# edavalosanaya/FastPoseCNN

Hardware: AMD Instinct MI355X
Metric: img/s end-to-end 640x480 inference; hough-vote kernel HBM GB/s vs roofline (higher is better)
Workload: dtype f32

## Files before the change

### fastposecnn_amd/_native.py

```python
import ctypes
import os

import torch

_HERE = os.path.dirname(os.path.abspath(__file__))
LIB_PATH = os.path.join(_HERE, "libfpc_hip.so")

_lib = None

_vp = ctypes.c_void_p
_i = ctypes.c_int
_i64 = ctypes.c_int64
_u64 = ctypes.c_uint64
_f = ctypes.c_float
_d = ctypes.c_double
_sz = ctypes.c_size_t

_SIGNATURES = {
    "fpc_abi_version": (ctypes.c_int, []),
    "fpc_error_string": (ctypes.c_char_p, [_i]),
    "fpc_last_hip_error": (ctypes.c_char_p, []),
    "fpc_generate_hypothesis": (_i, [_vp, _vp, _vp, _vp, _i, _i, _i, _vp]),
    "fpc_voting_for_hypothesis": (_i, [_vp, _vp, _vp, _vp, _i, _i, _i, _f, _vp]),
    "fpc_ransac_workspace_bytes": (_sz, [_i, _i, _i, _i]),
    "fpc_ransac_voting_v3": (_i, [_vp, _vp, _i64, _i64, _i64, _i64, _i, _vp, _i, _i, _i, _vp, _vp, _u64, _f, _i, _i,
                                  _vp, _vp, _vp, _vp, _vp, _vp, _vp, _vp, _vp, _sz, _vp]),
    "fpc_ransac_voting_v3_bits": (_i, [_vp, _vp, _vp, _i64, _i64, _i64, _i64, _i, _vp, _i, _i, _i, _vp, _vp, _u64, _f, _i, _i, _vp, _vp, _vp, _vp, _vp, _vp, _vp, _vp, _vp, _sz, _vp]),
    "fpc_ransac_voting_v3_pose": (_i, [_vp, _vp, _vp, _i64, _i64, _i64, _i64, _i, _vp, _i, _i, _i, _vp, _vp, _u64, _f, _i, _i, _vp, _vp, _vp, _vp, _vp, _vp, _vp, _vp,
                                       _vp, _vp, _vp, _vp, _vp, _vp, _vp, _sz, _vp]),
    "fpc_vote_set_prune": (_i, [_i, _i, ctypes.POINTER(ctypes.c_int32)]),
    "fpc_vote_prune_info": (_i, [_vp, _sz, _i, _i, _i, _i, _vp, _vp]),
    "fpc_class_compress": (_i, [_vp, _vp, _vp, _vp, _vp, _vp, _i, _i, _i, _vp, _vp, _vp, _vp, _vp, _vp]),
    "fpc_class_compress_bits": (_i, [_vp, _vp, _vp, _vp, _vp, _vp, _i, _i, _i, _vp, _vp, _vp, _vp, _vp, _vp, _vp]),
    "fpc_cc_workspace_bytes": (_sz, [_i, _i, _i]),
    "fpc_cc_bits_supported": (_i, [_i, _i, _i]),
    "fpc_fg_bits": (_i, [_vp, _i, _i, _i, _vp, _vp]),
    "fpc_cc_label_bits": (_i, [_vp, _i, _i, _i, _vp, _vp, _vp, _i, _vp, _sz, _vp]),
    "fpc_cc_label": (_i, [_vp, _i, _i, _i, _vp, _vp, _vp, _i, _vp, _sz, _vp]),
    "fpc_aggregate_workspace_bytes": (_sz, [_i]),
    "fpc_aggregate": (_i, [_vp, _vp, _vp, _vp, _vp, _vp, _i, _i, _i, _i, _vp, _vp, _vp, _vp, _vp, _vp, _vp, _vp, _vp, _vp, _sz,
                           _vp]),
    "fpc_aggregate_bits": (_i, [_vp, _vp, _vp, _vp, _vp, _vp, _i, _i, _i, _i, _vp, _vp, _vp, _vp, _vp, _vp, _vp, _vp, _vp, _vp, _vp, _vp, _sz, _vp]),
    "fpc_mask_bits_words": (_sz, [_i, _i]),
    "fpc_pose_errors": (_i, [_vp, _vp, _vp, _vp, _i, _vp, _vp, _vp, _vp, _vp, _vp, _i, _vp, _vp, _vp, _vp]),
    "fpc_pose_metrics_state_words": (_sz, [_i, _i, _i, _i, _i]),
    "fpc_pose_metrics_update": (_i, [_vp, _vp, _vp, _i, _i] + [_vp] * 11 + [_i, _vp, _i, _vp, _i, _vp, _i, _vp, _i, _vp, _i] + [_vp] * 5 + [_i, _vp]),
    "fpc_confusion_update": (_i, [_vp, _vp, _i64, _i, _vp, _vp]),
    "fpc_post_network_backward": (_i, [_vp, _vp, _i, _i, _i, _i, _vp, _vp, _f, _i, _u64, _vp, _vp, _vp, _vp, _vp, _vp]),
    "fpc_vote_refine_backward": (_i, [_vp, _vp, _i64, _i64, _i64, _i64, _i, _i, _i, _vp, _f, _i, _u64, _vp, _vp, _vp]),
    "fpc_class_compress_backward": (_i, [_vp, _vp, _vp, _vp, _vp, _vp, _vp, _i, _i, _i, _vp, _vp, _vp, _vp, _vp]),
    "fpc_mask_losses": (_i, [_vp, _vp, _i, _i, _i, _i64, _i64, _f, _f, _vp, _vp, _vp, _vp]),
    "fpc_match_assign": (_i, [_vp, _vp, _vp, _i, _i, _vp, _vp, _vp, _vp]),
    "fpc_matched_losses": (_i, [_vp, _vp, _vp, _i, _i] + [_vp] * 10 + [_i, _d, _i, _i, _i, ctypes.POINTER(_d)] + [_vp] * 5),
    "fpc_matched_losses_backward": (_i, [_vp, _vp, _vp, _i, _i] + [_vp] * 10 + [_i, _d, _i, _i, _i, ctypes.POINTER(_d)] + [_vp] * 8),
    "fpc_grad_sumsq": (_i, [_vp, _sz, _vp, _vp]),
    "fpc_lookahead_radam_step": (_i, [_vp, _vp, _vp, _vp, _vp, _sz, _f, _f, _f, _f, _f, _i64, _i, _f, _vp, _vp]),
    "fpc_pose_rt": (_i, [_vp, _vp, _vp, _vp, _i, _vp, _vp, _vp, _vp]),
    "fpc_pack_pose_records": (_i, [_vp] * 9 + [_i, _i, _i, _vp, _vp]),
    "fpc_mask_iou_workspace_bytes": (_sz, [_i, _i, _i64]),
    "fpc_mask_iou": (_i, [_vp, _i, _vp, _i, _i64, _i, _vp, _vp, _vp, _vp, _sz, _vp]),
    "fpc_preprocess_workspace_bytes": (_sz, [_i]),
    "fpc_preprocess_u8": (_i, [_vp, _i, _i, _i, ctypes.POINTER(ctypes.c_double), ctypes.POINTER(ctypes.c_double), _i, _vp, _vp,
                               _sz, _vp]),
    "fpc_png_info": (_i, [_vp, _sz, ctypes.POINTER(ctypes.c_int32)]),
    "fpc_png_decode": (_i, [_vp, _sz, _vp, _sz, _i]),
    "fpc_png_decode_batch": (_i, [ctypes.POINTER(_vp), ctypes.POINTER(_sz), _i, _vp, _i, _i, _i]),
    "fpc_inflate_host": (_i, [_vp, _sz, _vp, _sz, ctypes.POINTER(_sz)]),
    "fpc_png_pack_bytes": (_sz, [_i, _i, _i]),
    "fpc_png_pack_batch": (_i, [ctypes.POINTER(_vp), ctypes.POINTER(_sz), _i, _i, _i, _i, _vp, _sz, _vp, ctypes.POINTER(_sz)]),
    "fpc_png_decode_device_workspace_bytes": (_sz, [_i, _i, _i, _i]),
    "fpc_png_decode_device": (_i, [_vp, _sz, _vp, _i, _i, _i, _i, _i, _vp, _sz, _vp, _vp, _sz, _vp]),
    "fpc_gt_build": (_i, [_vp, _i64, _i64, _i, _i, _i, _vp, _vp, _vp, _i, _vp, _vp, _i, _vp, _vp]),
    "fpc_depth_decode": (_i, [_vp, _i, _i, _i, _i, _i, _vp, _vp]),
    "fpc_net_create": (_i, [ctypes.c_char_p, _i, _i, _i, _i, ctypes.POINTER(_vp)]),
    "fpc_net_create_encoder": (_i, [_i, ctypes.POINTER(_i), _i, _i, _i, _i, ctypes.POINTER(_vp)]),
    "fpc_net_create_encoder_ex": (_i, [_i, ctypes.POINTER(_i), _i, _i, _i, _i, _i, _i, ctypes.POINTER(_vp)]),
    "fpc_net_create_encoder_se": (_i, [ctypes.POINTER(_i), _i, _i, _i, _i, _i, ctypes.POINTER(_vp)]),
    "fpc_net_destroy": (None, [_vp]),
    "fpc_net_set_graph": (_i, [_vp, _i]),
    "fpc_net_set_split_precision": (_i, [_vp, _i]),
    "fpc_net_param_count": (_i, [_vp]),
    "fpc_net_param_name": (ctypes.c_char_p, [_vp, _i]),
    "fpc_net_param_numel": (_i64, [_vp, _i]),
    "fpc_net_workspace_bytes": (_sz, [_vp]),
    "fpc_net_load_params": (_i, [_vp, _vp, _i, _vp, _sz, _vp]),
    "fpc_net_forward": (_i, [_vp, _vp, _vp, _vp, _vp, _vp, _vp, _vp, _vp, _vp, _vp, _vp, _vp]),
    "fpc_net_forward_bits": (_i, [_vp, _vp, _vp, _vp, _vp, _vp, _vp, _vp, _vp, _vp, _vp, _vp, _vp, _vp]),
    "fpc_net_autotune_next": (_i, [_vp, _i]),
    "fpc_net_conv_count": (_i, [_vp]),
    "fpc_net_conv_plan": (_i, [_vp, _i, ctypes.POINTER(_i)]),
    "fpc_net_copy_plans": (_i, [_vp, _vp]),
    "fpc_net_force_winograd": (_i, [_vp, _i]),
    "fpc_net_force_pointwise": (_i, [_vp, _i]),
    "fpc_net_force_fold": (_i, [_vp, _i]),
    "fpc_net_force_direct_h3": (_i, [_vp, _i]),
    "fpc_net_force_stem_pool": (_i, [_vp, _i]),
    "fpc_act_range": (_i, [_vp, ctypes.c_longlong, _vp, _vp]),
    "fpc_net_survey_next": (_i, [_vp, _vp, _i]),
    "fpc_net_guard_ranges": (_i, [_vp, ctypes.POINTER(ctypes.c_uint32), _i, _f, _f]),
    "fpc_net_guarded": (_i, [_vp, _i]),
    "fpc_stem_pool_tasks": (_i, [_i, _i, ctypes.POINTER(_i64)]),
    "fpc_wino_pack_geometry": (_i, [_i, _i, _i, _i, _i, ctypes.POINTER(_i64)]),
    "fpc_net_set_wino_pack": (_i, [_vp, _i]),
    "fpc_net_set_wino_orient": (_i, [_vp, _i]),
    "fpc_wino_orient_geometry": (_i, [_i, _i, _i, _i, _i, _i, ctypes.POINTER(_i64)]),
    "fpc_wino_recip": (_i, [ctypes.c_uint32, ctypes.POINTER(_i64)]),
    "fpc_wino_decode": (_i, [_i, _i, _i, _i, _i, _i, _i, ctypes.POINTER(_i64)]),
    "fpc_net_wino_blocks": (_i64, [_vp]),
    "fpc_net_graph_recorded": (_i, [_vp]),
    "fpc_net_flops": (_i, [_vp, ctypes.POINTER(ctypes.c_double)]),
    "fpc_net_tensor": (_i, [_vp, ctypes.c_char_p, ctypes.POINTER(_vp), ctypes.POINTER(_i), ctypes.POINTER(_i),
                            ctypes.POINTER(_i)]),
    "fpc_conv2d_workspace_bytes": (_sz, [_i, _i, _i, _i, _i, _i, _i]),
    "fpc_conv2d_workspace_bytes_for": (_sz, [_i, _i, _i, _i, _i, _i, _i, _i, _i, _i]),
    "fpc_conv2d_plan": (_i, [_i, _i, _i, _i, _i, _i, _i, _i, _i, _i, ctypes.POINTER(_i)]),
    "fpc_conv2d": (_i, [_vp, _i64, _i64, _i64, _i64, _vp, _vp, _vp, _vp, _vp, _vp, _vp, _i, _i, _i, _i, _i, _i, _i, _i,
                        _i, _i, _i, _i, _i, _vp, _sz, _vp]),
    "fpc_conv2d_grouped_workspace_bytes": (_sz, [_i, _i]),
    "fpc_conv2d_grouped": (_i, [_vp, _i64, _i64, _i64, _i64, _vp, _vp, _vp, _vp, _i, _i, _i, _i, _i, _i, _i, _i, _vp, _sz, _vp]),
    "fpc_conv2d_grouped_dgrad_workspace_bytes": (_sz, [_i, _i]),
    "fpc_conv2d_grouped_dgrad": (_i, [_vp, _vp, _vp, _i, _i, _i, _i, _i, _i, _vp, _sz, _vp]),
    "fpc_conv2d_grouped_wgrad_workspace_bytes": (_sz, [_i, _i, _i, _i, _i]),
    "fpc_conv2d_grouped_wgrad": (_i, [_vp, _i64, _i64, _i64, _vp, _vp, _i, _i, _i, _i, _i, _i, _vp, _sz, _vp]),
    "fpc_image_nhwc4": (_i, [_vp, _vp, _i, _i, _i, _vp]),
    "fpc_stem_wgrad_workspace_bytes": (_sz, [_i, _i, _i]),
    "fpc_stem_wgrad_slices": (_i, [_i, _i, _i]),
    "fpc_stem_wgrad": (_i, [_vp, _vp, _vp, _i, _i, _i, _vp, _sz, _vp]),
    "fpc_maxpool3x3s2_fwd": (_i, [_vp, _vp, _i, _i, _i, _i, _vp]),
    "fpc_maxpool3x3s2_bwd": (_i, [_vp, _vp, _vp, _i, _i, _i, _i, _vp]),
    "fpc_se_pool_slabs": (_i, [_i, _i, _i]),
    "fpc_se_scratch_floats": (_sz, [_i, _i, _i, _i]),
    "fpc_se_gate": (_i, [_vp, _vp, _vp, _vp, _vp, _vp, _vp, _i, _i, _i, _i, _i, _vp]),
    "fpc_se_scale_add_relu": (_i, [_vp, _vp, _vp, _vp, _i, _i, _i, _i, _vp]),
    "fpc_maxpool3x3s2_ceil_fwd": (_i, [_vp, _vp, _i, _i, _i, _i, _vp]),
    "fpc_dwconv3x3": (_i, [_vp, _vp, _vp, _vp, _vp, _i, _i, _i, _i, _i, _i, _vp]),
    "fpc_conv1x1_f32": (_i, [_vp, _vp, _vp, _vp, _vp, _vp, _i64, _i, _i, _i, _vp]),
    "fpc_conv1x1_f32_form": (_i, [_i64, _i, _i]),
    "fpc_stem3x3s2": (_i, [_vp, _vp, _vp, _vp, _vp, _i, _i, _i, _i, _vp]),
    "fpc_dwconv3x3_dgrad": (_i, [_vp, _vp, _vp, _i, _i, _i, _i, _i, _vp]),
    "fpc_dwconv3x3_wgrad_workspace_bytes": (_sz, [_i, _i, _i, _i]),
    "fpc_dwconv3x3_wgrad": (_i, [_vp, _vp, _vp, _i, _i, _i, _i, _i, _vp, _sz, _vp]),
    "fpc_se_gate_train": (_i, [_vp] * 9 + [_i, _i, _i, _i, _i, _vp]),
    "fpc_se_bwd_scratch_floats": (_sz, [_i, _i, _i, _i, _i]),
    "fpc_se_bwd": (_i, [_vp] * 15 + [_i, _i, _i, _i, _i, _vp]),
    "fpc_conv2d_wgrad_workspace_bytes": (_sz, [_i, _i, _i, _i, _i, _i, _i]),
    "fpc_upsample_bilinear_fwd": (_i, [_vp, _i64, _i64, _i64, _i64, _vp, _i, _i, _i, _i, _i, _i, _vp]),
    "fpc_upsample_bilinear_bwd_scratch_floats": (_sz, [_i, _i, _i, _i, _i]),
    "fpc_upsample_bilinear_bwd": (_i, [_vp, _i64, _i64, _i64, _i64, _vp, _vp, _i, _i, _i, _i, _i, _i, _vp]),
    "fpc_groupnorm4_relu_scratch_floats": (_sz, [_i, _i, _i]),
    "fpc_groupnorm4_relu_fwd": (_i, [_vp, _vp, _vp, _vp, _vp, _vp, _i, _i, _i, _i, ctypes.c_float, _vp]),
    "fpc_groupnorm4_relu_bwd": (_i, [_vp, _vp, _vp, _vp, _vp, _vp, _vp, _i, _i, _i, _i, _vp]),
    "fpc_batchnorm_scratch_floats": (_sz, [_i, _i]),
    "fpc_batchnorm_fwd": (_i, [_vp, _vp, _vp, _vp, _vp, _vp, _vp, _vp, _vp, _i, _i, _f, _f, _i, _vp]),
    "fpc_batchnorm_bwd": (_i, [_vp, _vp, _vp, _vp, _vp, _vp, _vp, _vp, _vp, _vp, _i, _i, _i, _vp]),
    "fpc_batchnorm_act_fwd": (_i, [_vp, _vp, _vp, _vp, _vp, _vp, _vp, _vp, _vp, _i, _i, _f, _f, _i, _vp]),
    "fpc_batchnorm_act_bwd": (_i, [_vp, _vp, _vp, _vp, _vp, _vp, _vp, _vp, _vp, _vp, _i, _i, _i, _vp]),
    "fpc_conv2d_wgrad": (_i, [_vp, _i64, _i64, _i64, _vp, _vp, _i, _i, _i, _i, _i, _i, _i, _i, _i, _vp, _sz, _vp]),
    "fpc_conv2d_wgrad_split": (_i, [_vp, _i64, _i64, _i64, _vp, _vp, _i, _i, _i, _i, _i, _i, _i, _i, _i, _vp, _sz, _vp]),
}

EXPORTED = tuple(_SIGNATURES)


def lib():
    global _lib
    if _lib is None:
        if not os.path.exists(LIB_PATH):
            raise RuntimeError(
                f"fastposecnn_amd: {LIB_PATH} is missing — build it with `python -m fastposecnn_amd.build` "
                "(hipcc --offload-arch=gfx950). There is no CPU fallback for the HIP hot path.")
        L = ctypes.CDLL(LIB_PATH)
        for name, (res, args) in _SIGNATURES.items():
            fn = getattr(L, name)
            fn.restype = res
            fn.argtypes = args
        if L.fpc_abi_version() != 11:
            raise RuntimeError("fastposecnn_amd: libfpc_hip.so ABI version mismatch")
        _lib = L
    return _lib


def check(rc, what):
    if rc != 0:
        L = lib()
        msg = L.fpc_error_string(rc).decode()
        hip = L.fpc_last_hip_error().decode() if rc == -3 else ""
        raise RuntimeError(f"fastposecnn_amd: {what} failed: {msg} (code {rc}){' — HIP: ' + hip if hip else ''}")


def ptr(t):
    return None if t is None else t.data_ptr()


_raw_stream = getattr(torch._C, "_cuda_getCurrentRawStream", None)
_cur_device = getattr(torch._C, "_cuda_getDevice", None)


def stream():
    if _raw_stream is not None and _cur_device is not None:
        return _raw_stream(_cur_device())
    return torch.cuda.current_stream().cuda_stream


def require_gpu(*tensors, what="this op"):
    for t in tensors:
        if t is not None and not t.is_cuda:
            raise RuntimeError(f"fastposecnn_amd: {what} runs only on GPU tensors (HIP kernels, no CPU fallback)")


_workspaces = {}


def workspace(tag, device, nbytes):
    key = (tag, device.index, stream())
    ws = _workspaces.get(key)
    if ws is None or ws.numel() < nbytes:
        ws = torch.empty(max(int(nbytes), 256), dtype=torch.uint8, device=device)
        assert ws.data_ptr() % 256 == 0
        _workspaces[key] = ws
    return ws
```

### fastposecnn_amd/csrc/conv2d.hip

```cpp
#include <algorithm>

#include "conv_plan.hpp"

using namespace fpc;

extern "C" int fpc_stem_pool_tasks(int Ho, int Wo, int64_t* out4) {
    if (!out4 || Ho < 2 || (Ho & 1) || Wo < 64 || (Wo & 63)) return FPC_EINVAL;
    long long o[4];
    stem_pool_tasks(Ho, Wo, kStemPoolBand, o);
    for (int i = 0; i < 4; ++i) out4[i] = o[i];
    return FPC_OK;
}

extern "C" int fpc_wino_pack_geometry(int H, int W, int B, int Cin, int fold, int64_t* out8) {
    if (!out8 || H < 1 || W < 1 || B < 1 || Cin < 1) return FPC_EINVAL;
    const WinoPackGeom q = wino_pack_geometry(H, W, B, Cin, !fold);
    out8[0] = q.G; out8[1] = q.tbx; out8[2] = q.tby; out8[3] = q.patches; out8[4] = q.slots; out8[5] = q.tiles; out8[6] = q.gn_rows;
    out8[7] = q.rx;
    return FPC_OK;
}

extern "C" int fpc_wino_orient_geometry(int H, int W, int B, int Cin, int fold, int pack, int64_t* out9) {
    if (!out9 || H < 1 || W < 1 || B < 1 || Cin < 1) return FPC_EINVAL;
    bool tr;
    const WinoPackGeom q = wino_launch_geometry(H, W, B, Cin, true, pack && !fold, &tr);
    out9[0] = tr ? 1 : 0;
    out9[1] = q.G; out9[2] = q.tbx; out9[3] = q.tby; out9[4] = q.patches; out9[5] = q.slots; out9[6] = q.tiles; out9[7] = q.gn_rows;
    out9[8] = q.rx;
    return FPC_OK;
}

extern "C" int fpc_wino_recip(uint32_t d, int64_t* out2) {
    if (!out2 || d < 1 || d > (1u << 31)) return FPC_EINVAL;
    const WinoRecip r = wino_recip(d);
    out2[0] = r.m; out2[1] = r.sh;
    return FPC_OK;
}
extern "C" int fpc_wino_decode(int Cout, int groups, int tbx, int tby, int W, int B, int pack, int64_t* out14) {
    if (!out14 || Cout < 64 || groups < 1 || tbx < 1 || tby < 1 || W < 1 || B < 1 || pack < 0) return FPC_EINVAL;
    const WinoDecode d = wino_decode(Cout, groups, tbx, tby, W, B, pack);
    const WinoRecip r[7] = {d.nnb, d.groups, d.tbx, d.tby, d.per, d.tbxl, d.tcw};
    for (int i = 0; i < 7; ++i) { out14[2 * i] = r[i].m; out14[2 * i + 1] = r[i].sh; }
    return FPC_OK;
}

extern "C" size_t fpc_conv2d_workspace_bytes(int B, int Ho, int Wo, int Cin, int Cout, int Kh, int Kw) {
    int K = Cin * Kh * Kw, Kpad = cdiv(K, kConvBK) * kConvBK, Npad = cdiv(Cout, kConvNAlign) * kConvNAlign;
    size_t packed = conv_packed_floats(Npad, Kpad);
    size_t splitk = (size_t)32 * B * (cdiv(Ho * Wo, 128) * 128) * Npad;
    size_t wino = wino_region_floats(kImgH3, Cout, Cin, true);
    return (packed + splitk + wino + kConvTickets) * sizeof(float);
}

namespace {
struct Conv2dLayout { size_t packed, splitk, wino, tickets, total; };
Conv2dLayout conv2d_layout(int B, int Cin, int Cout, int Kh, int Kw, const ConvPlan& p, const Conv2dRequest& r) {
    const int K = Cin * Kh * Kw, Kpad = cdiv(K, kConvBK) * kConvBK, Npad = cdiv(Cout, kConvNAlign) * kConvNAlign;
    Conv2dLayout L;
    L.packed = r.wino ? 0 : conv_packed_floats(Npad, Kpad);
    L.splitk = r.wino ? 0 : (splitk_floats_for(p, 1, B, Npad) + 63) / 64 * 64;
    L.wino = r.wino ? wino_region_floats(kWinoForms[r.wino].image, Cout, Cin, Cout % 128 == 0) : 0;
    L.tickets = (!r.wino && p.fused && p.nsplit > 1) ? kConvTickets : 0;
    L.total = L.packed + L.splitk + L.wino + L.tickets;
    return L;
}
ConvPlan conv2d_plan_for(int B, int Ho, int Wo, int Cin, int Cout, int Kh, int Kw, int bm, int bn, const Conv2dRequest& r) {
    const int Kpad = cdiv(Cin * Kh * Kw, kConvBK) * kConvBK;
    ConvPlan p = plan_conv(Ho * Wo, B, Cout, Kpad / kConvBK, 1, r.wino ? 0 : bm, bn, r.wino ? 1 : r.nsplit);
    p.bf3 = r.bf3 ? 1 : 0;
    p.h3 = r.h3 ? 1 : 0;
    if (r.two_launch) p.fused = 0;
    p.lat = r.lat;
    p.stem = r.stem ? 256 : 0;
    p.pool = r.pool ? 1 : 0;
    p.pw = r.pw;
    p.wino = r.wino;
    return p;
}
}

extern "C" int fpc_conv2d_plan(int B, int Ho, int Wo, int Cin, int Cout, int Kh, int Kw, int bm, int bn, int nsplit,
                               int* out4) {
    if (!out4) return FPC_EINVAL;
    const int Kpad = cdiv(Cin * Kh * Kw, kConvBK) * kConvBK;
    const Conv2dRequest r = decode_plan(nsplit);
    ConvPlan p = plan_conv(Ho * Wo, B, Cout, Kpad / kConvBK, 1, bm, bn, r.nsplit);
    p.wino = r.wino;
    out4[0] = p.bm; out4[1] = p.bn; out4[2] = r.wino ? nsplit : p.nsplit; out4[3] = plan_gn_rows(p, Ho, Wo, B, Cin, r.pack, r.orient);
    return FPC_OK;
}

extern "C" size_t fpc_conv2d_workspace_bytes_for(int B, int Ho, int Wo, int Cin, int Cout, int Kh, int Kw, int bm, int bn,
                                                 int nsplit) {
    if (B < 1 || Ho < 1 || Wo < 1 || Cin < 1 || Cout < 1 || Kh < 1 || Kw < 1) return 0;
    const Conv2dRequest r = decode_plan(nsplit);
    const ConvPlan p = conv2d_plan_for(B, Ho, Wo, Cin, Cout, Kh, Kw, bm, bn, r);
    return std::max<size_t>(conv2d_layout(B, Cin, Cout, Kh, Kw, p, r).total * sizeof(float), 256);
}

extern "C" int fpc_conv2d(const float* in, int64_t sb, int64_t sh, int64_t sw, int64_t sc, const float* w_oihw,
                          const float* scale, const float* shift, const float* res, const float* up, float* out,
                          float* gn_part, int B, int Hi, int Wi, int Cin, int Cout, int Kh, int Kw, int stride, int pad,
                          int relu, int bm, int bn, int nsplit, void* ws, size_t ws_bytes, fpc_stream_t stream) {
    if (!in || !w_oihw || !out || !ws || B < 1 || Kh != Kw) return FPC_EINVAL;
    int Ho = conv_out(Hi, Kh, stride, pad), Wo = conv_out(Wi, Kw, stride, pad);
    if (Ho < 1 || Wo < 1) return FPC_EINVAL;
    const Conv2dRequest rq = decode_plan(nsplit);
    if (rq.grp) return FPC_EINVAL;
    const int wino = rq.wino;
    ConvPlan p = conv2d_plan_for(B, Ho, Wo, Cin, Cout, Kh, Kw, bm, bn, rq);
    const Conv2dLayout lay = conv2d_layout(B, Cin, Cout, Kh, Kw, p, rq);
    if (ws_bytes < lay.total * sizeof(float) || ((uintptr_t)ws & 255)) return FPC_EWORKSPACE;
    PackedConv c;
    c.Cin = c.Cinp = Cin; c.Cout = Cout; c.Kh = Kh; c.Kw = Kw; c.stride = stride; c.pad = pad;
    c.K = Cin * Kh * Kw; c.Kpad = cdiv(c.K, kConvBK) * kConvBK; c.Npad = cdiv(Cout, kConvNAlign) * kConvNAlign;
    hipStream_t s = (hipStream_t)stream;
    float* packed = (float*)ws;
    if (rq.stem) {
        if (Cin != 4 || Kh != 7 || stride != 2 || pad != 3 || Cout != 64 || sc != 1 || sw != 4 || sh != (int64_t)4 * Wi ||
            sb != (int64_t)4 * Hi * Wi || res || up || gn_part)
            return FPC_EINVAL;
        c.Kwp = 8; c.K = 4 * 7 * 8; c.Kpad = 224;
        FPC_TRY((rq.pool ? launch_pack_weight_h3 : launch_pack_weight_bf3)(w_oihw, packed, Cout, Cin, Cin, Kh, Kw, c.Kwp, c.Npad, c.Kpad, s));
        ConvArgs a0;
        fill_conv_shape(a0, B, c, p, Hi, Wi, Ho, Wo, sb, sh, sw, sc, relu != 0, 0);
        a0.Cin = 8 * c.Cinp; a0.Kw = 1; a0.K = c.K; a0.lanepx = 1;
        a0.p[0] = ConvPtrs{in, packed, out, scale, shift, nullptr, nullptr, nullptr};
        return rq.pool ? launch_stem_pool(a0, packed, out, Ho / 2, Wo / 2, s) : launch_conv_plan(a0, p, 1, s);
    }
    static_assert(FPC_IGEMM_DMA_B, "the split-precision direct form stages its B rows from the bf16 planes by LDS-DMA; a build that loads "
                                   "them from the f32 image must pack that image here as well");
    if (!wino) FPC_TRY((p.h3 ? launch_pack_weight_h3 : p.bf3 ? launch_pack_weight_bf3 : launch_pack_weight)(w_oihw, packed, Cout, Cin, Cin, Kh, Kw, Kw, c.Npad, c.Kpad, s));
    int mode = (sc == 1 && Cin % kConvBK == 0 && Kh * Kw <= 32 && ((int64_t)Hi + 2 * pad) * sh * 4 < ((int64_t)1 << 31)) ? 0
               : (sc == 1 && Cin % 4 == 0 && sw % 4 == 0 && sh % 4 == 0 && sb % 4 == 0 && ((uintptr_t)in & 15) == 0) ? 2 : 1;
    ConvArgs a;
    fill_conv_shape(a, B, c, p, Hi, Wi, Ho, Wo, sb, sh, sw, sc, relu != 0, mode);
    a.wino_pack = rq.pack ? 1 : 0;
    a.wino_orient = rq.orient ? 1 : 0;
    a.splitk_ws = packed + lay.packed;
    a.p[0] = ConvPtrs{in, packed, out, scale, shift, res, up, gn_part};
    if (lay.tickets) {
        float* tk = packed + lay.packed + lay.splitk + lay.wino;
        a.tickets = (int*)tk;
        if (hipMemsetAsync(tk, 0, kConvTickets * sizeof(int), s) != hipSuccess) return FPC_ELAUNCH;
    }
#ifdef FPC_STAMP_WINO
    if (wino && relu == 77) { a.dbg = gn_part; a.p[0].gn_part = nullptr; a.relu = 0; }
#endif
#ifdef FPC_STAMP_IGEMM
    if (!wino && relu == 77) { a.dbg = gn_part; a.p[0].gn_part = nullptr; a.relu = 0; }
#endif
    if (wino) {
        if (Kh != 3 || stride != 1 || pad != 1 || Cin % 8 || Cout % 64 || sc != 1 || up || sw != Cin ||
            sh != (int64_t)Wi * Cin || sb != (int64_t)Hi * Wi * Cin)
            return FPC_EINVAL;
        float* wp = packed + lay.packed + lay.splitk;
        if (!wino_form_ok(wino, Cin, Cout)) return FPC_EINVAL;
        const WinoImage img = kWinoForms[wino].image;
        if (rq.orient && wino_orient_rule(Ho, Wo)) FPC_TRY(launch_wino_pack_h3(w_oihw, wp + wino_image_offset(img, Cout, Cin), Cout, Cin, true, s));
        else FPC_TRY(kWinoImages[img].pack(w_oihw, wp + wino_image_offset(img, Cout, Cin), Cout, Cin, s));
        a.wino_w[0] = wp;
        a.zeros = zero_page();
        if (!a.zeros) {
            float* zp = wp + lay.wino - 64;
            if (hipMemsetAsync(zp, 0, 64 * sizeof(float), s) != hipSuccess) return FPC_ELAUNCH;
            a.zeros = zp;
        }
        return launch_conv_plan(a, p, 1, s);
    }
    if (p.h3) {
        if (mode != 0) return FPC_EINVAL;
        a.h3_w[0] = packed;
        return launch_conv_plan(a, p, 1, s);
    }
    a.bf3 = (p.bf3 && mode == 0) ? 1 : 0;
    if (p.bf3 && mode != 0) return FPC_EINVAL;
    if (p.lat || p.pw) return launch_conv_plan(a, p, 1, s);
    return launch_conv_plan(a, ConvPlan{a.bm, a.bn, a.nsplit, a.mtiles, a.ntiles, 0, a.bf3, a.fused}, 1, s);
}

extern "C" size_t fpc_conv2d_grouped_workspace_bytes(int C, int groups) {
    if (C < 32 || C % 32 || groups < 1 || C % groups || !grouped_cg_ok(C / groups)) return 0;
    return std::max<size_t>(align_up((size_t)C * (C / groups) * 9 * sizeof(float), 256), 256);
}

extern "C" int fpc_conv2d_grouped(const float* in, int64_t sb, int64_t sh, int64_t sw, int64_t sc, const float* w_oihw,
                                  const float* scale, const float* shift, float* out, int B, int Hi, int Wi, int C, int groups,
                                  int stride, int relu, int form, void* ws, size_t ws_bytes, fpc_stream_t stream) {
    if (!in || !w_oihw || !out || !ws || B < 1 || Hi < 1 || Wi < 1 || C < 32 || C % 32 || groups < 1 || C % groups ||
        !grouped_cg_ok(C / groups) || (stride != 1 && stride != 2) || sc != 1 || form < 0 || form >= 1000)
        return FPC_EINVAL;
    const Conv2dRequest rq = decode_plan(FPC_PLAN_GROUPED + form);
    if (!rq.grp || rq.grp > kGroupedForms) return FPC_EINVAL;
    if (ws_bytes < fpc_conv2d_grouped_workspace_bytes(C, groups) || ((uintptr_t)ws & 255)) return FPC_EWORKSPACE;
    hipStream_t s = (hipStream_t)stream;
    GroupedArgs g;
    memset(&g, 0, sizeof(g));
    g.in = in; g.w = (const float*)ws; g.out = out; g.scale = scale; g.shift = shift;
    g.in_sb = sb; g.in_sh = sh; g.in_sw = sw;
    g.B = B; g.Hi = Hi; g.Wi = Wi; g.Ho = conv_out(Hi, 3, stride, 1); g.Wo = conv_out(Wi, 3, stride, 1);
    g.C = C; g.CG = C / groups; g.stride = stride; g.relu = relu ? 1 : 0; g.form = rq.grp - 1;
    if (((uintptr_t)in | (uintptr_t)out | (uintptr_t)scale | (uintptr_t)shift | (uintptr_t)w_oihw) & 15) return FPC_EINVAL;
    if ((sb | sh | sw) % 4 || sw < C) return FPC_EINVAL;
    FPC_TRY(launch_pack_grouped(w_oihw, (float*)ws, C, g.CG, s));
    return launch_conv3x3_grouped(g, s);
}
```

### fastposecnn_amd/csrc/conv_launch.hip

```cpp
#include "conv_plan.hpp"

namespace fpc {

int launch_conv_plan(ConvArgs& a, const ConvPlan& p, int groups, hipStream_t s) {
    if (p.grp || a.cg) {
        if (!p.grp || p.grp > kGroupedForms || !a.cg || !a.grp_w || groups != 1 || a.in_sc != 1 || a.Kh != 3 || a.pad != 1 ||
            a.Cin != a.Cout || a.p[0].res || a.p[0].up || a.p[0].gn_part)
            return FPC_EINVAL;
        GroupedArgs g;
        memset(&g, 0, sizeof(g));
        g.in = a.p[0].in; g.w = a.grp_w; g.out = a.p[0].out; g.scale = a.p[0].scale; g.shift = a.p[0].shift;
        g.in_sb = a.in_sb; g.in_sh = a.in_sh; g.in_sw = a.in_sw;
        g.B = a.B; g.Hi = a.Hi; g.Wi = a.Wi; g.Ho = a.Ho; g.Wo = a.Wo; g.C = a.Cout; g.CG = a.cg; g.stride = a.stride; g.relu = a.relu;
        g.form = p.grp - 1;
        return launch_conv3x3_grouped(g, s);
    }
    if (p.stem) {
        if (groups != 1 || !stem_ok(a)) return FPC_EINVAL;
        StemArgs t;
        memset(&t, 0, sizeof(t));
        t.in = a.p[0].in;
        t.wpl = reinterpret_cast<const unsigned short*>(a.p[0].w + (size_t)a.Npad * a.Kpad);
        t.out = a.p[0].out; t.scale = a.p[0].scale; t.shift = a.p[0].shift;
        t.B = a.B; t.Hi = a.Hi; t.Wi = a.Wi; t.Ho = a.Ho; t.Wo = a.Wo; t.Cout = a.Cout; t.Npad = a.Npad; t.Kpad = a.Kpad; t.relu = a.relu;
        t.grid = p.stem;
        return launch_stem7x7(t, s);
    }
    if (p.pw) {
        if (!pw_ok(a, groups)) return FPC_EINVAL;
        PwArgs w;
        memset(&w, 0, sizeof(w));
        w.in = a.p[0].in;
        for (int g = 0; g < groups; ++g) {
            w.wpl[g] = reinterpret_cast<const unsigned short*>(a.p[g].w + (size_t)a.Npad * a.Kpad);
            w.out[g] = a.p[g].out; w.scale[g] = a.p[g].scale; w.shift[g] = a.p[g].shift; w.res[g] = a.p[g].res; w.up[g] = a.p[g].up;
        }
        w.in_sb = a.in_sb; w.in_sh = a.in_sh; w.in_sw = a.in_sw;
        w.B = a.B; w.Ho = a.Ho; w.Wo = a.Wo; w.Cin = a.Cin; w.Cout = a.Cout; w.Npad = a.Npad; w.Kpad = a.Kpad; w.stride = a.stride;
        w.groups = groups; w.relu = a.relu;
        w.has_scale = a.p[0].scale != nullptr; w.has_shift = a.p[0].shift != nullptr;
        w.has_res = a.p[0].res != nullptr; w.has_up = a.p[0].up != nullptr;
        w.variant = p.pw - 1;
        return launch_conv1x1(w, s);
    }
    if (p.lat) {
        if (!lateral_ok(a, groups)) return FPC_EINVAL;
        LatArgs l;
        memset(&l, 0, sizeof(l));
        l.in = a.p[0].in;
        for (int g = 0; g < groups; ++g) {
            if (p.h3 && !a.h3_w[g]) return FPC_EINVAL;
            l.wpl[g] = reinterpret_cast<const unsigned short*>(p.h3 ? a.h3_w[g] : a.p[g].w + (size_t)a.Npad * a.Kpad);
            l.out[g] = a.p[g].out; l.shift[g] = a.p[g].shift; l.up[g] = a.p[g].up;
        }
        l.B = a.B; l.Ho = a.Ho; l.Wo = a.Wo; l.Cout = a.Cout; l.Npad = a.Npad; l.Kpad = a.Kpad; l.groups = groups; l.relu = a.relu;
        l.parts = p.lat;
        l.h3 = p.h3;
        return launch_lateral1x1(l, s);
    }
    if (p.wino) {
        if (!wino_form_ok(p.wino, a.Cin, a.Cout)) return FPC_EINVAL;
        const WinoForm& f = kWinoForms[p.wino];
        WinoArgs w;
        memset(&w, 0, sizeof(w));
        for (int g = 0; g < groups; ++g) {
            if (!a.wino_w[g] || a.p[g].up) return FPC_EINVAL;
            w.p[g] = a.p[g];
            w.p[g].w = a.wino_w[g] + wino_image_offset(f.image, a.Cout, a.Cin);
        }
        w.variant = f.variant;
        w.zeros = a.zeros;
        w.dbg = (long long*)a.dbg;
        w.groups = groups;
        w.B = a.B; w.H = a.Ho; w.W = a.Wo; w.Cin = a.Cin; w.Cout = a.Cout; w.relu = a.relu;
        w.waves = f.waves;
        const WinoGrid wg = wino_grid(p.wino, a.Ho, a.Wo);
        w.tbx = wg.tbx; w.tby = wg.tby;
        if (p.wino == kWinoH3) {
            bool tr;
            const WinoPackGeom q = wino_launch_geometry(a.Ho, a.Wo, a.B, a.Cin, a.wino_orient, a.wino_pack && !p.fold, &tr);
            if (q.G > 1 || tr) { w.pack = q.G; w.tbx = q.tbx; w.tby = q.tby; w.pack_rx = q.rx; }
            w.orient = tr ? 1 : 0;
            a.wino_blocks = q.patches * (a.Cout / 64) * groups;
        }
        if (p.fold) {
            if (p.wino != kWinoH3 || !a.fold_in) return FPC_EINVAL;
            for (int g = 0; g < groups; ++g) {
                w.in2[g] = a.fold_up[g]; w.w2[g] = a.fold_w2[g];
                w.btab[g] = a.fold_tab[g];
                w.p[g].in = a.fold_in; w.p[g].w = a.fold_w[g];
            }
            w.fold = 1; w.Cin2 = a.Cin; w.Cin = a.fold_cin;
        }
        return f.launch(w, groups, s);
    }
    a.bm = p.bm; a.bn = p.bn; a.nsplit = p.nsplit; a.mtiles = p.mtiles; a.ntiles = p.ntiles; a.groups = groups;
    a.bf3 = (p.bf3 && a.generic == 0) ? 1 : 0;
    a.fused = (p.fused && p.nsplit > 1) ? 1 : 0;
    a.h3 = 0;
    ConvArgs h;
    if (p.h3) {
        if (a.generic != 0) return FPC_EINVAL;
        h = a;
        h.bf3 = 0; h.h3 = 1;
        for (int g = 0; g < groups; ++g) {
            if (!a.h3_w[g]) return FPC_EINVAL;
            h.p[g].w = a.h3_w[g];
        }
    }
    const ConvArgs& l = p.h3 ? h : a;
    int rc = launch_conv(l, groups, s);
    if (!rc && l.nsplit > 1 && !l.fused) rc = launch_conv_splitk_epilogue(l, groups, s);
    return rc;
}

int plan_gn_rows(const ConvPlan& p, int Ho, int Wo, int B, int Cin, int pack, int orient) {
    bool tr;
    if (p.wino == kWinoH3) return wino_launch_geometry(Ho, Wo, B, Cin, orient, pack && !p.fold, &tr).gn_rows;
    return p.wino ? wino_grid(p.wino, Ho, Wo).patches() : p.mtiles * p.bm / 32;
}

int launch_stem_pool(const ConvArgs& a, const float* h3_image, float* pool, int Hp, int Wp, hipStream_t s) {
    if (!h3_image || !stem_ok(a)) return FPC_EINVAL;
    StemPoolArgs t;
    memset(&t, 0, sizeof(t));
    t.in = a.p[0].in; t.wpl = reinterpret_cast<const unsigned short*>(h3_image); t.out = pool;
    t.scale = a.p[0].scale; t.shift = a.p[0].shift;
    t.B = a.B; t.Hi = a.Hi; t.Wi = a.Wi; t.Ho = a.Ho; t.Wo = a.Wo; t.Hp = Hp; t.Wp = Wp; t.Npad = a.Npad; t.Kpad = a.Kpad; t.relu = a.relu;
    t.band = kStemPoolBand; t.grid = 256;
    return launch_stem_pool_h3(t, s);
}

}
```

### fastposecnn_amd/csrc/conv_plan.hpp

```cpp
#pragma once
#include <math.h>
#include <string.h>

#include <vector>

#include "net_kernels.hpp"

#define FPC_TRY(x) do { int rc__ = (x); if (rc__) return rc__; } while (0)

namespace fpc {

struct PackedConv {
    int Cin = 0, Cinp = 0, Cout = 0, Kh = 1, Kw = 1, stride = 1, pad = 0;
    int Kwp = 1;
    int K = 0, Kpad = 0, Npad = 0;
    int p_w = -1;
    int p_bn = -1;
    int p_bias = -1;
    size_t w_off = 0, scale_off = 0, shift_off = 0;
    size_t wino_off = 0;
    bool wino_ok = false;
    size_t h3_off = 0;
    bool h3_ok = false;
    int cg = 0;
// ... 6 lines not shown
    int bm = 64, bn = 64, nsplit = 1, mtiles = 1, ntiles = 1, wino = 0, bf3 = 0, fused = 0;
    int lat = 0;
    int stem = 0;
    int pw = 0;
    int fold = 0;
    int h3 = 0;
    int pool = 0;
    int grp = 0;
};

inline bool stem_ok(const ConvArgs& a) {
    return a.lanepx == 1 && a.generic == 0 && a.Kh == 7 && a.stride == 2 && a.pad == 3 && a.Cout == 64 && a.Kpad == 224 &&
           a.Wo % 64 == 0 && !a.p[0].res && !a.p[0].up && !a.p[0].gn_part && a.in_sc == 1 && a.in_sw == 4 &&
           a.in_sh == (long long)4 * a.Wi && a.in_sb == (long long)4 * a.Hi * a.Wi;
}

inline bool lateral_ok(const ConvArgs& a, int groups) {
    if (a.Kh != 1 || a.Kw != 1 || a.stride != 1 || a.pad != 0 || a.generic != 0 || (a.Cin != 64 && a.Cin != 128) || a.Kpad != a.Cin ||
        a.Cout % 32 != 0 || a.in_sc != 1 || a.in_sw != a.Cin || a.in_sh != (long long)a.Wi * a.Cin ||
        a.in_sb != (long long)a.Hi * a.Wi * a.Cin || a.lanepx)
        return false;
    for (int g = 0; g < groups; ++g)
        if (a.p[g].in != a.p[0].in || a.p[g].scale || a.p[g].res || a.p[g].gn_part || ((a.p[g].up != nullptr) != (a.p[0].up != nullptr)))
            return false;
    return !(a.p[0].up && ((a.Ho | a.Wo) & 1));
}

inline bool pw_ok(const ConvArgs& a, int groups) {
    if (a.Kh != 1 || a.Kw != 1 || a.pad != 0 || (a.stride != 1 && a.stride != 2) || a.generic != 0 || a.lanepx || a.Cin % 64 != 0 ||
        a.Kpad != a.Cin || a.Cout % 64 != 0 || a.in_sc != 1)
        return false;
    for (int g = 0; g < groups; ++g)
        if (a.p[g].in != a.p[0].in || a.p[g].gn_part || (a.p[g].scale != nullptr) != (a.p[0].scale != nullptr) ||
            (a.p[g].shift != nullptr) != (a.p[0].shift != nullptr) || (a.p[g].res != nullptr) != (a.p[0].res != nullptr) ||
            (a.p[g].up != nullptr) != (a.p[0].up != nullptr))
            return false;
    return !(a.p[0].up && ((a.Ho | a.Wo) & 1));
}

inline bool can_fuse(const ConvPlan& p, int groups, int B) {
    return p.nsplit > 1 && (long long)groups * B * p.mtiles * p.ntiles <= kConvTickets;
}

inline ConvPlan plan_conv(int HoWo, int B, int Cout, int ksteps, int groups, int force_bm = 0, int force_bn = 0,
                          int force_split = 0) {
    ConvPlan best;
    double best_t = 1e300;
    const int bms[2] = {64, 128}, bns[2] = {64, 128};
    for (int bi = 0; bi < 2; ++bi)
        for (int bj = 0; bj < 2; ++bj) {
            int bm = bms[bi], bn = bns[bj];
            if (force_bm && bm != force_bm) continue;
            if (force_bn && bn != force_bn) continue;
            if (!force_bn && bn == 128 && Cout <= 64) continue;
            int mt = cdiv(HoWo, bm), nt = cdiv(Cout, bn);
            for (int ns = 1; ns <= 32; ++ns) {
                if (force_split && ns != force_split) continue;
                int per = cdiv(ksteps, ns);
                if ((ns - 1) * per >= ksteps) continue;
                if (ns > 1 && (Cout % 4 != 0)) continue;
                double nblk = (double)groups * B * mt * nt * ns;
                double work = (double)(bm / 64) * (bn / 64) * per * 16.0 * 64.0 + 4000.0;
                double t = ceil(nblk / 256.0) * work + (ns > 1 ? 10000.0 + 200.0 * ns : 0.0);
                if (t < best_t) { best_t = t; best = ConvPlan{bm, bn, ns, mt, nt, 0}; }
            }
        }
    best.fused = can_fuse(best, groups, B) ? 1 : 0;
    return best;
}

inline std::vector<ConvPlan> conv_candidates(int HoWo, int B, int Cout, int ksteps, int groups) {
    std::vector<ConvPlan> out;
    const int splits[] = {1, 2, 3, 4, 6, 8, 12, 16, 24};
    for (int bm = 64; bm <= 128; bm += 64)
        for (int bn = 64; bn <= 128; bn += 64) {
            if (bn == 128 && Cout <= 64) continue;
            int mt = cdiv(HoWo, bm), nt = cdiv(Cout, bn);
            long long base = (long long)groups * B * mt * nt;
            for (int ns : splits) {
                int per = cdiv(ksteps, ns);
                if (ns > 1 && (per < 2 || (ns - 1) * per >= ksteps || Cout % 4 != 0)) continue;
                if (ns > 1 && base * ns > 4096) continue;
                out.push_back(ConvPlan{bm, bn, ns, mt, nt, 0});
                if (can_fuse(out.back(), groups, B)) { ConvPlan f = out.back(); f.fused = 1; out.push_back(f); }
            }
        }
    return out;
}

inline size_t splitk_floats_for(const ConvPlan& p, int groups, int B, int Npad) {
    return p.nsplit > 1 ? (size_t)groups * p.nsplit * B * p.mtiles * p.bm * Npad : 0;
}

enum WinoImage { kImgF32, kImgBf3, kImgC128, kImgH2, kImgH3, kWinoImageCount };
struct WinoImageDesc { int units, tail; int (*pack)(const float* w_oihw, float* packed, int Cout, int Cin, hipStream_t s); };
inline int pack_h3_plain(const float* w_oihw, float* packed, int Cout, int Cin, hipStream_t s) { return launch_wino_pack_h3(w_oihw, packed, Cout, Cin, false, s); }
constexpr WinoImageDesc kWinoImages[kWinoImageCount] = {
    {16, 0, launch_wino_pack},
    {24, 0, launch_wino_pack_bf3},
    {24, 0, launch_wino_pack_c128},
    {16, 8, launch_wino_pack_h2},
    {16, 8, pack_h3_plain},
};
constexpr size_t kWinoSlack = 128;

constexpr int kWinoFormCount = 10;
constexpr int kWinoBf3 = 5, kWinoW4 = 7;
constexpr int kWinoH2 = 8, kWinoH3 = 9;
struct WinoForm {
    int waves;
    int bn, ck;
    int variant;
    WinoImage image;
    int wg_per_cu;
    int min_split;
    bool zeros;
    bool range_limited;
    int (*launch)(const WinoArgs& a, int groups, hipStream_t s);
};
constexpr WinoForm kWinoForms[kWinoFormCount] = {
    {},
    {4, 64, 8, 0, kImgF32, 2, 0, false, false, launch_conv_wino},
    {8, 64, 8, 0, kImgF32, 1, 0, false, false, launch_conv_wino},
    {4, 64, 8, 1, kImgF32, 2, 0, false, false, launch_conv_wino},
    {8, 64, 8, 2, kImgF32, 1, 0, true, false, launch_conv_wino},
    {8, 64, 8, 3, kImgBf3, 1, 1, true, false, launch_conv_wino},
    {4, 128, 8, 0, kImgC128, 1, 1, false, false, launch_conv_wino_c128},
    {8, 64, 8, 0, kImgBf3, 1, 1, false, false, launch_conv_wino_w4},
    {8, 64, 8, 0, kImgH2, 1, 2, false, true, launch_conv_wino_h2},
    {8, 64, 16, 0, kImgH3, 1, 3, false, true, launch_conv_wino_h3},
};
inline bool wino_form_ok(int form, int Cin, int Cout) {
    return form >= 1 && form < kWinoFormCount && Cout % kWinoForms[form].bn == 0 && Cin % kWinoForms[form].ck == 0;
}
struct WinoSpan { size_t units, tails; };
inline WinoSpan wino_span(int end, bool c128) {
    WinoSpan sp{0, 0};
    for (int i = 0; i < end; ++i)
        if (i != kImgC128 || c128) { sp.units += kWinoImages[i].units; sp.tails += kWinoImages[i].tail; }
    return sp;
}
static_assert(kWinoImages[kImgH2].tail + kWinoImages[kImgH3].tail <= 64, "kWinoSlack keeps one 64-float line for all tails");
inline size_t wino_image_offset(WinoImage img, int Cout, int Cin) {
    const WinoSpan sp = wino_span(img, Cout % 128 == 0);
    return sp.units * Cout * Cin + sp.tails;
}
inline size_t wino_region_floats(WinoImage last, int Cout, int Cin, bool c128) { return (wino_span(last, c128).units + kWinoImages[last].units) * Cout * Cin + kWinoSlack; }
inline bool plan_range_limited(const ConvPlan& p) {
    return p.h3 || p.fold || p.pool || (p.wino && kWinoForms[p.wino].range_limited);
}
struct WinoGrid { int tbx, tby; int patches() const { return tbx * tby; } };
inline WinoGrid wino_grid(int form, int H, int W) { return {cdiv(cdiv(W, 2), 8), cdiv(cdiv(H, 2), kWinoForms[form].waves)}; }

struct Conv2dRequest { int nsplit; bool bf3, two_launch; int wino, lat; bool stem; int pw; bool h3, pool, pack, orient; int grp; };
inline Conv2dRequest decode_plan(int code) {
    Conv2dRequest r{code, false, false, 0, 0, false, 0, false, false, false, false, 0};
    if (code >= FPC_PLAN_GROUPED && code < FPC_PLAN_GROUPED + 1000) { r.grp = code - FPC_PLAN_GROUPED + 1; r.nsplit = 1; return r; }
    if (code == FPC_PLAN_WINO_ORIENT) { r.orient = true; r.nsplit = -kWinoH3; }
    if (code == FPC_PLAN_WINO_PACKED) { r.pack = true; r.nsplit = -kWinoH3; }
    if (r.nsplit >= FPC_PLAN_LATERAL_H3 && r.nsplit < FPC_PLAN_LATERAL_H3 + 1000) { r.lat = r.nsplit - FPC_PLAN_LATERAL_H3; r.h3 = true; r.nsplit = 1; return r; }
    if (r.nsplit >= FPC_PLAN_H3 && r.nsplit < FPC_PLAN_H3 + 200) { r.h3 = true; r.nsplit -= FPC_PLAN_H3; }
    if (r.nsplit >= FPC_PLAN_POINTWISE) { r.pw = r.nsplit - FPC_PLAN_POINTWISE + 1; r.bf3 = true; r.nsplit = 1; return r; }
    if (r.nsplit == FPC_PLAN_STEM_POOL) { r.stem = true; r.pool = true; r.h3 = true; r.nsplit = 1; return r; }
    if (r.nsplit == FPC_PLAN_STEM) { r.stem = true; r.bf3 = true; r.nsplit = 1; return r; }
    if (r.nsplit >= FPC_PLAN_LATERAL) { r.lat = r.nsplit - FPC_PLAN_LATERAL; r.bf3 = true; r.nsplit = 1; return r; }
    if (r.nsplit >= FPC_PLAN_BF3) { r.bf3 = true; r.nsplit -= FPC_PLAN_BF3; }
    if (r.nsplit >= FPC_PLAN_TWO_LAUNCH) { r.two_launch = true; r.nsplit -= FPC_PLAN_TWO_LAUNCH; }
    if (r.nsplit <= -1 && r.nsplit > -kWinoFormCount) r.wino = -r.nsplit;
    return r;
}
inline int encode_plan(const ConvPlan& p, bool folded_away) {
    if (folded_away) return FPC_PLAN_FOLDED;
    if (p.grp) return FPC_PLAN_GROUPED + p.grp - 1;
    if (p.h3) return p.lat ? FPC_PLAN_LATERAL_H3 + p.lat : FPC_PLAN_H3 + p.nsplit;
    if (p.pw) return FPC_PLAN_POINTWISE + p.pw - 1;
    if (p.stem) return p.pool ? FPC_PLAN_STEM_POOL : FPC_PLAN_STEM;
    if (p.lat) return FPC_PLAN_LATERAL + p.lat;
    return p.wino ? -p.wino : p.nsplit;
}

inline int conv_out(int x, int k, int s, int p) { return (x + 2 * p - k) / s + 1; }
inline void fill_conv_shape(ConvArgs& a, int B, const PackedConv& c, const ConvPlan& p, int Hi, int Wi, int Ho, int Wo, long long sb,
                            long long sh, long long sw, long long sc, bool relu, int mode) {
    memset(&a, 0, sizeof(a));
    a.B = B; a.Hi = Hi; a.Wi = Wi; a.Cin = c.Cin; a.Ho = Ho; a.Wo = Wo; a.Cout = c.Cout; a.Npad = c.Npad;
    a.Kh = c.Kh; a.Kw = c.Kw; a.stride = c.stride; a.pad = c.pad; a.K = c.K; a.Kpad = c.Kpad;
    a.in_sb = sb; a.in_sh = sh; a.in_sw = sw; a.in_sc = sc;
    a.relu = relu ? 1 : 0; a.nsplit = p.nsplit; a.mtiles = p.mtiles; a.ntiles = p.ntiles; a.ksteps = c.Kpad / kConvBK;
    a.bm = p.bm; a.bn = p.bn; a.generic = mode;
    a.fused = p.fused;
}

int launch_conv_plan(ConvArgs& a, const ConvPlan& p, int groups, hipStream_t s);
int plan_gn_rows(const ConvPlan& p, int Ho, int Wo, int B, int Cin, int pack, int orient);
int launch_stem_pool(const ConvArgs& a, const float* h3_image, float* pool, int Hp, int Wp, hipStream_t s);

}
```

### fastposecnn_amd/csrc/net.hip

```cpp
#include <initializer_list>
#include <utility>

#include "net_plan.hpp"

static void drop_graph(fpc_net* n) {
    if (n->graph_exec) { (void)hipGraphExecDestroy(n->graph_exec); n->graph_exec = nullptr; }
}

extern "C" void fpc_net_destroy(fpc_net_t* n) {
    if (!n) return;
    if (n->graph_exec) (void)hipGraphExecDestroy(n->graph_exec);
    delete n;
}

static int pack_h3_images(fpc_net* n, hipStream_t s) {
    for (const PackedConv& c : n->convs)
        if (c.h3_ok) {
            int rc = launch_pack_weight_h3(n->pptr[c.p_w], n->ws + c.h3_off, c.Cout, c.Cin, c.Cinp, c.Kh, c.Kw, c.Kwp, c.Npad, c.Kpad, s);
            if (rc) return rc;
        }
    if (n->c_stem >= 0) {
        const PackedConv& st = n->convs[n->c_stem];
        int rc = launch_pack_weight_h3(n->pptr[st.p_w], n->ws + n->stem_h3_off, st.Cout, st.Cin, st.Cinp, st.Kh, st.Kw, st.Kwp, st.Npad, st.Kpad, s);
        if (rc) return rc;
    }
    n->h3_packed = true;
    return FPC_OK;
}

extern "C" int fpc_net_set_split_precision(fpc_net_t* n, int on) {
    if (!n) return FPC_EINVAL;
    n->split_precision = on < 0 ? 0 : (on > 3 ? 3 : on);
    if (n->split_precision >= 3 && n->loaded && !n->h3_packed) return pack_h3_images(n, n->load_stream);
    return FPC_OK;
}

extern "C" int fpc_net_graph_recorded(const fpc_net_t* n) { return n && n->use_graph && n->graph_exec ? 1 : 0; }

extern "C" int fpc_net_set_wino_pack(fpc_net_t* n, int on) {
    if (!n || on < 0 || on > 1) return FPC_EINVAL;
    if (n->wino_pack != on) drop_graph(n);
    n->wino_pack = on;
    return FPC_OK;
}

static int pack_wino_h3_image(const fpc_net* n, int ci, hipStream_t s) {
    const PackedConv& c = n->convs[ci];
    return launch_wino_pack_h3(n->pptr[c.p_w], n->ws + c.wino_off + wino_image_offset(kImgH3, c.Cout, c.Cin), c.Cout, c.Cin,
                               n->wino_orient && n->c_tr[ci], s);
}
static int pack_fold_images(const fpc_net* n, int d, hipStream_t s) {
    const PackedConv &sc = n->convs[n->dec[d].seg[6]], &lc = n->convs[n->dec[d].lat[3]];
    const bool tr = n->wino_orient && n->c_tr[n->dec[d].seg[6]];
    int rc = launch_fold_compose(n->pptr[sc.p_w], n->pptr[lc.p_w], n->pptr[lc.p_bias], n->ws + n->fold_wc_off[d],
                                 n->ws + n->fold_tab_off[d], sc.Cout, sc.Cin, lc.Cin, tr, s);
    if (!rc) rc = launch_wino_pack_h3_pair(n->ws + n->fold_wc_off[d], n->ws + n->fold_img1_off[d], lc.Cin, n->pptr[sc.p_w],
                                           n->ws + n->fold_img2_off[d], sc.Cin, sc.Cout, tr, s);
    return rc;
}

extern "C" int fpc_net_set_wino_orient(fpc_net_t* n, int on) {
    if (!n || on < 0 || on > 1) return FPC_EINVAL;
    if (n->wino_orient == on) return FPC_OK;
    drop_graph(n);
    n->wino_orient = on;
    if (!n->loaded) return FPC_OK;
    if (hipDeviceSynchronize() != hipSuccess) return FPC_ELAUNCH;
    for (size_t ci = 0; ci < n->convs.size(); ++ci)
        if (n->c_tr[ci] && wino_form_ok(kWinoH3, n->convs[ci].Cin, n->convs[ci].Cout)) { const int rc = pack_wino_h3_image(n, (int)ci, n->load_stream); if (rc) return rc; }
    if (n->fold_ok && n->c_tr[n->dec[0].seg[6]])
        for (int d = 0; d < 4; ++d) { const int rc = pack_fold_images(n, d, n->load_stream); if (rc) return rc; }
    return hipStreamSynchronize(n->load_stream) == hipSuccess ? FPC_OK : FPC_ELAUNCH;
}

extern "C" int64_t fpc_net_wino_blocks(const fpc_net_t* n) { return n ? (int64_t)n->wino_blocks : -1; }

extern "C" int fpc_net_set_graph(fpc_net_t* n, int on) {
    if (!n) return FPC_EINVAL;
    n->use_graph = on ? 1 : 0;
    if (!on) drop_graph(n);
    return FPC_OK;
}
extern "C" int fpc_net_param_count(const fpc_net_t* n) { return n ? (int)n->pnames.size() : 0; }
extern "C" const char* fpc_net_param_name(const fpc_net_t* n, int i) {
    return (n && i >= 0 && i < (int)n->pnames.size()) ? n->pnames[i].c_str() : nullptr;
}
extern "C" int64_t fpc_net_param_numel(const fpc_net_t* n, int i) {
    return (n && i >= 0 && i < (int)n->pnumel.size()) ? n->pnumel[i] : -1;
}
extern "C" size_t fpc_net_workspace_bytes(const fpc_net_t* n) { return n ? n->total_floats * sizeof(float) : 0; }

static int fold_bn_of(const fpc_net* n, int p_bn, int C, size_t scale_off, size_t shift_off, hipStream_t s) {
    return launch_fold_bn(n->pptr[p_bn], n->pptr[p_bn + 1], n->pptr[p_bn + 2], n->pptr[p_bn + 3], 1e-5f, C, n->ws + scale_off, n->ws + shift_off, s);
}

extern "C" int fpc_net_load_params(fpc_net_t* n, const float* const* params, int count, void* ws, size_t ws_bytes,
                                   fpc_stream_t stream) {
    if (!n || !params || count != (int)n->pnames.size() || !ws) return FPC_EINVAL;
    if (((uintptr_t)ws & 255) != 0 || ws_bytes < n->total_floats * sizeof(float)) return FPC_EWORKSPACE;
    drop_graph(n);
    for (int i = 0; i < count; ++i)
        if (!params[i] || ((uintptr_t)params[i] & 15)) return FPC_EINVAL;
    hipStream_t s = (hipStream_t)stream;
    n->ws = (float*)ws;
    n->pptr.assign(params, params + count);
    n->load_stream = s;
    n->h3_packed = false;
    if (n->split_precision >= 3) { int rc = pack_h3_images(n, s); if (rc) return rc; }
    if (hipMemsetAsync(n->ws + n->zeros_off, 0, 64 * sizeof(float), s) != hipSuccess) return FPC_ELAUNCH;
    if (hipMemsetAsync(n->ws + n->tickets_off, 0, kConvTickets * sizeof(int), s) != hipSuccess) return FPC_ELAUNCH;
    for (size_t ci = 0; ci < n->convs.size(); ++ci) {
        const PackedConv& c = n->convs[ci];
        if (c.cg) {
            int rg = launch_pack_grouped(n->pptr[c.p_w], n->ws + c.grp_off, c.Cout, c.cg, s);
            if (!rg) rg = fold_bn_of(n, c.p_bn, c.Cout, c.scale_off, c.shift_off, s);
            if (rg) return rg;
            continue;
        }
        int rc = launch_pack_weight(n->pptr[c.p_w], n->ws + c.w_off, c.Cout, c.Cin, c.Cinp, c.Kh, c.Kw, c.Kwp, c.Npad, c.Kpad, s);
        if (rc) return rc;
        rc = launch_pack_weight_bf3(n->pptr[c.p_w], n->ws + c.w_off, c.Cout, c.Cin, c.Cinp, c.Kh, c.Kw, c.Kwp, c.Npad, c.Kpad, s);
        if (rc) return rc;
        if (c.wino_ok) {
            for (int f = 1, done = 0; f < kWinoFormCount; ++f) {
                const WinoImage img = kWinoForms[f].image;
                if (!wino_form_ok(f, c.Cin, c.Cout) || (done >> img & 1)) continue;
                done |= 1 << img;
                rc = img == kImgH3 ? pack_wino_h3_image(n, (int)ci, s)
                                   : kWinoImages[img].pack(n->pptr[c.p_w], n->ws + c.wino_off + wino_image_offset(img, c.Cout, c.Cin), c.Cout, c.Cin, s);
                if (rc) return rc;
            }
        }
        if (c.p_bn >= 0) {
            rc = fold_bn_of(n, c.p_bn, c.Cout, c.scale_off, c.shift_off, s);
            if (rc) return rc;
        }
    }
    if (n->fold_ok)
        for (int d = 0; d < 4; ++d) {
            const int rc = pack_fold_images(n, d, s);
            if (rc) return rc;
        }
    for (const fpc_net::MbOp& o : n->mops) {
        const int rc = fold_bn_of(n, o.p_bn, o.Cout, o.scale_off, o.shift_off, s);
        if (rc) return rc;
    }
    n->loaded = true;
    return FPC_OK;
}

namespace {

struct ConvIO {
    const float* in; long long sb, sh, sw, sc; int Hi, Wi;
    float* out; int Ho, Wo;
    const float* res; const float* up; float* gn_part;
};

void fill_conv_args(const fpc_net* n, ConvArgs& a, const PackedConv& c, const ConvPlan& p, int Hi, int Wi, int Ho,
                    int Wo, long long sb, long long sh, long long sw, long long sc, bool relu, int mode) {
    fill_conv_shape(a, n->B, c, p, Hi, Wi, Ho, Wo, sb, sh, sw, sc, relu, mode);
    a.splitk_ws = n->ws + n->splitk_off; a.zeros = n->ws + n->zeros_off; a.tickets = (int*)(n->ws + n->tickets_off);
    a.wino_pack = n->wino_pack; a.wino_orient = n->wino_orient;
}


template <class F> float min_ms(hipStream_t s, int reps, F run) {
    hipEvent_t e0 = nullptr, e1 = nullptr;
    float ms = 1e30f;
    if (hipEventCreate(&e0) == hipSuccess && hipEventCreate(&e1) == hipSuccess)
        for (int rep = 0; rep < reps; ++rep) {
            float t = 0.f;
            bool timed = hipEventRecord(e0, s) == hipSuccess && run() == FPC_OK && hipEventRecord(e1, s) == hipSuccess &&
                         hipEventSynchronize(e1) == hipSuccess && hipEventElapsedTime(&t, e0, e1) == hipSuccess;
            if (timed && t < ms) ms = t;
        }
    if (e0) (void)hipEventDestroy(e0);
    if (e1) (void)hipEventDestroy(e1);
    return ms;
}

std::vector<ConvPlan> tune_candidates(const ConvArgs& a, int groups, int split, bool pointwise) {
    if (a.cg) {
        std::vector<ConvPlan> gc;
        for (int f = 0; f < kGroupedForms; ++f) { ConvPlan q; q.grp = f + 1; gc.push_back(q); }
        return gc;
    }
    std::vector<ConvPlan> cands = conv_candidates(a.Ho * a.Wo, a.B, a.Cout, a.ksteps, groups);
    const size_t nf = cands.size();
    if (split && a.generic == 0) {
        for (size_t i = 0; i < nf; ++i) { ConvPlan q = cands[i]; q.bf3 = 1; cands.push_back(q); }
    }
    if (split >= 3 && a.generic == 0 && a.h3_w[0]) {
        for (size_t i = 0; i < nf; ++i) { ConvPlan q = cands[i]; q.h3 = 1; cands.push_back(q); }
    }
    if (split && groups == 1 && stem_ok(a)) {
        ConvPlan sq; sq.stem = 256; cands.push_back(sq);
    }
    if (split && lateral_ok(a, groups)) {
        const int tiles = groups * (a.Cout / 32);
        for (int parts = 1; parts <= tiles; parts *= 2)
            if (tiles % parts == 0) {
                ConvPlan lq; lq.lat = parts; cands.push_back(lq);
                if (split >= 3 && a.h3_w[0]) { lq.h3 = 1; cands.push_back(lq); }
            }
    }
    if (split && pointwise && pw_ok(a, groups)) {
        ConvPlan pq;
        pq.pw = 1; cands.push_back(pq);
        pq.pw = 2; cands.push_back(pq);
    }
    if (a.wino_w[0] && !a.p[0].up) {
        auto offered = [&](int f) { return split >= kWinoForms[f].min_split && wino_form_ok(f, a.Cin, a.Cout) && (a.zeros || !kWinoForms[f].zeros); };
        for (int f = 1; f < kWinoFormCount; ++f) {
            if (!offered(f) || (f == kWinoH2 && offered(kWinoH3))) continue;
            ConvPlan wq; wq.wino = f; cands.push_back(wq);
        }
    }
    return cands;
}

struct PlanFootprint { double nblk, share; };
PlanFootprint plan_footprint(const ConvPlan& q, const ConvArgs& a, int groups) {
    bool tr;
    double nblk = q.grp ? (double)cdiv(a.Ho, 8) * cdiv(a.Wo, grouped_tile_cols(a.stride)) * (a.Cout / 32) * a.B
                  : q.stem ? 512.0
                  : q.lat ? (double)cdiv(a.Ho * a.Wo, 128) * a.B * q.lat
                  : q.pw ? (double)cdiv(a.B * a.Ho * a.Wo, pw_tile_pixels(q.pw - 1)) * (a.Cout / 64) * groups * q.pw
                  : q.wino == kWinoH3 ? (double)wino_launch_geometry(a.Ho, a.Wo, a.B, a.Cin, a.wino_orient, a.wino_pack && !q.fold, &tr).patches * (a.Cout / 64) * groups
                  : q.wino ? (double)wino_grid(q.wino, a.Ho, a.Wo).patches() * a.B * (a.Cout / kWinoForms[q.wino].bn) * groups
                         : (double)q.mtiles * q.ntiles * q.nsplit * a.B * groups;
    double share = nblk / (256.0 * (q.wino ? kWinoForms[q.wino].wg_per_cu : 2));
    if (share > 1.0) share = 1.0;
    if (share < 0.125) share = 0.125;
    return {nblk, share};
}

int survey_site(const fpc_net* n, const ConvArgs& a, const ConvPlan& p, int groups, int ci, hipStream_t s) {
    unsigned* rec = n->survey + 4 * (size_t)ci;
    if (p.fold) {
        unsigned* rec_up = n->survey + 4 * (size_t)n->dec[0].lat[3];
        int rc = launch_act_range(a.fold_in, (long long)a.B * a.Ho * a.Wo * a.fold_cin, rec, s);
        for (int g = 0; g < groups && !rc; ++g) rc = launch_act_range(a.fold_up[g], (long long)a.B * (a.Ho / 2) * (a.Wo / 2) * a.Cin, rec_up, s);
        return rc;
    }
    for (int g = 0; g < groups; ++g) {
        bool seen = false;
        for (int h = 0; h < g; ++h) seen = seen || a.p[h].in == a.p[g].in;
        if (seen) continue;
        const int rc = launch_act_range(a.p[g].in, (long long)a.B * a.in_sb, rec, s);
        if (rc) return rc;
    }
    return FPC_OK;
}

int run_conv(fpc_net* n, ConvArgs& a, int groups, int ci, hipStream_t s) {
    if (n->tuning) {
        float best_ms = 1e30f, free_ms = 1e30f;
        ConvPlan best = n->cplan[ci];
        n->has_free[ci] = 0;
        for (const ConvPlan& q : tune_candidates(a, groups, n->split_precision, n->enc.pointwise())) {
            if (splitk_floats_for(q, groups, a.B, a.Npad) > n->splitk_floats) continue;
            if (n->guarded[ci] && plan_range_limited(q)) continue;
            int rc = launch_conv_plan(a, q, groups, s);
            if (rc == FPC_EINVAL) continue;
            if (rc) return rc;
            const float ms = min_ms(s, 3, [&] { return launch_conv_plan(a, q, groups, s); });
            float score = ms;
            if (n->tune_mode >= 1) {
                const double share = plan_footprint(q, a, groups).share;
                score = ms * (float)(n->tune_mode == 2 ? share : sqrt(share));
            }
            if (score < best_ms) { best_ms = score; best = q; }
            if (score < free_ms && !plan_range_limited(q)) { free_ms = score; n->free_plan[ci] = q; n->has_free[ci] = 1; }
        }
        n->tune_score[ci] = best_ms;
        if (n->split_precision >= 3 && a.fold_in && a.fold_lat_ms > 0.f && !n->guarded[ci]) {
            ConvPlan fq;
            fq.wino = kWinoH3; fq.fold = 1;
            int rc = launch_conv_plan(a, fq, groups, s);
            if (rc && rc != FPC_EINVAL) return rc;
            const float ms = rc ? 1e30f : min_ms(s, 3, [&] { return launch_conv_plan(a, fq, groups, s); });
            if (ms < best_ms + a.fold_lat_ms) best = fq;
        }
        n->cplan[ci] = best;
    }
    const ConvPlan p = n->cplan[ci];
    if (n->survey) { const int rs = survey_site(n, a, p, groups, ci, s); if (rs) return rs; }
    const int rc = launch_conv_plan(a, p, groups, s);
    if (!rc && p.wino == kWinoH3) n->wino_blocks += a.wino_blocks;
    return rc;
}

}


static int forward_middle(fpc_net* n, hipStream_t s) {
    float* ws = n->ws;
    n->wino_blocks = 0;
    const int B = n->B, H = n->H, W = n->W;
    ConvArgs a;
    auto nhwc = [&](const Act& t, long long& sb, long long& sh, long long& sw, long long& sc) {
        sc = 1; sw = t.C; sh = (long long)t.W * t.C; sb = (long long)t.H * sh;
    };
    if (n->c_stem >= 0) {
        const PackedConv& c = n->convs[n->c_stem];
        fill_conv_args(n, a, c, n->cplan[n->c_stem], H, W, n->a_stem.H, n->a_stem.W, (long long)4 * H * W, (long long)4 * W, 4,
                       1, true, 0);
        a.Cin = 8 * c.Cinp; a.Kw = 1; a.K = c.K; a.lanepx = 1;
        a.p[0] = ConvPtrs{ws + n->a_img4.off, ws + c.w_off, ws + n->a_stem.off, ws + c.scale_off, ws + c.shift_off, nullptr, nullptr, nullptr};
        const float* h3img = n->h3_packed ? ws + n->stem_h3_off : nullptr;
        const bool ceil = n->enc.resnet.ceil_pool();
        auto pool_launch = [&]() {
            return ceil ? launch_maxpool3x3s2_ceil(ws + n->a_stem.off, ws + n->a_pool.off, B, n->a_stem.H, n->a_stem.W, 64, s)
                        : launch_maxpool3x3s2(ws + n->a_stem.off, ws + n->a_pool.off, B, n->a_stem.H, n->a_stem.W, 64, n->a_pool.H, n->a_pool.W, s);
        };
// ... 487 lines not shown
```

### fastposecnn_amd/csrc/net_kernels.hpp

```cpp
#pragma once
#include "common.hpp"

namespace fpc {

#ifndef FPC_IGEMM_DMA_B
#define FPC_IGEMM_DMA_B 1
#endif

constexpr int kMaxGroup = 4;
constexpr int kConvBK = 32;
constexpr int kConvNAlign = 128;
constexpr int kConvTickets = 16384;

struct ConvPtrs {
    const float* in;
    const float* w;
    float* out;
    const float* scale;
    const float* shift;
    const float* res;
    const float* up;
    float* gn_part;
};

struct ConvArgs {
    ConvPtrs p[kMaxGroup];
    float* splitk_ws;
    int* tickets;
    int fused;
    int B, Hi, Wi, Cin, Ho, Wo, Cout, Npad, Kh, Kw, stride, pad, K, Kpad;
    long long in_sb, in_sh, in_sw, in_sc;
    int relu, nsplit, mtiles, ntiles, ksteps, bm, bn, generic, groups;
    int bf3;
    int h3;
    int lanepx;
    const float* wino_w[kMaxGroup];
    const float* h3_w[kMaxGroup];
    const float* zeros;
    const float* fold_in;
    const float* fold_w[kMaxGroup];
    const float* fold_w2[kMaxGroup];
    const float* fold_up[kMaxGroup];
    const float* fold_tab[kMaxGroup];
    int fold_cin;
    float fold_lat_ms;
    void* dbg;
    long long wino_blocks;
    int wino_pack;
    int wino_orient;
    int cg;
    const float* grp_w;
};

struct LatArgs {
    const float* in;
    const unsigned short* wpl[kMaxGroup];
    float* out[kMaxGroup];
    const float* shift[kMaxGroup];
    const float* up[kMaxGroup];
    int B, Ho, Wo, Cout, Npad, Kpad, groups, relu;
    unsigned bias_mask;
    int parts;
    int h3;
};
int launch_lateral1x1(const LatArgs& a, hipStream_t s);

struct PwArgs {
    const float* in;
    const unsigned short* wpl[kMaxGroup];
    float* out[kMaxGroup];
    const float* scale[kMaxGroup];
    const float* shift[kMaxGroup];
    const float* res[kMaxGroup];
    const float* up[kMaxGroup];
    long long in_sb, in_sh, in_sw;
    int B, Ho, Wo, Cin, Cout, Npad, Kpad, stride, groups, relu;
    int has_scale, has_shift, has_res, has_up;
    int variant;
};
int launch_conv1x1(const PwArgs& a, hipStream_t s);
inline int pw_tile_pixels(int variant) { return variant == 0 ? 64 : 128; }

struct GroupedArgs {
    const float* in;
    const float* w;
    float* out;
    const float* scale;
    const float* shift;
    long long in_sb, in_sh, in_sw;
    int B, Hi, Wi, Ho, Wo, C, CG, stride, relu;
    int form;
    int tx, ty;
};
constexpr int kGroupedForms = 1;
bool grouped_cg_ok(int cg);
int launch_pack_grouped(const float* w_oihw, float* packed, int C, int CG, hipStream_t s, int mode = 0);
int launch_conv3x3_grouped(const GroupedArgs& a, hipStream_t s);
inline int grouped_tile_cols(int stride) { return stride == 1 ? 16 : 8; }

struct StemArgs {
    const float* in;
    const unsigned short* wpl;
    float* out;
    const float* scale;
    const float* shift;
    int B, Hi, Wi, Ho, Wo, Cout, Npad, Kpad, relu;
    int grid;
};
int launch_stem7x7(const StemArgs& a, hipStream_t s);

struct StemPoolArgs {
    const float* in;
    const unsigned short* wpl;
    float* out;
    const float* scale;
    const float* shift;
    int B, Hi, Wi, Ho, Wo, Hp, Wp, Npad, Kpad, relu;
    int band;
    int grid;
};
constexpr int kStemPoolBand = 10;
int launch_stem_pool_h3(const StemPoolArgs& a, hipStream_t s);
void stem_pool_tasks(int Ho, int Wo, int band, long long out4[4]);

constexpr int kMaxGnSites = 4;
struct GnFinArgs {
    const float* gn_part[kMaxGnSites * kMaxGroup];
    const float* gamma[kMaxGnSites * kMaxGroup];
    const float* beta[kMaxGnSites * kMaxGroup];
    float* affine[kMaxGnSites * kMaxGroup];
    int P[kMaxGnSites];
    long long count[kMaxGnSites];
    int B, C, groups, sites;
    float eps;
};

constexpr int kMaxUpJobs = 2;
struct GnUpArgs {
    const float* in[kMaxUpJobs * kMaxGroup];
    const float* affine[kMaxUpJobs * kMaxGroup];
    float* out[kMaxUpJobs * kMaxGroup];
    int h[kMaxUpJobs], w[kMaxUpJobs];
    int B, C, jobs;
};

struct MergeHeadArgs {
    const float* t_lo[kMaxGroup][3];
    const float* a_lo[kMaxGroup][3];
    const float* t_hi[kMaxGroup];
    const float* a_hi[kMaxGroup];
    const float* hw[kMaxGroup];
    const float* hb[kMaxGroup];
    float* out[kMaxGroup];
    int ch[kMaxGroup];
    int chp[kMaxGroup];
    int B, h, w, C;
};

struct HeadPartArgs {
    const float* t[kMaxGroup][3];
    const float* aff[kMaxGroup][3];
    const float* hw[kMaxGroup];
    const float* hb[kMaxGroup];
    const float* lsum[kMaxGroup];
    float* out[kMaxGroup];
    int ch[kMaxGroup], chp[kMaxGroup];
    int B, H, W, C, hl, wl;
};
int launch_head_part(const HeadPartArgs& a, bool hi, int groups, hipStream_t s);

struct Up4Args {
    const float* lm; const float* lq; const float* lt; const float* ls;
    int pm, pq, pt, ps;
    float* o_mask; float* o_quat; float* o_scales; float* o_xy; float* o_z;
    long long* cat_mask; float* cq; float* cs; float* cxy; float* cz;
    int B, hl, wl, H, W, C;
    unsigned long long* fg_bits; size_t fg_stride;
};

#ifdef FPC_STAMP_WINO
constexpr bool kWinoStamp = true;
#else
constexpr bool kWinoStamp = false;
#endif
constexpr int kWinoSerialStamps = 16;

struct WinoRecip { unsigned m; int sh; };
inline WinoRecip wino_recip(unsigned d) {
    int l = 0;
    while ((1ull << l) < d) ++l;
    const int sh = 31 + l;
    return WinoRecip{(unsigned)(((1ull << sh) + d - 1) / d), sh};
}
struct WinoDecode { WinoRecip nnb, groups, tbx, tby, per, tbxl, tcw; };
inline WinoDecode wino_decode(int Cout, int groups, int tbx, int tby, int W, int B, int pack) {
    const int tcw = (W + 1) / 2, last = pack > 0 ? ((B % pack) * tcw + 7) / 8 : 0;
    return WinoDecode{wino_recip(Cout / 64), wino_recip(groups), wino_recip(tbx), wino_recip(tby), wino_recip(tbx * tby),
                      wino_recip(last ? last : tbx), wino_recip(tcw)};
}

struct WinoArgs {
    ConvPtrs p[kMaxGroup];
    long long* dbg;
    const float* zeros;
    int variant;
    int groups;
    int waves;
    int B, H, W, Cin, Cout, relu, tbx, tby;
    const float* in2[kMaxGroup];
    const float* w2[kMaxGroup];
    const float* btab[kMaxGroup];
    int fold, Cin2;
    int pack, pack_rx;
    int orient;
    WinoDecode dec;
};
int launch_conv_wino(const WinoArgs& a, int groups, hipStream_t s);
const float* zero_page();
int launch_wino_pack(const float* w_oihw, float* packed, int Cout, int Cin, hipStream_t s);
int launch_wino_pack_bf3(const float* w_oihw, float* packed, int Cout, int Cin, hipStream_t s);
int launch_conv_wino_c128(const WinoArgs& a, int groups, hipStream_t s);
int launch_wino_pack_c128(const float* w_oihw, float* packed, int Cout, int Cin, hipStream_t s);
int launch_conv_wino_w4(const WinoArgs& a, int groups, hipStream_t s);
int launch_conv_wino_h2(const WinoArgs& a, int groups, hipStream_t s);
int launch_wino_pack_h2(const float* w_oihw, float* packed, int Cout, int Cin, hipStream_t s);
int launch_absmax_bits(const float* w, long long n, unsigned* out_bits, hipStream_t s);
int launch_act_range(const float* x, long long n, unsigned* rec4, hipStream_t s);
int launch_conv_wino_h3(const WinoArgs& a, int groups, hipStream_t s);
struct WinoPackGeom { int G, tbx, tby, rx; long long patches, slots, tiles; int gn_rows; };
WinoPackGeom wino_pack_geometry(int H, int W, int B, int Cin, bool allow);
bool wino_orient_rule(int H, int W);
WinoPackGeom wino_launch_geometry(int H, int W, int B, int Cin, bool orient, bool pack_allow, bool* transposed);
int launch_wino_pack_h3(const float* w_oihw, float* packed, int Cout, int Cin, bool transpose, hipStream_t s);
int launch_wino_pack_h3_pair(const float* w1, float* packed1, int Cin1, const float* w2, float* packed2, int Cin2, int Cout, bool transpose,
                             hipStream_t s);
int launch_fold_compose(const float* W, const float* L, const float* bias, float* wc, float* btab, int Cout, int Cmid, int Cin,
                        bool transpose, hipStream_t s);
int launch_conv(const ConvArgs& a, int groups, hipStream_t s);
int launch_conv_splitk_epilogue(const ConvArgs& a, int groups, hipStream_t s);
int launch_maxpool3x3s2(const float* in, float* out, int B, int Hi, int Wi, int C, int Ho, int Wo, hipStream_t s);
int launch_maxpool3x3s2_ceil(const float* in, float* out, int B, int Hi, int Wi, int C, hipStream_t s);
int se_pool_slabs(int H, int W, int C);
int launch_se_pool(const float* x, float* partial, int B, int H, int W, int C, hipStream_t s);
int launch_se_excite(const float* partial, const float* w1, const float* b1, const float* w2, const float* b2, float* gate, int B, int H,
                     int W, int C, int R, hipStream_t s);
int launch_se_scale_add_relu(const float* x, const float* gate, const float* res, float* y, int B, int H, int W, int C, hipStream_t s);
int launch_se_excite_train(const float* partial, const float* w1, const float* b1, const float* w2, const float* b2, float* gate,
                           float* mean, float* hidden, int B, int H, int W, int C, int R, hipStream_t s);
constexpr int kSeThreads = 256;
constexpr int kSeRowPixels = 64;
constexpr int kSeMaxC = 8192;
inline int se_lanes(int C) { return C / 4 < kSeThreads ? C / 4 : kSeThreads; }
inline int se_rows(int C) { return kSeThreads / se_lanes(C); }
inline bool se_shape_ok(int B, int H, int W, int C) {
    return B >= 1 && B <= 65535 && H >= 1 && W >= 1 && C >= 64 && C % 64 == 0 && C <= kSeMaxC && (long long)H * W < (1LL << 31) &&
           (long long)B * H * W * (C / 4) < (1LL << 32) - 4096LL * 256 - 8;
}
int launch_stem3x3s2(const float* in4, const float* w, const float* scale, const float* shift, float* out, int B, int Hi, int Wi,
                     hipStream_t s);
int launch_dwconv3x3(const float* in, const float* w, const float* scale, const float* shift, float* out, int B, int Hi, int Wi, int C,
                     int stride, int act, hipStream_t s);
int launch_conv1x1_f32(const float* in, const float* w, const float* scale, const float* shift, const float* res, float* out, long long M,
                       int Cin, int Cout, int act, hipStream_t s);
int conv1x1_f32_tiles(long long M, int Cout);
int launch_gn_finalize(const GnFinArgs& a, int groups, hipStream_t s);
int launch_gn_relu_up2(const GnUpArgs& a, int groups, hipStream_t s);
int launch_merge_head(const MergeHeadArgs& a, int groups, hipStream_t s);
int launch_up4_compress(const Up4Args& a, hipStream_t s, bool allow_wide = true);
void launch_up4_compress7x4(const Up4Args& a, hipStream_t s);
void launch_up4_compress_wide(const Up4Args& a, hipStream_t s);

struct Lerp { int i0, i1; float l0, l1; };
__device__ __forceinline__ Lerp lerp_coord(int dst, int in, int out) {
    float scale = out > 1 ? (float)(in - 1) / (float)(out - 1) : 0.f;
    float src = scale * (float)dst;
    Lerp L;
    L.i0 = (int)src;
    L.i1 = L.i0 + (L.i0 < in - 1 ? 1 : 0);
    L.l1 = src - (float)L.i0;
    L.l0 = 1.f - L.l1;
    return L;
}

__device__ __forceinline__ Lerp lerp_scaled(int dst, int in, float scale) {
    float src = scale * (float)dst;
    Lerp L;
    L.i0 = (int)src;
    L.i1 = L.i0 + (L.i0 < in - 1 ? 1 : 0);
    L.l1 = src - (float)L.i0;
    L.l0 = 1.f - L.l1;
    return L;
}

int launch_pack_weight(const float* w_oihw, float* packed, int Cout, int Cin, int Cinp, int Kh, int Kw, int Kwp, int Npad,
                       int Kpad, hipStream_t s);
int launch_pack_weight_bf3(const float* w_oihw, float* packed, int Cout, int Cin, int Cinp, int Kh, int Kw, int Kwp, int Npad,
                           int Kpad, hipStream_t s);
inline size_t conv_packed_floats(int Npad, int Kpad) { return ((size_t)Npad * Kpad * 5 / 2 + 63) / 64 * 64; }
int launch_pack_weight_h3(const float* w_oihw, float* packed, int Cout, int Cin, int Cinp, int Kh, int Kw, int Kwp, int Npad,
                          int Kpad, hipStream_t s);
inline size_t h3_packed_floats(int Npad, int Kpad) { return ((size_t)Npad * Kpad + 2 + 63) / 64 * 64; }
int launch_nchw3_to_nhwc4(const float* x, float* out, int B, int HW, hipStream_t s);
int launch_fold_bn(const float* gamma, const float* beta, const float* mean, const float* var, float eps, int C,
                   float* scale, float* shift, hipStream_t s);

}
```

### fastposecnn_amd/csrc/net_plan.hpp

```cpp
#pragma once
#include <string>

#include "conv_plan.hpp"

using namespace fpc;

enum Buf { kBufNone, kBufIn, kBufT1, kBufT2, kBufD, kBufY, kBufRes, kBufCount };
struct BlockSite { int k; bool strided, grouped; Buf in, out; bool relu; Buf res; };
struct BlockKind {
    int nsites;
    BlockSite site[3];
    int ds_before;
    bool se_gate;
    bool shared;
};
constexpr BlockKind kBasicBlock = {2, {{3, true, false, kBufIn, kBufT1, true, kBufNone}, {3, false, false, kBufT1, kBufY, true, kBufRes}}, 1, false, false};
constexpr BlockKind kBottleneck = {3, {{1, false, false, kBufIn, kBufT1, true, kBufNone}, {3, true, true, kBufT1, kBufT2, true, kBufNone}, {1, false, false, kBufT2, kBufY, true, kBufRes}}, 2, false, true};
constexpr BlockKind kSEBottleneck = {3, {{1, true, false, kBufIn, kBufT1, true, kBufNone}, {3, false, false, kBufT1, kBufT2, true, kBufNone}, {1, false, false, kBufT2, kBufY, false, kBufNone}}, 2, true, true};

enum EncoderFamily {
    kFamilyResNet,
    kFamilyMobileNetV2,
    kFamilyCount
};
struct ResNetDesc {
    int expansion = 1;
    int groups = 1, width = 64;
    int se = 0;
    const BlockKind& kind() const { return se ? kSEBottleneck : expansion == 4 ? kBottleneck : kBasicBlock; }
    const char* stem_prefix() const { return se ? "encoder.layer0." : "encoder."; }
    bool ceil_pool() const { return se != 0; }
};
struct EncoderDesc {
    EncoderFamily family = kFamilyResNet;
    ResNetDesc resnet;
    int layers[4] = {};
    bool basic() const { return family == kFamilyResNet && resnet.expansion == 1; }
    bool pointwise() const { return family == kFamilyResNet && resnet.expansion == 4; }
};

enum StepKind {
    kStepConv,
    kStepSeGate,
    kStepMb
};
struct Step { StepKind kind; int op; Act in, out; bool relu; Act res; };
inline Step conv_step(int conv, const Act& in, const Act& out, bool relu, const Act& res = Act()) {
    Step s; s.kind = kStepConv; s.op = conv; s.in = in; s.out = out; s.relu = relu; s.res = res; return s;
}
inline Step se_gate_step(int p_se, const Act& y, const Act& res) {
    Step s; s.kind = kStepSeGate; s.op = p_se; s.in = s.out = y; s.relu = true; s.res = res; return s;
}
inline Step mb_step(int mop, const Act& in, const Act& out, const Act& res = Act()) {
    Step s; s.kind = kStepMb; s.op = mop; s.in = in; s.out = out; s.relu = false; s.res = res; return s;
}

struct fpc_net {
    EncoderDesc enc;
    int classes, B, H, W;
    std::vector<std::string> pnames;
    std::vector<int64_t> pnumel;
    std::vector<const float*> pptr;
    std::vector<PackedConv> convs;
    size_t packed_floats = 0;
    size_t total_floats = 0;
    float* ws = nullptr;
    bool loaded = false;
    bool tuning = false;
    bool tuned = false;
    int tune_mode = 0;

    int c_stem = -1;
    std::vector<Step> tape;
    enum MbKind { kMbStem, kMbDw, kMbPw };
    struct MbOp { MbKind kind; int p_w, p_bn, Cin, Cout, stride, act; size_t scale_off, shift_off; long long howo; };
    std::vector<MbOp> mops;
    int add_mop(MbKind kind, const std::string& wname, int64_t wnumel, const std::string& bn, int Cin, int Cout, int stride, int act) {
        MbOp o{kind, add_param(wname, wnumel), add_bn(bn, Cout), Cin, Cout, stride, act, 0, 0, 0};
        o.scale_off = alloc(Cout); o.shift_off = alloc(Cout);
        mops.push_back(o);
        return (int)mops.size() - 1;
    }
    struct Dec {
        int lat[4];
        int seg[7];
        int p_gn[7];
        int p_head_w, p_head_b;
        int head_ch, head_chp;
    } dec[4];

    Act a_img4, a_stem, a_pool;
    Act a_feat[4];
    Act a_p[4][4];
    Act a_seg[4][7];
    Act a_up[4][3];
    size_t gn_part_off[4][7], gn_aff_off[4][7];
    int gn_P[7];
    Act a_low[4];
    Act a_lsum[4];
    int up4_wide = 1;
    int merge_split = -1;
    size_t splitk_off = 0, splitk_floats = 0;
    size_t se_gate_off = 0, se_part_off = 0;
    int use_graph = 0;
    long long wino_blocks = 0;
    int wino_pack = 1;
    int wino_orient = 1;
    std::vector<char> c_tr;
    int split_precision = 0;
    hipGraphExec_t graph_exec = nullptr;
    size_t zeros_off = 0;
    size_t tickets_off = 0;

    bool h3_packed = false;
    hipStream_t load_stream = nullptr;
    size_t stem_h3_off = 0;
    bool fold_ok = false;
    size_t fold_wc_off[4] = {}, fold_img1_off[4] = {}, fold_img2_off[4] = {}, fold_tab_off[4] = {};

    std::vector<ConvPlan> cplan;
    std::vector<float> tune_score;
    unsigned* survey = nullptr;
    std::vector<ConvPlan> free_plan;
    std::vector<char> has_free;
    std::vector<char> guarded;
    std::vector<int> c_howo, c_groups;

    size_t bump = 0;
    size_t alloc(size_t n) { size_t o = bump; bump += (n + 63) / 64 * 64; return o; }
    Act alloc_act(int h, int w, int c) { Act a; a.H = h; a.W = w; a.C = c; a.off = alloc((size_t)B * h * w * c); return a; }
    int add_param(const std::string& n, int64_t numel) { pnames.push_back(n); pnumel.push_back(numel); return (int)pnames.size() - 1; }
    int add_bn(const std::string& p, int C) {
        add_param(p + ".weight", C); add_param(p + ".bias", C); add_param(p + ".running_mean", C);
        return add_param(p + ".running_var", C) - 3;
    }

    int add_conv(const std::string& wname, int Cin, int Cout, int k, int stride, int pad, const char* bn_prefix,
                 const char* bias_name, int Cinp = 0, int Kwp = 0) {
        PackedConv c;
        c.Cin = Cin; c.Cinp = Cinp ? Cinp : Cin; c.Cout = Cout; c.Kh = c.Kw = k; c.stride = stride; c.pad = pad;
        c.Kwp = Kwp ? Kwp : k;
        c.K = c.Cinp * k * c.Kwp; c.Kpad = cdiv(c.K, kConvBK) * kConvBK; c.Npad = cdiv(Cout, kConvNAlign) * kConvNAlign;
        c.p_w = add_param(wname, (int64_t)Cout * Cin * k * k);
        if (bn_prefix) c.p_bn = add_bn(bn_prefix, Cout);
        if (bias_name) c.p_bias = add_param(bias_name, Cout);
        c.w_off = alloc(conv_packed_floats(c.Npad, c.Kpad));
        if (bn_prefix) { c.scale_off = alloc(Cout); c.shift_off = alloc(Cout); }
        c.wino_ok = (k == 3 && stride == 1 && pad == 1 && c.Cinp == Cin && Cin % 8 == 0 && Cout % 64 == 0);
        if (c.wino_ok) c.wino_off = alloc(wino_region_floats(kImgH3, Cout, Cin, Cout % 128 == 0));
        convs.push_back(c);
        return (int)convs.size() - 1;
    }
    int add_grouped_conv(const std::string& wname, int C, int cg, int stride, const char* bn_prefix) {
        PackedConv c;
        c.Cin = c.Cinp = c.Cout = C; c.Kh = c.Kw = c.Kwp = 3; c.stride = stride; c.pad = 1; c.cg = cg;
        c.K = cg * 9; c.Kpad = cdiv(c.K, kConvBK) * kConvBK; c.Npad = cdiv(C, kConvNAlign) * kConvNAlign;
        c.p_w = add_param(wname, (int64_t)C * cg * 9);
        c.p_bn = add_bn(bn_prefix, C);
        c.grp_off = alloc((size_t)C * cg * 9);
        c.scale_off = alloc(C); c.shift_off = alloc(C);
        convs.push_back(c);
        return (int)convs.size() - 1;
    }
};

inline int lateral_mode(const PackedConv& c) { return c.Cin % kConvBK == 0 ? 0 : 2; }
```

### fastposecnn_amd/csrc/wino_h3.hip

```cpp
#include <algorithm>
#ifdef FPC_STAMP_WINO
#include <cstdlib>
#endif
#include <type_traits>
#include "wino_tile.hpp"

namespace fpc {
using namespace wino_tile;

namespace {

constexpr int kRing = 4;
static_assert(kLdsFloats >= kRing * kInFloats, "the K loop's input ring lives in the output image's space");

__device__ __forceinline__ const float* sgpr_ptr(const float* p) {
    const unsigned long long v = reinterpret_cast<unsigned long long>(p);
    const unsigned lo = __builtin_amdgcn_readfirstlane((unsigned)v), hi = __builtin_amdgcn_readfirstlane((unsigned)(v >> 32));
    return reinterpret_cast<const float*>(((unsigned long long)hi << 32) | lo);
}

}

template <int VAR, bool FOLD, bool PACK, bool TR = false>
__global__ __launch_bounds__(256, 1) void k_conv_wino_h3(const WinoArgs a) {
    __shared__ __attribute__((aligned(16))) float lds[kLdsFloats];
    long long* const dbg = kWinoStamp ? a.dbg : nullptr;
    const long long t_entry = dbg ? clock64() : 0;
    const int t = threadIdx.x, lane = t & 63;
    const int wi = __builtin_amdgcn_readfirstlane(t >> 6);
    const int li = lane & 31, lh = lane >> 5;
    const int H = a.H, W = a.W, Cout = a.Cout;
    const int nnb = Cout / kBN;
    const WinoPatch pt = wino_patch<PACK>(blockIdx.x, nnb, a.groups, a.tbx, a.tby, a.pack, W, a.B, a.dec);
    const int nb = pt.nb, grp = pt.grp, pk_ks = pt.pk_ks;
    const ConvPtrs P = wino_group(a.p[0], a.p[1], a.p[2], a.p[3], grp);
    const int y_in0 = 2 * pt.ty0 - 1, x_in0 = 2 * pt.tx0 - 1;
    const bool fine = kWinoStamp && dbg && a.variant == kWinoSerialStamps;
    long long t_dec = fine ? clock64() : 0, t_wld = 0, t_plan = 0, t_zero = 0;

    f32x16 acc[4][2][2];
    float inv_s = 1.f;
    long long t_issued = 0, t_landed = 0, t_synced = 0, c_begin = 0, r_begin = 0;
    const bool stamp = dbg != nullptr;

    auto kloop = [&](auto ph, const float* src, const float* wimg, const int Cs, const int up) __attribute__((always_inline)) {
    constexpr int PH = decltype(ph)::value;
    constexpr bool SKIPC = PH == 1;
    const int nkb = Cs >> 3;
    const int npair = nkb >> 1;
    const __amdgpu_buffer_rsrc_t rs_w = make_rsrc(reinterpret_cast<const char*>(wimg) + (size_t)nb * npair * kPairBytes);
    inv_s = wimg[(size_t)nnb * npair * (kPairBytes / 4)];
    const int vo_u = lane * 16;
    int so_u = wi * 4 * 4096;
    u32x4 U1[4][2], U2[4][2];
#define FPC_H3_XI_LIVE(J) (!(SKIPC && (J) == 2))
#define FPC_H3_LOAD_U1_AT(SO, J, NT) do { if (FPC_H3_XI_LIVE(J)) U1[J][NT] = __builtin_bit_cast(u32x4, __builtin_amdgcn_raw_buffer_load_b128(rs_w, vo_u, (SO) + (J) * 4096 + (NT) * 2048, 0)); } while (0)
#define FPC_H3_LOAD_U2_AT(SO, J, NT) do { if (FPC_H3_XI_LIVE(J)) U2[J][NT] = __builtin_bit_cast(u32x4, __builtin_amdgcn_raw_buffer_load_b128(rs_w, vo_u, (SO) + (J) * 4096 + (NT) * 2048 + 1024, 0)); } while (0)
#define FPC_H3_LOAD_U1(J, NT) FPC_H3_LOAD_U1_AT(so_u, J, NT)
#define FPC_H3_LOAD_U2(J, NT) FPC_H3_LOAD_U2_AT(so_u, J, NT)
#pragma unroll
    for (int j = 0; j < 4; ++j)
#pragma unroll
        for (int nt = 0; nt < 2; ++nt) { FPC_H3_LOAD_U1(j, nt); FPC_H3_LOAD_U2(j, nt); }
    if (npair > 1) so_u += kPairBytes;
    if (PH == 0) t_wld = fine ? clock64() : 0;

    const float* isb = sgpr_ptr(src + (size_t)pt.b * (H >> up) * (W >> up) * Cs);
    unsigned ivo[5];
    unsigned long long imask[5];
    wino_stage_plan<PACK, TR>(ivo, imask, wi, lane, y_in0, x_in0, H, W, Cs, up, pk_ks, pt.pk_two);
#define FPC_H3_ISSUE_IN(BUF, PTR) wino_issue_in(lds + (BUF) * kInFloats, wi, ivo, imask, PTR)
    int in_a[2], in_b[2];
    const float sgn = wino_frag<PACK>(in_a, in_b, wi, li, lh, pk_ks);
    if (PH == 0) t_plan = fine ? clock64() : 0;
    wino_zero_ring(lds, t, kRing, y_in0, x_in0, H, W, PACK && pk_ks < kTX);
    if (PH == 0) t_zero = fine ? clock64() : 0;
    FPC_H3_ISSUE_IN(0, isb);
    isb += 8;
    FPC_H3_ISSUE_IN(1, isb);
    isb += 8;
    FPC_H3_ISSUE_IN(2, nkb > 2 ? isb : isb - 8);
    isb += 8;
    int sn = 3;
#pragma unroll
    for (int j = 0; j < 4; ++j)
#pragma unroll
        for (int mt = 0; mt < 2; ++mt)
#pragma unroll
            for (int nt = 0; nt < 2; ++nt)
#pragma unroll
                for (int r = 0; r < 16; ++r)
                    if (PH == 0) acc[j][mt][nt][r] = 0.f;

    t_issued = stamp ? clock64() : 0;
    asm volatile("s_waitcnt vmcnt(10)" ::: "memory");
    t_landed = stamp ? clock64() : 0;
    __syncthreads();
    t_synced = stamp ? clock64() : 0;

    u32x4 TA1[4][2], TA2[4][2];
    f32x4 vn[2][4];
    float m1;
    asm volatile("s_mov_b32 %0, 0xbf800000" : "=s"(m1));
#define FPC_H3_SPLIT_PAIR(J, MT, PAIR, HALF) FPC_H3_SPLIT_PAIR_V(vn, J, MT, PAIR, HALF)
#define FPC_H3_SPLIT_PAIR_V(V, J, MT, PAIR, HALF)                                                             \
    if (FPC_H3_XI_LIVE(J)) do {                                                                               \
        const float x0_ = V[MT][J][2 * (PAIR)], x1_ = V[MT][J][2 * (PAIR) + 1];                               \
        const fp16x2 h_ = __builtin_amdgcn_cvt_pkrtz(x0_, x1_);                                               \
                                                          \
        const float r0_ = VAR == 1 ? x0_ - (float)h_[0] : __builtin_fmaf((float)h_[0], m1, x0_);              \
        const float r1_ = VAR == 1 ? x1_ - (float)h_[1] : __builtin_fmaf((float)h_[1], m1, x1_);              \
        const unsigned k1_ = __builtin_bit_cast(unsigned, h_);                                                \
        const unsigned k2_ = __builtin_bit_cast(unsigned, __builtin_amdgcn_cvt_pkrtz(r0_, r1_));              \
        asm volatile("" :: "v"(k1_), "v"(k2_));                                                               \
        TA1[J][MT][2 * (HALF) + (PAIR)] = k1_; TA2[J][MT][2 * (HALF) + (PAIR)] = k2_;                         \
    } while (0)
#pragma unroll
    for (int j = 0; j < 4; ++j)
#pragma unroll
        for (int mt = 0; mt < 2; ++mt) { TA1[j][mt] = u32x4{0u, 0u, 0u, 0u}; TA2[j][mt] = u32x4{0u, 0u, 0u, 0u}; }
    {
#pragma unroll
        for (int mt = 0; mt < 2; ++mt) {
            f32x4 e[4];
#pragma unroll
            for (int c = 0; c < 4; ++c)
                e[c] = fma_s4(sgn, *reinterpret_cast<const f32x4*>(lds + in_b[c >> 1] + (c & 1) * in_cs + mt * in_ms),
                              *reinterpret_cast<const f32x4*>(lds + in_a[c >> 1] + (c & 1) * in_cs + mt * in_ms));
            vn[mt][0] = sub_s4(e[0], e[2]); vn[mt][1] = add_s4(e[1], e[2]); vn[mt][2] = sub_s4(e[2], e[1]); vn[mt][3] = sub_s4(e[1], e[3]);
#pragma unroll
            for (int j = 0; j < 3; ++j) { FPC_H3_SPLIT_PAIR(j, mt, 0, 0); FPC_H3_SPLIT_PAIR(j, mt, 1, 0); }
        }
    }
    asm volatile("s_waitcnt vmcnt(0)" ::: "memory");
    __syncthreads();

#define FPC_H3_MFMA(J, MT, NT, A, B) do { if (FPC_H3_XI_LIVE(J)) acc[J][MT][NT] = __builtin_amdgcn_mfma_f32_32x32x16_f16(__builtin_bit_cast(f16x8, A), __builtin_bit_cast(f16x8, B), acc[J][MT][NT], 0, 0, 0); } while (0)
#define FPC_H3_PIN4(V) asm volatile("" :: "v"(V))
#define FPC_H3_SPLIT_Q(J, Q, HALF) do { if ((Q) == 0) FPC_H3_SPLIT_PAIR(J, 0, 0, HALF); if ((Q) == 1) FPC_H3_SPLIT_PAIR(J, 0, 1, HALF); if ((Q) == 2) FPC_H3_SPLIT_PAIR(J, 1, 0, HALF); if ((Q) == 3) FPC_H3_SPLIT_PAIR(J, 1, 1, HALF); } while (0)
    c_begin = stamp ? clock64() : 0; r_begin = stamp ? wall_clock64() : 0;
#pragma unroll 1
    for (int p = 0; p < npair; ++p) {
        {
            const float* InE = lds + ((2 * p + 1) & 3) * kInFloats;
            f32x4 ea[2][4], eb[2][4];
#pragma unroll
            for (int mt = 0; mt < 2; ++mt)
#pragma unroll
                for (int c = 0; c < 4; ++c) {
                    ea[mt][c] = *reinterpret_cast<const f32x4*>(InE + in_a[c >> 1] + (c & 1) * in_cs + mt * in_ms);
                    eb[mt][c] = *reinterpret_cast<const f32x4*>(InE + in_b[c >> 1] + (c & 1) * in_cs + mt * in_ms);
                }
            __builtin_amdgcn_sched_barrier(0);
            if (sn < nkb) { FPC_H3_ISSUE_IN((sn & 3), isb); isb += 8; }
            if (sn + 1 < nkb) { FPC_H3_ISSUE_IN(((sn + 1) & 3), isb); isb += 8; }
            sn += 2;
#pragma unroll
            for (int q = 0; q < 4; ++q) FPC_H3_SPLIT_Q(3, q, 0);
            __builtin_amdgcn_sched_barrier(0);
#pragma unroll
            for (int mt = 0; mt < 2; ++mt) {
                f32x4 e[4];
#pragma unroll
                for (int c = 0; c < 4; ++c) e[c] = fma_s4(sgn, eb[mt][c], ea[mt][c]);
                vn[mt][0] = sub_s4(e[0], e[2]); vn[mt][1] = add_s4(e[1], e[2]); vn[mt][2] = sub_s4(e[2], e[1]); vn[mt][3] = sub_s4(e[1], e[3]);
                FPC_H3_SPLIT_PAIR(0, mt, 0, 1); FPC_H3_SPLIT_PAIR(0, mt, 1, 1);
            }
        }
        __builtin_amdgcn_sched_barrier(0);
        const float* In = lds + ((2 * p + 2) & 3) * kInFloats;
        f32x4 da[2][4], db[2][4], e[2][4];
        __builtin_amdgcn_s_setprio(1);
#pragma unroll
        for (int j = 0; j < 4; ++j)
#pragma unroll
            for (int g = 0; g < 3; ++g)
#pragma unroll
                for (int mt = 0; mt < 2; ++mt)
#pragma unroll
                    for (int nt = 0; nt < 2; ++nt) {
                        const int sl = 12 * j + 4 * g + 2 * mt + nt;
                        if (g == 0) FPC_H3_MFMA(j, mt, nt, TA1[j][mt], U1[j][nt]);
                        if (g == 1) {
                            FPC_H3_MFMA(j, mt, nt, TA2[j][mt], U1[j][nt]);
                            if (mt == 1) FPC_H3_LOAD_U1(j, nt);
                        }
                        if (g == 2) {
                            FPC_H3_MFMA(j, mt, nt, TA1[j][mt], U2[j][nt]);
                            if (mt == 1) FPC_H3_LOAD_U2(j, nt);
                        }
                        if (sl < 4) {
#pragma unroll
                            for (int c = 2 * (sl & 1); c < 2 * (sl & 1) + 2; ++c) {
                                da[sl >> 1][c] = *reinterpret_cast<const f32x4*>(In + in_a[c >> 1] + (c & 1) * in_cs + (sl >> 1) * in_ms);
                                db[sl >> 1][c] = *reinterpret_cast<const f32x4*>(In + in_b[c >> 1] + (c & 1) * in_cs + (sl >> 1) * in_ms);
                            }
                        }
                        if (sl >= 4 && sl < 12) {
                            const int m_ = (sl - 4) >> 2, c = (sl - 4) & 3;
                            e[m_][c] = fma_s4(sgn, db[m_][c], da[m_][c]);
                            FPC_H3_PIN4(e[m_][c]);
                        }
                        if (sl < 4) FPC_H3_SPLIT_Q(1, sl, 1);
                        if (sl >= 4 && sl < 8) FPC_H3_SPLIT_Q(2, sl - 4, 1);
                        if (sl >= 8 && sl < 12) FPC_H3_SPLIT_Q(3, sl - 8, 1);
                        if (sl >= 12 && sl < 20 && !(SKIPC && ((sl - 12) & 3) == 2)) {
                            const int m_ = (sl - 12) >> 2, jx = (sl - 12) & 3;
                            if (jx == 0) vn[m_][0] = sub_s4(e[m_][0], e[m_][2]);
                            if (jx == 1) vn[m_][1] = add_s4(e[m_][1], e[m_][2]);
                            if (jx == 2) vn[m_][2] = sub_s4(e[m_][2], e[m_][1]);
                            if (jx == 3) vn[m_][3] = sub_s4(e[m_][1], e[m_][3]);
                            FPC_H3_PIN4(vn[m_][jx]);
                        }
                        if (sl >= 20 && sl < 24) FPC_H3_SPLIT_Q(0, sl - 20, 0);
                        if (sl >= 24 && sl < 28) FPC_H3_SPLIT_Q(1, sl - 24, 0);
                        if (sl >= 36 && sl < 40) FPC_H3_SPLIT_Q(2, sl - 36, 0);
                        __builtin_amdgcn_sched_barrier(0);
                    }
        __builtin_amdgcn_s_setprio(0);
        so_u += p + 2 < npair ? kPairBytes : 0;
        if (PH == 0) asm volatile("s_waitcnt vmcnt(16)" ::: "memory");
        if (PH == 1) asm volatile("s_waitcnt vmcnt(12)" ::: "memory");
        __syncthreads();
    }
#undef FPC_H3_MFMA
#undef FPC_H3_SPLIT_PAIR
#undef FPC_H3_SPLIT_PAIR_V
#undef FPC_H3_SPLIT_Q
#undef FPC_H3_PIN4
#undef FPC_H3_ISSUE_IN
#undef FPC_H3_LOAD_U1
#undef FPC_H3_LOAD_U2
#undef FPC_H3_LOAD_U1_AT
#undef FPC_H3_LOAD_U2_AT
#undef FPC_H3_XI_LIVE
    };

    if (!FOLD) {
        kloop(std::integral_constant<int, 0>(), P.in, P.w, a.Cin, 0);
    } else {
        kloop(std::integral_constant<int, 0>(), P.in, P.w, a.Cin, 0);
        kloop(std::integral_constant<int, 1>(), wino_group(a.in2[0], a.in2[1], a.in2[2], a.in2[3], grp), wino_group(a.w2[0], a.w2[1], a.w2[2], a.w2[3], grp), a.Cin2, 1);
    }
    const long long t_kend = dbg ? clock64() : 0;
    if (!(FOLD && PACK) && dbg && lane == 0) {
        long long* o = dbg + ((size_t)blockIdx.x * 4 + wi) * 8;
        o[0] = t_issued - t_entry; o[1] = t_landed - t_issued; o[2] = t_synced - t_landed;
        o[3] = t_kend - c_begin; o[4] = wall_clock64() - r_begin; o[5] = a.Cin >> 3; o[6] = c_begin - t_entry;
    }
    long long* const fdbg = (!(FOLD && PACK) && fine) ? dbg + (size_t)gridDim.x * 32 + ((size_t)blockIdx.x * 4 + wi) * 16 : nullptr;
    if (fdbg && lane == 0) { fdbg[0] = t_dec - t_entry; fdbg[1] = t_wld - t_entry; fdbg[2] = t_plan - t_entry; fdbg[3] = t_zero - t_entry; fdbg[4] = t_issued - t_entry; }
    wino_output<PACK, FOLD, TR>(lds, acc, P, pt, WinoEpi{H, W, Cout, a.relu, a.tbx, a.tby, a.pack_rx}, inv_s,
                            wino_group(a.btab[0], a.btab[1], a.btab[2], a.btab[3], grp), dbg, t_kend, t, wi, fdbg);
}

WinoPackGeom wino_pack_geometry(int H, int W, int B, int Cin, bool allow) {
    WinoPackGeom q;
    const int tcw = cdiv(W, 2), tch = cdiv(H, 2);
    q.G = 1;
    q.tby = cdiv(tch, kTY);
    if (allow && tcw >= kTX && 2LL * H * W * Cin * (long long)sizeof(float) < (1LL << 32)) {
        int best = cdiv(tcw, kTX);
        for (int g = 2; g <= std::min(B, 8); ++g)
            if ((long long)cdiv(g * tcw, kTX) * q.G < (long long)best * g) { best = cdiv(g * tcw, kTX); q.G = g; }
    }
    q.tbx = cdiv(q.G * tcw, kTX);
    q.rx = 1;
    for (int f = 0; f < q.G; ++f) q.rx = std::max(q.rx, (f * tcw + tcw - 1) / kTX - (f * tcw) / kTX + 1);
    q.patches = (long long)q.tby * ((long long)(B / q.G) * q.tbx + cdiv((B % q.G) * tcw, kTX));
    q.slots = q.patches * kNT;
    q.tiles = (long long)B * tch * tcw;
    q.gn_rows = q.tby * q.rx;
    return q;
}

static int wino_fold_check(const WinoArgs& a, int groups) {
    if (a.Cin2 % 16 != 0 || (a.H | a.W) & 1 || (long long)(a.H / 2) * (a.W / 2) * a.Cin2 * (long long)sizeof(float) >= (1LL << 32) ||
        (long long)(a.Cin2 >> 4) * kPairBytes >= (1LL << 31) || a.relu || a.dbg)
        return FPC_EINVAL;
    for (int g = 0; g < groups; ++g)
        if (!a.in2[g] || !a.w2[g] || !a.btab[g] || a.p[g].scale || a.p[g].shift || a.p[g].res || a.p[g].up) return FPC_EINVAL;
    return 0;
}

bool wino_orient_rule(int H, int W) {
    const int tcw = cdiv(W, 2), tch = cdiv(H, 2);
    return tcw % kTX == 0 && tch % kTY != 0 && tch >= kTY;
}

WinoPackGeom wino_launch_geometry(int H, int W, int B, int Cin, bool orient, bool pack_allow, bool* transposed) {
#ifdef FPC_STAMP_WINO
    static const bool g1 = getenv("FPC_H3_ORIENT_G1") && atoi(getenv("FPC_H3_ORIENT_G1")) != 0;
#else
    constexpr bool g1 = false;
#endif
    *transposed = orient && wino_orient_rule(H, W);
    return *transposed ? wino_pack_geometry(W, H, B, Cin, !g1) : wino_pack_geometry(H, W, B, Cin, pack_allow);
}

int launch_conv_wino_h3(const WinoArgs& a_in, int groups, hipStream_t s) {
    long long nblk;
    if (a_in.orient) {
        const WinoArgs& a = a_in;
        WinoArgs t = a;
        std::swap(t.H, t.W);
        if (a.pack < 1 || a.dbg) return FPC_EINVAL;
        if (const int rc = wino_tile_check(t, groups, 16, kPairBytes, true, &nblk)) return rc;
        t.dec = wino_decode(t.Cout, groups, t.tbx, t.tby, t.W, t.B, t.pack);
        if (a.fold) {
            if (const int rc = wino_fold_check(a, groups)) return rc;
            hipLaunchKernelGGL((k_conv_wino_h3<0, true, true, true>), dim3((unsigned)nblk), dim3(256), 0, s, t);
        } else {
            hipLaunchKernelGGL((k_conv_wino_h3<0, false, true, true>), dim3((unsigned)nblk), dim3(256), 0, s, t);
        }
        return check_launch();
    }
    if (const int rc = wino_tile_check(a_in, groups, 16, kPairBytes, a_in.pack > 1, &nblk)) return rc;
    WinoArgs a = a_in;
    a.dec = wino_decode(a.Cout, groups, a.tbx, a.tby, a.W, a.B, a.pack > 1 ? a.pack : 0);
    if (a.pack > 1) {
        hipLaunchKernelGGL((k_conv_wino_h3<0, false, true>), dim3((unsigned)nblk), dim3(256), 0, s, a);
        return check_launch();
    }
    if (a.fold) {
        if (const int rc = wino_fold_check(a, groups)) return rc;
        hipLaunchKernelGGL((k_conv_wino_h3<0, true, false>), dim3((unsigned)nblk), dim3(256), 0, s, a);
        return check_launch();
    }
#ifdef FPC_STAMP_WINO
    static const int var = getenv("FPC_H3_VAR") ? atoi(getenv("FPC_H3_VAR")) : 0;
    static const bool serial = getenv("FPC_WINO_SERIAL") && atoi(getenv("FPC_WINO_SERIAL")) != 0;
    if (serial && a.dbg) a.variant = kWinoSerialStamps;
    if (var == 1) hipLaunchKernelGGL((k_conv_wino_h3<1, false, false>), dim3((unsigned)nblk), dim3(256), 0, s, a);
    else
#endif
    hipLaunchKernelGGL((k_conv_wino_h3<0, false, false>), dim3((unsigned)nblk), dim3(256), 0, s, a);
    return check_launch();
}

__global__ __launch_bounds__(256) void k_fold_compose(const float* __restrict__ w, const float* __restrict__ l, const float* __restrict__ bias,
                                                      float* __restrict__ wc, float* __restrict__ btab, int Cout, int Cmid, int Cin, int tr) {
    const int g = blockIdx.x * blockDim.x + threadIdx.x;
    const int nw = Cout * Cin * 9;
    if (g < nw) {
        const int tap = g % 9, k = (g / 9) % Cin, o = g / (9 * Cin);
        double acc = 0.0;
        for (int c = 0; c < Cmid; ++c) acc += (double)w[((size_t)o * Cmid + c) * 9 + tap] * (double)l[(size_t)c * Cin + k];
        wc[g] = (float)acc;
    } else if (g < nw + 16 * Cout) {
        const int o = (g - nw) % Cout, cls = (g - nw) / Cout, rc = cls >> 2, cc = cls & 3;
        double acc = 0.0;
        for (int ky = (rc & 1); ky < 3 - ((rc >> 1) & 1); ++ky)
            for (int kx = (cc & 1); kx < 3 - ((cc >> 1) & 1); ++kx)
                for (int c = 0; c < Cmid; ++c) acc += (double)w[((size_t)o * Cmid + c) * 9 + (tr ? kx * 3 + ky : ky * 3 + kx)] * (double)bias[c];
        btab[(size_t)cls * Cout + o] = (float)acc;
    }
}

int launch_fold_compose(const float* W, const float* L, const float* bias, float* wc, float* btab, int Cout, int Cmid, int Cin,
                        bool transpose, hipStream_t s) {
    if (!W || !L || !bias || !wc || !btab || Cout < 1 || Cmid < 1 || Cin < 1) return FPC_EINVAL;
    const long long work = (long long)Cout * Cin * 9 + 16LL * Cout;
    hipLaunchKernelGGL(k_fold_compose, dim3((unsigned)((work + 255) / 256)), dim3(256), 0, s, W, L, bias, wc, btab, Cout, Cmid, Cin, transpose ? 1 : 0);
    return check_launch();
}

int launch_wino_pack_h3_pair(const float* w1, float* packed1, int Cin1, const float* w2, float* packed2, int Cin2, int Cout, bool transpose,
                             hipStream_t s) {
    if (Cin2 % 16 != 0 || ((uintptr_t)w2 & 15)) return FPC_EINVAL;
    const int rc = launch_wino_pack_fp16(w1, packed1, Cout, Cin1, true, w2, Cin2, transpose, s);
    return rc ? rc : launch_wino_pack_fp16(w2, packed2, Cout, Cin2, true, w1, Cin1, transpose, s);
}

int launch_wino_pack_h3(const float* w_oihw, float* packed, int Cout, int Cin, bool transpose, hipStream_t s) {
    return launch_wino_pack_fp16(w_oihw, packed, Cout, Cin, true, nullptr, 0, transpose, s);
}

}
```

### fastposecnn_amd/csrc/wino_tile.hpp

```cpp
#pragma once
#include <algorithm>
#include "net_kernels.hpp"

namespace fpc {
namespace wino_tile {

typedef float f32x16 __attribute__((ext_vector_type(16)));
typedef unsigned u32x4 __attribute__((ext_vector_type(4)));
typedef _Float16 f16x8 __attribute__((ext_vector_type(8)));
typedef __fp16 fp16x2 __attribute__((ext_vector_type(2)));

constexpr int kTX = 8, kTY = 8;
constexpr int kRW = 2 * kTX + 2, kRH = 2 * kTY + 2;
constexpr int kBN = 64;
constexpr int kNT = kTX * kTY;
constexpr int kInPieces = 18;
constexpr int kInFloats = kInPieces * 256;
constexpr int kPairBytes = 16 * 2 * 2 * 64 * 16;
constexpr int kZOdd = 64 * 1024 + 128;
constexpr int z_run(int cc, int mt, int r, int nt) { return ((((cc * 2 + mt) * 8 + (r >> 1)) * 2 + nt) * 4) * 256 + (r & 1) * kZOdd; }
constexpr int kZOddM0 = 64704;
constexpr int kZM0Slack = 65535 - 3 * 256 - kZOddM0;
static_assert(z_run(1, 1, 15, 1) - kZOddM0 < 65536 && z_run(0, 0, 1, 0) >= kZOddM0 && kZM0Slack >= 0, "ds_write_addtid_b32's reach");
constexpr int kLdsFloats = 4 * 2 * kNT * kBN + 32;
static_assert(z_run(1, 1, 15, 1) + 3 * 256 + 256 == kLdsFloats * 4, "the last run ends the image");

__device__ __forceinline__ __amdgpu_buffer_rsrc_t make_rsrc(const void* base) {
    return __builtin_amdgcn_make_buffer_rsrc(const_cast<void*>(base), 0, 0x7FFFFFFF, 0x00020000);
}
__device__ __forceinline__ f32x4 fma_s4(float s, f32x4 b, f32x4 a) {
    return f32x4{__builtin_fmaf(s, b[0], a[0]), __builtin_fmaf(s, b[1], a[1]), __builtin_fmaf(s, b[2], a[2]), __builtin_fmaf(s, b[3], a[3])};
}
__device__ __forceinline__ f32x4 sub_s4(f32x4 a, f32x4 b) { return f32x4{a[0] - b[0], a[1] - b[1], a[2] - b[2], a[3] - b[3]}; }
__device__ __forceinline__ f32x4 add_s4(f32x4 a, f32x4 b) { return f32x4{a[0] + b[0], a[1] + b[1], a[2] + b[2], a[3] + b[3]}; }

__device__ __forceinline__ unsigned lds_addr(const void* p) { return (unsigned)(size_t)(__attribute__((address_space(3))) const void*)p; }

struct WinoPatch {
    int nb, grp, bx, by, b, tx0, ty0;
    int pk_ks, pk_raw, pk_slot;
    bool pk_two;
};
__device__ __forceinline__ int wino_div(int n, const WinoRecip r) { return (int)(((unsigned long long)(unsigned)n * r.m) >> r.sh); }
template <bool PACK>
__device__ __forceinline__ WinoPatch wino_patch(int bid, int nnb, int groups, int tbx, int tby, int pack, int W, int B, const WinoDecode dc) {
    WinoPatch q;
    q.pk_ks = 99; q.pk_raw = 99; q.pk_slot = 0; q.pk_two = false;
    int up = wino_div(bid, dc.nnb);
    q.nb = bid - up * nnb; bid = up;
    up = wino_div(bid, dc.groups);
    q.grp = bid - up * groups; bid = up;
    if constexpr (!PACK) {
        up = wino_div(bid, dc.tbx);
        q.bx = bid - up * tbx; bid = up;
        q.b = wino_div(bid, dc.tby);
        q.by = bid - q.b * tby;
        q.tx0 = q.bx * kTX;
    } else {
        const int G = pack, tcw = (W + 1) >> 1, per = tbx * tby;
        const int g = wino_div(bid, dc.per), rem = bid - g * per;
        const int nf = min(G, B - g * G);
        const int tbxg = min(tbx, (nf * tcw + kTX - 1) / kTX);
        q.by = wino_div(rem, tbxg == tbx ? dc.tbx : dc.tbxl); q.bx = rem - q.by * tbxg;
        const int f = wino_div(kTX * q.bx, dc.tcw);
        q.tx0 = kTX * q.bx - f * tcw;
        q.b = g * G + f;
        q.pk_raw = tcw - q.tx0;
        q.pk_ks = q.pk_raw < kTX ? q.pk_raw : 99;
        q.pk_two = q.pk_ks < kTX && f + 1 < nf;
        q.pk_slot = q.bx - (f * tcw) / kTX;
    }
    q.ty0 = q.by * kTY;
    return q;
}
template <class T>
__device__ __forceinline__ T wino_group(const T v0, const T v1, const T v2, const T v3, int grp) {
    T r = v0;
    if (grp == 1) r = v1;
    if (grp == 2) r = v2;
    if (grp == 3) r = v3;
    return r;
}

template <bool PACK, bool TR = false>
__device__ __forceinline__ void wino_stage_plan(unsigned (&ivo)[5], unsigned long long (&imask)[5], int wi, int lane, int y_in0, int x_in0, int H,
                                                int W, int Cs, int up, int pk_ks, bool pk_two) {
    const int Hs = H >> up, Ws = W >> up;
#pragma unroll
    for (int i = 0; i < 5; ++i) {
        const int slot = (wi + 4 * i) * 64 + lane;
        const int blk = slot >> 4, res = slot & 15, cell = blk >> 3;
        const int ah = (cell / 3) * 4 + (res & 3), qh = (cell % 3) * 4 + (res >> 2);
        const int hf = blk & 1;
        const int ry = 2 * ah + ((blk >> 2) & 1), rx = 2 * qh + ((blk >> 1) & 1);
        const bool far = PACK && qh > pk_ks;
        const int y = y_in0 + ry, x = far ? rx - 2 * pk_ks - 3 : x_in0 + rx;
        const int qmax = (PACK && pk_ks < kTX) ? kTX + 1 : kTX;
        const bool iok = wi + 4 * i < kInPieces && ah <= kTY && qh <= qmax && y >= 0 && y < H && x >= 0 && x < W && (!far || pk_two);
        const size_t px = TR ? (size_t)(x >> up) * Hs + (y >> up) : (size_t)(y >> up) * Ws + (x >> up);
        ivo[i] = iok ? (unsigned)((px * Cs + 4 * hf) * sizeof(float)) +
                              (far ? (unsigned)((size_t)Hs * Ws * Cs * sizeof(float)) : 0u)
                        : 0u;
        imask[i] = __ballot(iok);
    }
}
#pragma clang diagnostic push
#pragma clang diagnostic ignored "-Winline-asm"
__device__ __forceinline__ void wino_issue_in(const float* buf, int wi, const unsigned (&ivo)[5], const unsigned long long (&imask)[5], const float* src) {
    unsigned long long sv_;
    const unsigned l0_ = lds_addr(buf + wi * 256);
    asm volatile("s_mov_b64 %0, exec\n"
                 "s_mov_b64 exec, %1\n s_mov_b32 m0, %6\n s_nop 0\n global_load_lds_dwordx4 %11, %16\n"
                 "s_mov_b64 exec, %2\n s_mov_b32 m0, %7\n s_nop 0\n global_load_lds_dwordx4 %12, %16\n"
                 "s_mov_b64 exec, %3\n s_mov_b32 m0, %8\n s_nop 0\n global_load_lds_dwordx4 %13, %16\n"
                 "s_mov_b64 exec, %4\n s_mov_b32 m0, %9\n s_nop 0\n global_load_lds_dwordx4 %14, %16\n"
                 "s_mov_b64 exec, %5\n s_mov_b32 m0, %10\n s_nop 0\n global_load_lds_dwordx4 %15, %16\n"
                 "s_mov_b64 exec, %0\n"
                 : "=&s"(sv_)
                 : "s"(imask[0]), "s"(imask[1]), "s"(imask[2]), "s"(imask[3]), "s"(imask[4]),
                   "s"(l0_), "s"(l0_ + 4096), "s"(l0_ + 8192), "s"(l0_ + 12288), "s"(l0_ + 16384),
                   "v"(ivo[0]), "v"(ivo[1]), "v"(ivo[2]), "v"(ivo[3]), "v"(ivo[4]), "s"(src)
                 : "memory", "m0");
}
#pragma clang diagnostic pop

constexpr int in_cs = 2 * 16 * 4;
constexpr int in_ms = 3 * 8 * 16 * 4;
template <bool PACK>
__device__ __forceinline__ float wino_frag(int (&in_a)[2], int (&in_b)[2], int wi, int li, int lh, int pk_ks) {
    const int tyl = li >> 3, txl = (li & 7) + ((PACK && (li & 7) >= pk_ks) ? 1 : 0);
    const int ra = (wi == 0) ? 0 : (wi == 2 ? 2 : 1);
    const int rb = (wi == 0) ? 2 : (wi == 1 ? 2 : (wi == 2 ? 1 : 3));
    auto unit = [&](int r, int ch) {
        const int ah = tyl + (r >> 1), qh = txl + ch;
        return ((((ah >> 2) * 3 + (qh >> 2)) * 8 + (r & 1) * 4 + lh) * 16 + 4 * (qh & 3) + (ah & 3)) * 4;
    };
    in_a[0] = unit(ra, 0); in_a[1] = unit(ra, 1);
    in_b[0] = unit(rb, 0); in_b[1] = unit(rb, 1);
    return (wi == 1) ? 1.f : -1.f;
}
__device__ __forceinline__ void wino_zero_ring(float* lds, int t, int nbuf, int y_in0, int x_in0, int H, int W, bool seam) {
    if (y_in0 < 0 || x_in0 < 0 || y_in0 + kRH > H || x_in0 + kRW > W || seam) {
        for (int i = t; i < nbuf * kInFloats / 4; i += 256) reinterpret_cast<f32x4*>(lds)[i] = f32x4{0.f, 0.f, 0.f, 0.f};
        asm volatile("s_waitcnt lgkmcnt(0)" ::: "memory");
        __syncthreads();
    }
}

struct WinoEpi { int H, W, Cout, relu, tbx, tby, pack_rx; };
#pragma clang diagnostic push
#pragma clang diagnostic ignored "-Winline-asm"
template <bool PACK, bool FOLD, bool TR = false>
__device__ __forceinline__ void wino_output(float* lds, const f32x16 (&acc)[4][2][2], const ConvPtrs P, const WinoPatch pt, const WinoEpi e,
                                            const float inv_s, const float* btab, long long* dbg, const long long t_kend, const int t,
                                            const int wi, long long* fdbg = nullptr) {
    const int H = e.H, W = e.W, Cout = e.Cout, HW = H * W;
    const int lane = PACK ? (int)__builtin_amdgcn_mbcnt_hi(~0u, __builtin_amdgcn_mbcnt_lo(~0u, 0u)) : t & 63;
    const int t_e = PACK ? wi * 64 + lane : t;
    const int oq = t_e & 15, otl = t_e >> 4;
    const bool o_far = PACK && (otl & 7) >= pt.pk_ks;
    const int ob = o_far ? pt.b + 1 : pt.b, otx = o_far ? (otl & 7) - pt.pk_ks : pt.tx0 + (otl & 7);
    const bool o_ok = !o_far || pt.pk_two;
    const int n = pt.nb * kBN + oq * 4;
    const f32x4 e_sc = (!FOLD && P.scale) ? *reinterpret_cast<const f32x4*>(P.scale + n) : f32x4{1.f, 1.f, 1.f, 1.f};
    const f32x4 e_sh = (!FOLD && P.shift) ? *reinterpret_cast<const f32x4*>(P.shift + n) : f32x4{0.f, 0.f, 0.f, 0.f};
    f32x4 e_res[4][4];
#pragma unroll
    for (int tp = 0; tp < 4; ++tp)
#pragma unroll
        for (int q = 0; q < 4; ++q) {
            const int ot = otl + 16 * tp;
            const int y = 2 * (pt.ty0 + (ot >> 3)) + (q >> 1), x = 2 * otx + (q & 1);
            e_res[tp][q] = (!FOLD && P.res && o_ok && y < H && x < W) ? *reinterpret_cast<const f32x4*>(P.res + ((size_t)ob * HW + (TR ? (size_t)x * H + y : (size_t)y * W + x)) * Cout + n)
                                                             : f32x4{0.f, 0.f, 0.f, 0.f};
        }
    __syncthreads();
    if (kWinoStamp && fdbg && (t & 63) == 0) fdbg[8] = clock64() - t_kend;
    {
        const unsigned zm0 = lds_addr(lds) + wi * 256;
#pragma unroll
        for (int mt = 0; mt < 2; ++mt)
#pragma unroll
            for (int nt = 0; nt < 2; ++nt)
#pragma unroll
                for (int cc = 0; cc < 2; ++cc)
#pragma unroll
                    for (int odd = 0; odd < 2; ++odd) {
                        float z[8];
#pragma unroll
                        for (int h = 0; h < 8; ++h) {
                            const int r = 2 * h + odd;
                            const float m0 = acc[0][mt][nt][r], m1 = acc[1][mt][nt][r], m2 = acc[2][mt][nt][r], m3 = acc[3][mt][nt][r];
                            z[h] = cc == 0 ? m0 + m1 + m2 : m1 - m2 - m3;
                        }
#define FPC_Z_IMM(H) "i"(z_run(cc, mt, 2 * (H) + odd, nt) - odd * kZOddM0)
                        asm volatile("s_mov_b32 m0, %8\n s_nop 0\n"
                                     "ds_write_addtid_b32 %0 offset:%9\n ds_write_addtid_b32 %1 offset:%10\n"
                                     "ds_write_addtid_b32 %2 offset:%11\n ds_write_addtid_b32 %3 offset:%12\n"
                                     "ds_write_addtid_b32 %4 offset:%13\n ds_write_addtid_b32 %5 offset:%14\n"
                                     "ds_write_addtid_b32 %6 offset:%15\n ds_write_addtid_b32 %7 offset:%16\n"
                                     :: "v"(z[0]), "v"(z[1]), "v"(z[2]), "v"(z[3]), "v"(z[4]), "v"(z[5]), "v"(z[6]), "v"(z[7]),
                                        "s"(zm0 + odd * kZOddM0), FPC_Z_IMM(0), FPC_Z_IMM(1), FPC_Z_IMM(2), FPC_Z_IMM(3), FPC_Z_IMM(4),
                                        FPC_Z_IMM(5), FPC_Z_IMM(6), FPC_Z_IMM(7)
                                     : "memory", "m0");
#undef FPC_Z_IMM
                    }
        asm volatile("s_waitcnt lgkmcnt(0)" ::: "memory");
    }
    if (kWinoStamp && fdbg && (t & 63) == 0) fdbg[9] = clock64() - t_kend;
    __syncthreads();
    if (kWinoStamp && fdbg && (t & 63) == 0) fdbg[10] = clock64() - t_kend;
    f32x4 s1 = {0.f, 0.f, 0.f, 0.f}, s2 = {0.f, 0.f, 0.f, 0.f};
    const float* const zr = lds + z_run(0, 0, (otl & 3) + 4 * (otl >> 3), oq >> 3) / 4 +
                            ((otl >> 2) & 1) * 32 + (oq & 7) * 4;
#pragma unroll
    for (int tp = 0; tp < 4; ++tp) {
        const int ot = otl + 16 * tp;
        const int oty = pt.ty0 + (ot >> 3);
        f32x4 z[4][2];
#pragma unroll
        for (int i = 0; i < 4; ++i)
#pragma unroll
            for (int cc = 0; cc < 2; ++cc) z[i][cc] = *reinterpret_cast<const f32x4*>(zr + (z_run(cc, tp >> 1, 8 * (tp & 1), 0) + 256 * i) / 4);
#pragma unroll
        for (int rr = 0; rr < 2; ++rr)
#pragma unroll
            for (int cc = 0; cc < 2; ++cc) {
                const int y = 2 * oty + rr, x = 2 * otx + cc;
                if (y >= H || x >= W || !o_ok) continue;
                f32x4 val = (rr == 0 ? z[0][cc] + z[1][cc] + z[2][cc] : z[1][cc] - z[2][cc] - z[3][cc]) * inv_s;
                if (FOLD) {
                    const int cls = (((y == 0) | ((y == H - 1) << 1)) << 2) | (x == 0) | ((x == W - 1) << 1);
                    val += *reinterpret_cast<const f32x4*>(btab + (size_t)cls * Cout + n);
                }
                if (!FOLD && P.scale) val = val * e_sc;
                val = val + e_sh;
                const size_t o = ((size_t)ob * HW + (TR ? (size_t)x * H + y : (size_t)y * W + x)) * Cout + n;
                if (!FOLD && P.res) val += e_res[tp][2 * rr + cc];
                if (!FOLD && e.relu) { val[0] = fmaxf(val[0], 0.f); val[1] = fmaxf(val[1], 0.f); val[2] = fmaxf(val[2], 0.f); val[3] = fmaxf(val[3], 0.f); }
                *reinterpret_cast<f32x4*>(P.out + o) = val;
                s1 += val;
                s2 += val * val;
            }
    }
    if (kWinoStamp && fdbg && (t & 63) == 0) fdbg[11] = clock64() - t_kend;
    if (PACK && P.gn_part) {
        f32x4 q1[2] = {o_far ? f32x4{0.f, 0.f, 0.f, 0.f} : s1, o_far ? s1 : f32x4{0.f, 0.f, 0.f, 0.f}};
        f32x4 q2[2] = {o_far ? f32x4{0.f, 0.f, 0.f, 0.f} : s2, o_far ? s2 : f32x4{0.f, 0.f, 0.f, 0.f}};
#pragma unroll
        for (int sd = 0; sd < 2; ++sd)
#pragma unroll
            for (int o = 16; o < 64; o <<= 1)
#pragma unroll
                for (int k = 0; k < 4; ++k) { q1[sd][k] += __shfl_xor(q1[sd][k], o, 64); q2[sd][k] += __shfl_xor(q2[sd][k], o, 64); }
        __syncthreads();
        float* red = lds;
        if (lane < 16) {
#pragma unroll
            for (int sd = 0; sd < 2; ++sd)
#pragma unroll
                for (int k = 0; k < 4; ++k) {
                    red[((sd * 4 + wi) * kBN + oq * 4 + k) * 2] = q1[sd][k];
                    red[((sd * 4 + wi) * kBN + oq * 4 + k) * 2 + 1] = q2[sd][k];
                }
        }
        __syncthreads();
        if (t_e < 2 * kBN && (t_e < kBN || pt.pk_two)) {
            const int sd = t_e >> 6, ch = t_e & (kBN - 1);
            float u1 = 0.f, u2 = 0.f;
#pragma unroll
            for (int w = 0; w < 4; ++w) { u1 += red[((sd * 4 + w) * kBN + ch) * 2]; u2 += red[((sd * 4 + w) * kBN + ch) * 2 + 1]; }
            const int rx = e.pack_rx, Pn = e.tby * rx, slot = sd ? 0 : pt.pk_slot;
            float* g = P.gn_part + (((size_t)(pt.b + sd) * Pn + pt.by * rx + slot) * Cout + pt.nb * kBN + ch) * 2;
            g[0] = u1; g[1] = u2;
            if (sd == 0 && pt.pk_raw <= kTX)
                for (int z = slot + 1; z < rx; ++z) { g += (size_t)Cout * 2; g[0] = 0.f; g[1] = 0.f; }
        }
    } else if (P.gn_part) {
#pragma unroll
        for (int o = 16; o < 64; o <<= 1)
#pragma unroll
            for (int k = 0; k < 4; ++k) { s1[k] += __shfl_xor(s1[k], o, 64); s2[k] += __shfl_xor(s2[k], o, 64); }
        __syncthreads();
        float* red = lds;
        if (lane < 16) {
#pragma unroll
            for (int k = 0; k < 4; ++k) { red[(wi * kBN + oq * 4 + k) * 2] = s1[k]; red[(wi * kBN + oq * 4 + k) * 2 + 1] = s2[k]; }
        }
        __syncthreads();
        if (t_e < kBN) {
            float u1 = 0.f, u2 = 0.f;
#pragma unroll
            for (int w = 0; w < 4; ++w) { u1 += red[(w * kBN + t_e) * 2]; u2 += red[(w * kBN + t_e) * 2 + 1]; }
            const int Pn = e.tbx * e.tby;
            float* g = P.gn_part + (((size_t)pt.b * Pn + pt.by * e.tbx + pt.bx) * Cout + pt.nb * kBN + t_e) * 2;
            g[0] = u1; g[1] = u2;
        }
    }
    if (kWinoStamp && fdbg && lane == 0) fdbg[12] = clock64() - t_kend;
    if (kWinoStamp && dbg && lane == 0) {
        asm volatile("s_waitcnt vmcnt(0)" ::: "memory");
        dbg[((size_t)blockIdx.x * 4 + wi) * 8 + 7] = clock64() - t_kend;
    }
}
#pragma clang diagnostic pop

inline int wino_tile_check(const WinoArgs& a, int groups, int kch, int step_bytes, bool packed, long long* nblk) {
    if (groups < 1 || groups > kMaxGroup || a.Cin % kch != 0 || a.Cout % kBN != 0 || (!kWinoStamp && a.dbg)) return FPC_EINVAL;
    if ((long long)a.H * a.W * a.Cin * (long long)sizeof(float) >= (1LL << 32)) return FPC_EINVAL;
    if ((long long)(a.Cin / kch) * step_bytes >= (1LL << 31)) return FPC_EINVAL;
    if (packed) {
        const WinoPackGeom q = wino_pack_geometry(a.H, a.W, a.B, a.Cin, a.orient ? a.pack > 1 : !a.fold);
        if (q.G != a.pack || q.tbx != a.tbx || q.tby != a.tby || q.rx != a.pack_rx) return FPC_EINVAL;
        *nblk = q.patches * (a.Cout / kBN) * groups;
    } else {
        if (a.tbx != cdiv(cdiv(a.W, 2), kTX) || a.tby != cdiv(cdiv(a.H, 2), kTY)) return FPC_EINVAL;
        *nblk = (long long)a.tbx * a.tby * a.B * (a.Cout / kBN) * groups;
    }
    return (*nblk < 1 || *nblk >= (1LL << 31)) ? FPC_EINVAL : 0;
}
}

int launch_wino_pack_fp16(const float* w_oihw, float* packed, int Cout, int Cin, bool pair, const float* w_also, int Cin_also, bool transpose,
                          hipStream_t s);

}
```

### fastposecnn_amd/engine.py

```python
import ctypes
import operator

import torch

from fastposecnn_amd import _native as nat


_DATA_PTR = torch.Tensor.data_ptr
_VERSION = operator.attrgetter('_version')

class NetEngine:

    def __init__(self, model, B, H, W, device, autotune=True, tune_mode=0, graph=False, split_precision=False):
        L = nat.lib()
        self._lib = L
        self.B, self.H, self.W, self.device = B, H, W, device
        self.classes = model.classes
        h = ctypes.c_void_p()
        from fastposecnn_amd.lib import backbone
        name = model.encoder.name
        mobilenet = backbone.encoder_family(name) == "mobilenet_v2"
        block, layers = (0, [0] * 4) if mobilenet else backbone.encoder_layout(name)
        groups, width = (1, 64) if mobilenet else backbone.encoder_groups(name)
        reduction = 0 if mobilenet else backbone.encoder_reduction(name)
        arr, tail = (ctypes.c_int * 4)(*layers), (self.classes, B, H, W, ctypes.byref(h))
        if mobilenet:
            nat.check(L.fpc_net_create(name.encode(), *tail), "fpc_net_create")
        elif reduction:
            nat.check(L.fpc_net_create_encoder_se(arr, reduction, *tail), "fpc_net_create_encoder_se")
        elif groups > 1:
            nat.check(L.fpc_net_create_encoder_ex(block, arr, groups, width, *tail), "fpc_net_create_encoder_ex")
        elif block == 1:
            nat.check(L.fpc_net_create(name.encode(), *tail), "fpc_net_create")
        else:
            nat.check(L.fpc_net_create_encoder(block, arr, *tail), "fpc_net_create_encoder")
        self._h = h
        self._names = [L.fpc_net_param_name(h, i).decode() for i in range(L.fpc_net_param_count(h))]
        nbytes = L.fpc_net_workspace_bytes(h)
        with torch.cuda.device(device):
            self._ws = torch.empty(nbytes, dtype=torch.uint8, device=device)
            assert self._ws.data_ptr() % 256 == 0
        self.reloads = 0
        self.generation = 0
        self.guard_forwards = 0
        self.bind(model)
        if split_precision:
            nat.check(L.fpc_net_set_split_precision(h, int(split_precision)), "fpc_net_set_split_precision")
        if autotune:
            nat.check(L.fpc_net_autotune_next(h, int(tune_mode)), "fpc_net_autotune_next")
            self.forward(torch.zeros((B, 3, H, W), dtype=torch.float32, device=device), want_logits=False)
        if graph:
            nat.check(L.fpc_net_set_graph(h, 1), "fpc_net_set_graph")

    def bind(self, model):
        L, h, device = self._lib, self._h, self.device
        tensors = dict(model.named_parameters())
        tensors.update(dict(model.named_buffers()))
        params = []
        for i, name in enumerate(self._names):
            if name not in tensors:
                raise RuntimeError(f"fastposecnn_amd: the model has no parameter {name!r} (smp naming expected)")
            t = tensors[name]
            if t.device != device or t.dtype != torch.float32 or not t.is_contiguous():
                raise RuntimeError(f"fastposecnn_amd: parameter {name!r} must be a contiguous f32 tensor on {device}")
            if t.numel() != L.fpc_net_param_numel(h, i):
                raise RuntimeError(f"fastposecnn_amd: parameter {name!r} has {t.numel()} elements, expected "
                                   f"{L.fpc_net_param_numel(h, i)}")
            params.append(t)
        self._params = params
        n = len(params)
        ptrs = (ctypes.c_void_p * n)(*[t.data_ptr() for t in params])
        with torch.cuda.device(device):
            nat.check(L.fpc_net_load_params(h, ptrs, n, self._ws.data_ptr(), self._ws.numel(), nat.stream()),
                      "fpc_net_load_params")
        self._stamp = self._fingerprint()
        self.reloads += 1

    def _fingerprint(self):
        return (tuple(map(_DATA_PTR, self._params)), tuple(map(_VERSION, self._params)))

    def stale(self):
        return self._fingerprint() != self._stamp

    def conv_plans(self):
        out = []
        buf = (ctypes.c_int * 5)()
        for i in range(self._lib.fpc_net_conv_count(self._h)):
            self._lib.fpc_net_conv_plan(self._h, i, buf)
            out.append(tuple(buf))
        return out

    def copy_plans_from(self, other):
        nat.check(self._lib.fpc_net_copy_plans(self._h, other._h), "fpc_net_copy_plans")

    def force_winograd(self, form):
        rc = self._lib.fpc_net_force_winograd(self._h, int(form))
        if rc < 0:
            nat.check(rc, "fpc_net_force_winograd")
        return rc

    def force_fold(self, on):
        rc = self._lib.fpc_net_force_fold(self._h, int(on))
        if rc < 0:
            nat.check(rc, "fpc_net_force_fold")
        return rc

    def force_direct_h3(self, on):
        rc = self._lib.fpc_net_force_direct_h3(self._h, int(on))
        if rc < 0:
            nat.check(rc, "fpc_net_force_direct_h3")
        return rc

    def force_stem_pool(self, on):
        rc = self._lib.fpc_net_force_stem_pool(self._h, int(on))
        if rc < 0:
            nat.check(rc, "fpc_net_force_stem_pool")
        return rc

    def survey(self, x, want_logits=True):
        if tuple(x.shape) != (self.B, 3, self.H, self.W) or x.device != self.device:
            raise RuntimeError("NetEngine.survey: input shape / device does not match the plan")
        sites = self._lib.fpc_net_conv_count(self._h)
        with torch.cuda.device(self.device):
            rec = torch.zeros((sites, 4), dtype=torch.int32, device=self.device)
            nat.check(self._lib.fpc_net_survey_next(self._h, rec.data_ptr(), sites), "fpc_net_survey_next")
        try:
            logits, cat = self.forward(x, want_logits=want_logits)
        finally:
            self._lib.fpc_net_survey_next(self._h, None, sites)
        return logits, cat, rec.cpu().to(torch.int64) & 0xFFFFFFFF

    @staticmethod
    def record_max(records):
        return (records[:, 0] & 0xFFFFFFFF).to(torch.int32).view(torch.float32) if records.dtype == torch.int64 \
            else records[:, 0].contiguous().view(torch.float32)

    def guard_ranges(self, records, lo=2.0 ** -2, hi=2.0 ** 14):
        sites = self._lib.fpc_net_conv_count(self._h)
        flat = [int(v) & 0xFFFFFFFF for v in records.reshape(-1).tolist()]
        if len(flat) != 4 * sites:
            raise RuntimeError("NetEngine.guard_ranges: records must be [sites, 4]")
        before = set(self.guarded())
        rc = self._lib.fpc_net_guard_ranges(self._h, (ctypes.c_uint32 * len(flat))(*flat), sites, float(lo), float(hi))
        if rc < 0:
            nat.check(rc, "fpc_net_guard_ranges")
        return [i for i in self.guarded() if i not in before]

    def guarded(self):
        return [i for i in range(self._lib.fpc_net_conv_count(self._h)) if self._lib.fpc_net_guarded(self._h, i)]

    def graph_recorded(self):
        return bool(self._lib.fpc_net_graph_recorded(self._h))

    def set_wino_pack(self, on):
        nat.check(self._lib.fpc_net_set_wino_pack(self._h, int(on)), "fpc_net_set_wino_pack")

    def set_wino_orient(self, on):
        nat.check(self._lib.fpc_net_set_wino_orient(self._h, int(on)), "fpc_net_set_wino_orient")

    def wino_blocks(self):
        return int(self._lib.fpc_net_wino_blocks(self._h))

    def force_pointwise(self, on):
        rc = self._lib.fpc_net_force_pointwise(self._h, int(on))
        if rc < 0:
            nat.check(rc, "fpc_net_force_pointwise")
        return rc

    def flops(self):
        buf = (ctypes.c_double * 3)()
        nat.check(self._lib.fpc_net_flops(self._h, buf), "fpc_net_flops")
        return tuple(buf)

    def __del__(self):
        h = getattr(self, "_h", None)
        if h:
            self._lib.fpc_net_destroy(h)
            self._h = None

    def forward(self, x, want_logits=True):
        B, H, W, C, dev = self.B, self.H, self.W, self.classes, self.device
        G = C - 1
        if tuple(x.shape) != (B, 3, H, W) or x.device != dev:
            raise RuntimeError("NetEngine.forward: input shape / device does not match the plan")
        if x.dtype != torch.float32 or not x.is_contiguous():
            x = x.float().contiguous()
        f32 = dict(dtype=torch.float32, device=dev)
        logits = None
        lp = [None] * 5
        if want_logits:
            logits = {'mask': torch.empty((B, C, H, W), **f32), 'quaternion': torch.empty((B, 4 * G, H, W), **f32),
                      'scales': torch.empty((B, 3 * G, H, W), **f32), 'xy': torch.empty((B, 2 * G, H, W), **f32),
                      'z': torch.empty((B, G, H, W), **f32)}
            lp = [logits[k].data_ptr() for k in ('mask', 'quaternion', 'scales', 'xy', 'z')]
        cat = {'mask': torch.empty((B, H, W), dtype=torch.int64, device=dev),
               'quaternion': torch.empty((B, 4, H, W), **f32), 'scales': torch.empty((B, 3, H, W), **f32),
               'xy': torch.empty((B, 2, H, W), **f32), 'z': torch.empty((B, H, W), **f32)}
        bits = None
        if W % 64 == 0 and self._lib.fpc_cc_bits_supported(B, H, W):
            bits = torch.empty((B, self._lib.fpc_mask_bits_words(H, W)), dtype=torch.int64, device=dev)
        with torch.cuda.device(dev):
            nat.check(self._lib.fpc_net_forward_bits(self._h, x.data_ptr(), *lp, cat['mask'].data_ptr(),
                                                     cat['quaternion'].data_ptr(), cat['scales'].data_ptr(),
                                                     cat['xy'].data_ptr(), cat['z'].data_ptr(), nat.ptr(bits), nat.stream()),
                      "fpc_net_forward_bits")
        if bits is not None:
            cat['mask']._fpc_fg_bits = (bits, cat['mask']._version)
        return logits, cat

    def tensor(self, name):
        p = ctypes.c_void_p()
        H, W, C = ctypes.c_int(), ctypes.c_int(), ctypes.c_int()
        nat.check(self._lib.fpc_net_tensor(self._h, name.encode(), ctypes.byref(p), ctypes.byref(H), ctypes.byref(W),
                                           ctypes.byref(C)), "fpc_net_tensor")
        off = p.value - self._ws.data_ptr()
        n = self.B * H.value * W.value * C.value
        return self._ws[off:off + 4 * n].view(torch.float32).view(self.B, H.value, W.value, C.value)
```

### include/fpc.h

```cpp
#ifndef FPC_H_
#define FPC_H_

#include <stddef.h>
#include <stdint.h>

#ifdef __cplusplus
extern "C" {
#endif

#define FPC_ABI_VERSION 11

#define FPC_OK 0
#define FPC_EINVAL (-1)
#define FPC_EWORKSPACE (-2)
#define FPC_ELAUNCH (-3)
#define FPC_EDEVICE (-4)
#define FPC_EFORMAT (-5)

typedef void* fpc_stream_t;

int fpc_abi_version(void);
const char* fpc_error_string(int code);
const char* fpc_last_hip_error(void);

// ... 76 lines not shown
                       float* oq, float* os, float* oz, float* oxy, float* out_stats, uint64_t* inst_bits,
                       const int32_t* root_pix, void* ws, size_t ws_bytes, fpc_stream_t stream);

int fpc_pose_rt(const float* q, const float* xy, const float* z, const float* kinv, int n,
                float* R, float* T, float* RT, fpc_stream_t stream);

int fpc_pack_pose_records(const int64_t* sample_ids, const int64_t* class_ids, const float* q, const float* scales,
                          const float* xy, const float* z, const float* R, const float* T, const float* RT, int n,
                          int sample_offset, int capacity, float* out, fpc_stream_t stream);

size_t fpc_mask_iou_workspace_bytes(int n1, int n2, int64_t hw);
int fpc_mask_iou(const void* masks1, int n1, const void* masks2, int n2, int64_t hw, int elem_size,
                 float* iou, int32_t* inter, int32_t* uni, void* ws, size_t ws_bytes, fpc_stream_t stream);

size_t fpc_preprocess_workspace_bytes(int B);
int fpc_preprocess_u8(const uint8_t* img_hwc, int B, int H, int W, const double* mean3, const double* std3,
                      int input_range_01, float* out_nchw, void* ws, size_t ws_bytes, fpc_stream_t stream);

int fpc_png_info(const uint8_t* data, size_t nbytes, int32_t* out5);
int fpc_png_decode(const uint8_t* data, size_t nbytes, void* out, size_t out_bytes, int mode);
int fpc_png_decode_batch(const uint8_t* const* datas, const size_t* sizes, int n, uint8_t* out, int H, int W, int threads);

#define FPC_PNG_DESC_WORDS 8
#define FPC_INF_ETRUNCATED 1
#define FPC_INF_EBLOCK_TYPE 2
#define FPC_INF_ESTORED_LEN 3
#define FPC_INF_EOVERSUBSCRIBED 4
#define FPC_INF_EINCOMPLETE 5
#define FPC_INF_EREPEAT_FIRST 6
#define FPC_INF_ELITLEN_SYMBOL 7
#define FPC_INF_EDIST_SYMBOL 8
#define FPC_INF_EDIST_TOO_FAR 9
#define FPC_INF_EOUT_OVERFLOW 10
#define FPC_INF_EOUT_SHORT 11
#define FPC_INF_EADLER 12
#define FPC_INF_EFDICT 13
#define FPC_INF_EMETHOD 14
#define FPC_INF_EFCHECK 15
#define FPC_INF_ELENGTHS_OVERRUN 16
#define FPC_INF_ENO_END_CODE 17
#define FPC_INF_EBAD_CODE 18
#define FPC_PNG_EDESC 20
#define FPC_PNG_EFILTER 21
int fpc_inflate_host(const uint8_t* in, size_t zbytes, uint8_t* out, size_t cap, size_t* out_len);
size_t fpc_png_pack_bytes(int n, int H, int W);
int fpc_png_pack_batch(const uint8_t* const* datas, const size_t* sizes, int n, int H, int W, int mode, uint8_t* staging,
                       size_t staging_bytes, int64_t* desc, size_t* used);
size_t fpc_png_decode_device_workspace_bytes(int n, int H, int W, int max_bpp);
int fpc_png_decode_device(const uint8_t* staging, size_t staging_bytes, const int64_t* desc, int n, int H, int W, int mode,
                          int max_bpp, void* out, size_t frame_bytes, int32_t* status, void* workspace, size_t workspace_bytes,
                          fpc_stream_t stream);

int fpc_gt_build(const uint8_t* ids, int64_t pix_stride, int64_t frame_stride, int B, int H, int W,
                 const int16_t* row_of, const uint8_t* class_of, const int32_t* first_row, int n,
                 int64_t* class_mask, void* inst_masks, int mask_elem, int32_t* pix_count, fpc_stream_t stream);
int fpc_depth_decode(const void* src, int src_kind, int channels, int B, int H, int W, float* depth_f32, fpc_stream_t stream);

int fpc_pose_errors(const float* q0, const float* q1, const int64_t* symmetric_ids, const float* rot, int nrot,
                    const float* RT1, const float* RT2, const float* scales1, const float* scales2,
                    const float* T1, const float* T2, int n, double* out_degree, float* out_iou3d, float* out_offset,
                    fpc_stream_t stream);

size_t fpc_pose_metrics_state_words(int num_classes, int n_deg, int n_iou, int n_off, int n_complex);
int fpc_pose_metrics_update(const int32_t* order, const int32_t* match_pred, const int32_t* count, int n1, int n2,
                            const float* gt_quaternion, const float* gt_RT, const float* gt_scales, const float* gt_T,
                            const int64_t* symmetric_ids, const int64_t* class_ids, const float* quaternion, const float* RT,
                            const float* scales, const float* T, const float* rot, int nrot, const double* thr_degree, int n_deg,
                            const double* thr_iou, int n_iou, const double* thr_offset, int n_off, const double* thr_complex,
                            int n_complex, const double* thr_table, int num_classes, int64_t* state, double* raw_degree,
                            float* raw_iou, float* raw_offset, int32_t* raw_class, int raw_capacity, fpc_stream_t stream);

int fpc_confusion_update(const int64_t* pred, const int64_t* gt, int64_t n, int num_classes, int64_t* state, fpc_stream_t stream);

int fpc_post_network_backward(const int32_t* labels, const float* cat_xy, int B, int H, int W, int N,
                              const int32_t* n_dev, const double* table, float inlier_thresh, int max_num,
                              uint64_t seed, const uint8_t* keep, float* g_q, float* g_s, float* g_xy, float* g_z,
                              fpc_stream_t stream);
int fpc_vote_refine_backward(const float* mask, const float* vertex, int64_t vs_n, int64_t vs_h, int64_t vs_w,
                             int64_t vs_c, int n, int H, int W, const double* table, float inlier_thresh, int max_num,
                             uint64_t seed, const uint8_t* keep, float* g_vertex, fpc_stream_t stream);
int fpc_class_compress_backward(const int64_t* cat_mask, const float* quat, const float* xy, const float* go_q,
                                const float* go_s, const float* go_xy, const float* go_z, int B, int C, int HW,
                                float* g_q, float* g_s, float* g_xy, float* g_z, fpc_stream_t stream);
int fpc_mask_losses(const float* logits, const int64_t* target, int B, int C, int HW, int64_t ignore_ce,
                    int64_t ignore_cce, float alpha, float gamma, double* sums6, const float* w3, float* grad,
                    fpc_stream_t stream);
#define FPC_MATCH_MAX_INSTANCES 1024
int fpc_match_assign(const float* iou, const int64_t* gt_cls, const int64_t* pred_cls, int n1, int n2, int32_t* match_pred,
                     int32_t* order, int32_t* count, fpc_stream_t stream);
#define FPC_LOSS_L2 0
#define FPC_LOSS_L1 1
#define FPC_LOSS_SMOOTH_L1 2
int fpc_matched_losses(const int32_t* order, const int32_t* match_pred, const int32_t* count, int n1, int n2,
                       const float* gt_quaternion, const float* gt_xy, const float* gt_z, const float* gt_scales,
                       const int64_t* symmetric_ids, const float* quaternion, const float* xy, const float* z,
                       const float* scales, const float* rot, int nrot, double eps, int xy_type, int z_type, int scales_type,
                       const double* weights, double* losses, double* task_total, double* matched_total, int32_t* best_rot,
                       fpc_stream_t stream);
int fpc_matched_losses_backward(const int32_t* order, const int32_t* match_pred, const int32_t* count, int n1, int n2,
                                const float* gt_quaternion, const float* gt_xy, const float* gt_z, const float* gt_scales,
                                const int64_t* symmetric_ids, const float* quaternion, const float* xy, const float* z,
                                const float* scales, const float* rot, int nrot, double eps, int xy_type, int z_type,
                                int scales_type, const double* weights, const double* losses, const int32_t* best_rot,
                                const double* g_losses, float* g_quaternion, float* g_xy, float* g_z, float* g_scales,
                                fpc_stream_t stream);
int fpc_grad_sumsq(const float* g, size_t n, double* out2, fpc_stream_t stream);
int fpc_lookahead_radam_step(float* p, const float* g, float* m, float* v, float* slow, size_t n, float lr, float beta1,
                             float beta2, float eps, float weight_decay, int64_t step, int la_k, float la_alpha,
                             const float* ctl, fpc_stream_t stream);

typedef struct fpc_net fpc_net_t;
int fpc_net_create(const char* encoder, int classes, int B, int H, int W, fpc_net_t** out);
int fpc_net_create_encoder(int block, const int* layers4, int classes, int B, int H, int W, fpc_net_t** out);
int fpc_net_create_encoder_ex(int block, const int* layers4, int groups, int width_per_group, int classes, int B, int H, int W,
                              fpc_net_t** out);
int fpc_net_create_encoder_se(const int* layers4, int reduction, int classes, int B, int H, int W, fpc_net_t** out);
void fpc_net_destroy(fpc_net_t* net);
int fpc_net_param_count(const fpc_net_t* net);
const char* fpc_net_param_name(const fpc_net_t* net, int i);
int64_t fpc_net_param_numel(const fpc_net_t* net, int i);
size_t fpc_net_workspace_bytes(const fpc_net_t* net);
int fpc_net_load_params(fpc_net_t* net, const float* const* params, int count, void* ws, size_t ws_bytes,
                        fpc_stream_t stream);
int fpc_net_forward(fpc_net_t* net, const float* x, float* logits_mask, float* logits_quat,
                    float* logits_scales, float* logits_xy, float* logits_z, int64_t* cat_mask,
                    float* cq, float* cs, float* cxy, float* cz, fpc_stream_t stream);
int fpc_net_forward_bits(fpc_net_t* net, const float* x, float* logits_mask, float* logits_quat,
                         float* logits_scales, float* logits_xy, float* logits_z, int64_t* cat_mask,
                         float* cq, float* cs, float* cxy, float* cz, uint64_t* fg_bits, fpc_stream_t stream);

int fpc_net_autotune_next(fpc_net_t* net, int mode );
int fpc_net_set_split_precision(fpc_net_t* net, int on);
int fpc_net_set_graph(fpc_net_t* net, int on);
int fpc_net_graph_recorded(const fpc_net_t* net);
int fpc_net_conv_count(const fpc_net_t* net);
int fpc_net_conv_plan(const fpc_net_t* net, int i, int* out5);
int fpc_net_copy_plans(fpc_net_t* dst, const fpc_net_t* src);
int fpc_net_force_winograd(fpc_net_t* net, int form);
int fpc_net_force_pointwise(fpc_net_t* net, int on);
int fpc_net_force_fold(fpc_net_t* net, int on);
int fpc_net_force_direct_h3(fpc_net_t* net, int on);
int fpc_net_force_stem_pool(fpc_net_t* net, int on);
int fpc_act_range(const float* x, long long n, unsigned* rec4, fpc_stream_t stream);
int fpc_net_survey_next(fpc_net_t* net, unsigned* records_dev, int sites);
int fpc_net_guard_ranges(fpc_net_t* net, const unsigned* records_host, int sites, float lo, float hi);
int fpc_net_guarded(const fpc_net_t* net, int i);
int fpc_stem_pool_tasks(int Ho, int Wo, int64_t* out4);
int fpc_wino_pack_geometry(int H, int W, int B, int Cin, int fold, int64_t* out8);
int fpc_net_set_wino_pack(fpc_net_t* net, int on);
int fpc_net_set_wino_orient(fpc_net_t* net, int on);
int fpc_wino_orient_geometry(int H, int W, int B, int Cin, int fold, int pack, int64_t* out9);
int fpc_wino_recip(uint32_t d, int64_t* out2);
int fpc_wino_decode(int Cout, int groups, int tbx, int tby, int W, int B, int pack, int64_t* out14);
int64_t fpc_net_wino_blocks(const fpc_net_t* net);
int fpc_net_flops(const fpc_net_t* net, double* out3);
int fpc_net_tensor(const fpc_net_t* net, const char* name, const float** ptr, int* H, int* W, int* C);

enum {
    FPC_PLAN_WINO_ORIENT = -11, FPC_PLAN_WINO_PACKED = -10, FPC_PLAN_TWO_LAUNCH = 100, FPC_PLAN_BF3 = 1000, FPC_PLAN_LATERAL = 2000, FPC_PLAN_STEM = 3000,
    FPC_PLAN_STEM_POOL = 3100, FPC_PLAN_POINTWISE = 4000, FPC_PLAN_FOLDED = 5000, FPC_PLAN_H3 = 6000, FPC_PLAN_LATERAL_H3 = 7000,
    FPC_PLAN_GROUPED = 8000
};
size_t fpc_conv2d_workspace_bytes(int B, int Ho, int Wo, int Cin, int Cout, int Kh, int Kw);
size_t fpc_conv2d_workspace_bytes_for(int B, int Ho, int Wo, int Cin, int Cout, int Kh, int Kw, int bm, int bn, int nsplit);
int fpc_conv2d_plan(int B, int Ho, int Wo, int Cin, int Cout, int Kh, int Kw, int bm, int bn, int nsplit,
                    int* out4 );
int fpc_conv2d(const float* in, int64_t sb, int64_t sh, int64_t sw, int64_t sc, const float* w_oihw,
               const float* scale, const float* shift, const float* res, const float* up, float* out,
               float* gn_part, int B, int Hi, int Wi, int Cin, int Cout, int Kh, int Kw, int stride, int pad,
               int relu, int bm, int bn, int nsplit, void* ws, size_t ws_bytes, fpc_stream_t stream);

size_t fpc_conv2d_grouped_workspace_bytes(int C, int groups);
int fpc_conv2d_grouped(const float* in, int64_t sb, int64_t sh, int64_t sw, int64_t sc, const float* w_oihw, const float* scale,
                       const float* shift, float* out, int B, int Hi, int Wi, int C, int groups, int stride, int relu, int form,
                       void* ws, size_t ws_bytes, fpc_stream_t stream);

size_t fpc_conv2d_grouped_dgrad_workspace_bytes(int C, int groups);
int fpc_conv2d_grouped_dgrad(const float* dy, const float* w_oihw, float* dx, int B, int Hi, int Wi, int C, int groups, int stride,
                             void* ws, size_t ws_bytes, fpc_stream_t stream);
size_t fpc_conv2d_grouped_wgrad_workspace_bytes(int B, int Ho, int Wo, int C, int groups);
int fpc_conv2d_grouped_wgrad(const float* x, int64_t sb, int64_t sh, int64_t sw, const float* dy, float* dw, int B, int Hi, int Wi,
                             int C, int groups, int stride, void* ws, size_t ws_bytes, fpc_stream_t stream);

int fpc_image_nhwc4(const float* x, float* out, int B, int H, int W, fpc_stream_t stream);
size_t fpc_stem_wgrad_workspace_bytes(int B, int Hi, int Wi);
int fpc_stem_wgrad_slices(int B, int Hi, int Wi);
int fpc_stem_wgrad(const float* img4, const float* dy, float* dw, int B, int Hi, int Wi, void* ws, size_t ws_bytes,
                   fpc_stream_t stream);
int fpc_maxpool3x3s2_fwd(const float* x, float* y, int B, int Hi, int Wi, int C, fpc_stream_t stream);
int fpc_maxpool3x3s2_bwd(const float* x, const float* dy, float* dx, int B, int Hi, int Wi, int C, fpc_stream_t stream);

int fpc_se_pool_slabs(int H, int W, int C);
size_t fpc_se_scratch_floats(int B, int H, int W, int C);
int fpc_se_gate(const float* x, const float* w1, const float* b1, const float* w2, const float* b2, float* gate, float* scratch, int B,
                int H, int W, int C, int R, fpc_stream_t stream);
int fpc_se_scale_add_relu(const float* x, const float* gate, const float* res, float* y, int B, int H, int W, int C,
                          fpc_stream_t stream);
int fpc_maxpool3x3s2_ceil_fwd(const float* x, float* y, int B, int Hi, int Wi, int C, fpc_stream_t stream);

int fpc_dwconv3x3(const float* in, const float* w, const float* scale, const float* shift, float* out, int B, int Hi, int Wi, int C,
                  int stride, int act, fpc_stream_t stream);
int fpc_conv1x1_f32(const float* in, const float* w, const float* scale, const float* shift, const float* res, float* out, int64_t M,
                    int Cin, int Cout, int act, fpc_stream_t stream);
int fpc_conv1x1_f32_form(int64_t M, int Cin, int Cout);
int fpc_stem3x3s2(const float* in4, const float* w, const float* scale, const float* shift, float* out, int B, int Hi, int Wi, int Cout,
                  fpc_stream_t stream);

int fpc_dwconv3x3_dgrad(const float* dy, const float* w, float* dx, int B, int Hi, int Wi, int C, int stride, fpc_stream_t stream);
size_t fpc_dwconv3x3_wgrad_workspace_bytes(int B, int Ho, int Wo, int C);
int fpc_dwconv3x3_wgrad(const float* x, const float* dy, float* dw, int B, int Hi, int Wi, int C, int stride, void* ws,
                        size_t ws_bytes, fpc_stream_t stream);

int fpc_se_gate_train(const float* x, const float* w1, const float* b1, const float* w2, const float* b2, float* gate, float* mean,
                      float* hidden, float* scratch, int B, int H, int W, int C, int R, fpc_stream_t stream);
size_t fpc_se_bwd_scratch_floats(int B, int H, int W, int C, int R);
int fpc_se_bwd(const float* x, const float* y, const float* gy, const float* gate, const float* mean, const float* hidden,
               const float* w1, const float* w2, float* dx, float* dres, float* dw1, float* db1, float* dw2, float* db2, float* scratch,
               int B, int H, int W, int C, int R, fpc_stream_t stream);

size_t fpc_conv2d_wgrad_workspace_bytes(int B, int Ho, int Wo, int Cin, int Cout, int Kh, int Kw);
int fpc_conv2d_wgrad(const float* x, int64_t sb, int64_t sh, int64_t sw, const float* dy, float* dw, int B, int Hi,
                     int Wi, int Cin, int Cout, int Kh, int Kw, int stride, int pad, void* ws, size_t ws_bytes,
                     fpc_stream_t stream);
int fpc_conv2d_wgrad_split(const float* x, int64_t sb, int64_t sh, int64_t sw, const float* dy, float* dw, int B, int Hi,
                           int Wi, int Cin, int Cout, int Kh, int Kw, int stride, int pad, void* ws, size_t ws_bytes,
                           fpc_stream_t stream);

int fpc_upsample_bilinear_fwd(const float* in, int64_t sb, int64_t sc, int64_t sh, int64_t sw, float* out, int B, int C, int h,
                              int w, int scale, int out_nhwc, fpc_stream_t stream);
size_t fpc_upsample_bilinear_bwd_scratch_floats(int B, int C, int h, int w, int scale);
int fpc_upsample_bilinear_bwd(const float* dout, int64_t sb, int64_t sc, int64_t sh, int64_t sw, float* din, float* scratch,
                              int B, int C, int h, int w, int scale, int din_nhwc, fpc_stream_t stream);

size_t fpc_groupnorm4_relu_scratch_floats(int B, int HW, int C);
int fpc_groupnorm4_relu_fwd(const float* x, const float* gamma, const float* beta, float* y, float* stats, float* part, int B,
                            int HW, int C, int groups, float eps, fpc_stream_t stream);
int fpc_groupnorm4_relu_bwd(const float* x, const float* dy, const float* gamma, const float* beta, const float* stats, float* dx,
                            float* part, int B, int HW, int C, int groups, fpc_stream_t stream);

size_t fpc_batchnorm_scratch_floats(int P, int C);
int fpc_batchnorm_fwd(const float* x, const float* res, const float* gamma, const float* beta, float* running_mean,
                      float* running_var, float* y, float* stats, float* part, int P, int C, float eps, float momentum, int relu,
                      fpc_stream_t stream);
int fpc_batchnorm_bwd(const float* x, const float* y, const float* dy, const float* gamma, const float* stats, float* dx,
                      float* dres, float* dgamma, float* dbeta, float* part, int P, int C, int relu, fpc_stream_t stream);
int fpc_batchnorm_act_fwd(const float* x, const float* res, const float* gamma, const float* beta, float* running_mean,
                          float* running_var, float* y, float* stats, float* part, int P, int C, float eps, float momentum, int act,
                          fpc_stream_t stream);
int fpc_batchnorm_act_bwd(const float* x, const float* y, const float* dy, const float* gamma, const float* stats, float* dx,
                          float* dres, float* dgamma, float* dbeta, float* part, int P, int C, int act, fpc_stream_t stream);

#ifdef __cplusplus
}
#endif
#endif
```

Baseline: 2779.

## Share overlapping x-columns across Winograd tile fragments in packed h3 kernel

Adds an x-shared fragment map to the packed/transposed Winograd h3 convolution. Adjacent tiles reuse overlapping input columns, so each thread loads and transforms 6 input vectors per step instead of 8. This cuts LDS reads and FMAs in the inner loop. The output staging offsets are remapped to match. The path is enabled by default when the width rule holds, and the old row-split map stays selectable through new plan codes and a net setter.

```diff
diff --git a/fastposecnn_amd/_native.py b/fastposecnn_amd/_native.py
--- a/fastposecnn_amd/_native.py
+++ b/fastposecnn_amd/_native.py
@@ -104,6 +104,12 @@
     "fpc_net_set_wino_pack": (_i, [_vp, _i]),
     "fpc_net_set_wino_orient": (_i, [_vp, _i]),
     "fpc_wino_orient_geometry": (_i, [_i, _i, _i, _i, _i, _i, ctypes.POINTER(_i64)]),
+    "fpc_wino_xshare_rule": (_i, [_i]),
+    "fpc_net_set_wino_xshare": (_i, [_vp, _i]),
+    "fpc_wino_tile_frag": (_i, [_i, _i, _i, _i, ctypes.POINTER(_i64)]),
+    "fpc_wino_tile_slot": (_i, [_i] * 11 + [ctypes.POINTER(_i64)]),
+    "fpc_wino_tile_zrun": (_i, [_i, _i, _i, _i, _i, _i, ctypes.POINTER(_i64)]),
+    "fpc_wino_tile_zread": (_i, [_i, _i, _i, _i, _i, ctypes.POINTER(_i64)]),
     "fpc_wino_recip": (_i, [ctypes.c_uint32, ctypes.POINTER(_i64)]),
     "fpc_wino_decode": (_i, [_i, _i, _i, _i, _i, _i, _i, ctypes.POINTER(_i64)]),
     "fpc_net_wino_blocks": (_i64, [_vp]),
diff --git a/fastposecnn_amd/csrc/conv2d.hip b/fastposecnn_amd/csrc/conv2d.hip
--- a/fastposecnn_amd/csrc/conv2d.hip
+++ b/fastposecnn_amd/csrc/conv2d.hip
@@ -41,6 +41,33 @@
     const WinoDecode d = wino_decode(Cout, groups, tbx, tby, W, B, pack);
     const WinoRecip r[7] = {d.nnb, d.groups, d.tbx, d.tby, d.per, d.tbxl, d.tcw};
     for (int i = 0; i < 7; ++i) { out14[2 * i] = r[i].m; out14[2 * i + 1] = r[i].sh; }
+    return FPC_OK;
+}
+
+extern "C" int fpc_wino_xshare_rule(int W) { return W >= 1 && wino_xshare_rule(W) ? 1 : 0; }
+extern "C" int fpc_wino_tile_frag(int xshare, int wi, int lane, int pk_ks, int64_t* out17) {
+    long long o[17] = {0};
+    if (!out17 || wino_tile_frag(xshare != 0, wi, lane, pk_ks, o)) return FPC_EINVAL;
+    for (int i = 0; i < 17; ++i) out17[i] = o[i];
+    return FPC_OK;
+}
+extern "C" int fpc_wino_tile_slot(int xshare, int tr, int slot, int y_in0, int x_in0, int H, int W, int Cs, int up, int pk_ks, int pk_two,
+                                  int64_t* out6) {
+    long long o[6];
+    if (!out6 || wino_tile_slot(xshare != 0, tr != 0, slot, y_in0, x_in0, H, W, Cs, up, pk_ks, pk_two, o)) return FPC_EINVAL;
+    for (int i = 0; i < 6; ++i) out6[i] = o[i];
+    return FPC_OK;
+}
+extern "C" int fpc_wino_tile_zrun(int xshare, int wi, int mt, int r, int nt, int cc, int64_t* out3) {
+    long long o[3];
+    if (!out3 || wino_tile_zrun(xshare != 0, wi, mt, r, nt, cc, o)) return FPC_EINVAL;
+    for (int i = 0; i < 3; ++i) out3[i] = o[i];
+    return FPC_OK;
+}
+extern "C" int fpc_wino_tile_zread(int xshare, int t_e, int tp, int cc, int i, int64_t* out1) {
+    long long o[1];
+    if (!out1 || wino_tile_zread(xshare != 0, t_e, tp, cc, i, o)) return FPC_EINVAL;
+    out1[0] = o[0];
     return FPC_OK;
 }
 
@@ -137,6 +164,7 @@
     fill_conv_shape(a, B, c, p, Hi, Wi, Ho, Wo, sb, sh, sw, sc, relu != 0, mode);
     a.wino_pack = rq.pack ? 1 : 0;
     a.wino_orient = rq.orient ? 1 : 0;
+    a.wino_rowsplit = rq.rowsplit ? 1 : 0;
     a.splitk_ws = packed + lay.packed;
     a.p[0] = ConvPtrs{in, packed, out, scale, shift, res, up, gn_part};
     if (lay.tickets) {
diff --git a/fastposecnn_amd/csrc/conv_launch.hip b/fastposecnn_amd/csrc/conv_launch.hip
--- a/fastposecnn_amd/csrc/conv_launch.hip
+++ b/fastposecnn_amd/csrc/conv_launch.hip
@@ -81,6 +81,7 @@
             const WinoPackGeom q = wino_launch_geometry(a.Ho, a.Wo, a.B, a.Cin, a.wino_orient, a.wino_pack && !p.fold, &tr);
             if (q.G > 1 || tr) { w.pack = q.G; w.tbx = q.tbx; w.tby = q.tby; w.pack_rx = q.rx; }
             w.orient = tr ? 1 : 0;
+            w.xshare = ((q.G > 1 || tr) && !a.wino_rowsplit && wino_xshare_rule(tr ? a.Ho : a.Wo)) ? 1 : 0;
             a.wino_blocks = q.patches * (a.Cout / 64) * groups;
         }
         if (p.fold) {
diff --git a/fastposecnn_amd/csrc/conv_plan.hpp b/fastposecnn_amd/csrc/conv_plan.hpp
--- a/fastposecnn_amd/csrc/conv_plan.hpp
+++ b/fastposecnn_amd/csrc/conv_plan.hpp
@@ -182,9 +182,13 @@
 struct WinoGrid { int tbx, tby; int patches() const { return tbx * tby; } };
 inline WinoGrid wino_grid(int form, int H, int W) { return {cdiv(cdiv(W, 2), 8), cdiv(cdiv(H, 2), kWinoForms[form].waves)}; }
 
-struct Conv2dRequest { int nsplit; bool bf3, two_launch; int wino, lat; bool stem; int pw; bool h3, pool, pack, orient; int grp; };
+inline bool wino_xshare_rule(int W) { return (((W + 1) >> 1) & 1) == 0; }
+
+struct Conv2dRequest { int nsplit; bool bf3, two_launch; int wino, lat; bool stem; int pw; bool h3, pool, pack, orient; int grp; bool rowsplit; };
 inline Conv2dRequest decode_plan(int code) {
-    Conv2dRequest r{code, false, false, 0, 0, false, 0, false, false, false, false, 0};
+    Conv2dRequest r{code, false, false, 0, 0, false, 0, false, false, false, false, 0, false};
+    if (code == FPC_PLAN_WINO_PACKED_ROWSPLIT) { r.rowsplit = true; code = FPC_PLAN_WINO_PACKED; }
+    if (code == FPC_PLAN_WINO_ORIENT_ROWSPLIT) { r.rowsplit = true; code = FPC_PLAN_WINO_ORIENT; }
     if (code >= FPC_PLAN_GROUPED && code < FPC_PLAN_GROUPED + 1000) { r.grp = code - FPC_PLAN_GROUPED + 1; r.nsplit = 1; return r; }
     if (code == FPC_PLAN_WINO_ORIENT) { r.orient = true; r.nsplit = -kWinoH3; }
     if (code == FPC_PLAN_WINO_PACKED) { r.pack = true; r.nsplit = -kWinoH3; }
diff --git a/fastposecnn_amd/csrc/net.hip b/fastposecnn_amd/csrc/net.hip
--- a/fastposecnn_amd/csrc/net.hip
+++ b/fastposecnn_amd/csrc/net.hip
@@ -41,6 +41,13 @@
     if (!n || on < 0 || on > 1) return FPC_EINVAL;
     if (n->wino_pack != on) drop_graph(n);
     n->wino_pack = on;
+    return FPC_OK;
+}
+
+extern "C" int fpc_net_set_wino_xshare(fpc_net_t* n, int on) {
+    if (!n || on < 0 || on > 1) return FPC_EINVAL;
+    if (n->wino_xshare != on) drop_graph(n);
+    n->wino_xshare = on;
     return FPC_OK;
 }
 
@@ -161,7 +168,7 @@
                     int Wo, long long sb, long long sh, long long sw, long long sc, bool relu, int mode) {
     fill_conv_shape(a, n->B, c, p, Hi, Wi, Ho, Wo, sb, sh, sw, sc, relu, mode);
     a.splitk_ws = n->ws + n->splitk_off; a.zeros = n->ws + n->zeros_off; a.tickets = (int*)(n->ws + n->tickets_off);
-    a.wino_pack = n->wino_pack; a.wino_orient = n->wino_orient;
+    a.wino_pack = n->wino_pack; a.wino_orient = n->wino_orient; a.wino_rowsplit = n->wino_xshare ? 0 : 1;
 }
 
 
diff --git a/fastposecnn_amd/csrc/net_kernels.hpp b/fastposecnn_amd/csrc/net_kernels.hpp
--- a/fastposecnn_amd/csrc/net_kernels.hpp
+++ b/fastposecnn_amd/csrc/net_kernels.hpp
@@ -48,6 +48,7 @@
     long long wino_blocks;
     int wino_pack;
     int wino_orient;
+    int wino_rowsplit;
     int cg;
     const float* grp_w;
 };
@@ -213,6 +214,7 @@
     int fold, Cin2;
     int pack, pack_rx;
     int orient;
+    int xshare;
     WinoDecode dec;
 };
 int launch_conv_wino(const WinoArgs& a, int groups, hipStream_t s);
@@ -232,6 +234,10 @@
 bool wino_orient_rule(int H, int W);
 WinoPackGeom wino_launch_geometry(int H, int W, int B, int Cin, bool orient, bool pack_allow, bool* transposed);
 int launch_wino_pack_h3(const float* w_oihw, float* packed, int Cout, int Cin, bool transpose, hipStream_t s);
+int wino_tile_frag(bool xs, int wi, int lane, int pk_ks, long long* out17);
+int wino_tile_slot(bool xs, bool tr, int slot, int y_in0, int x_in0, int H, int W, int Cs, int up, int pk_ks, int pk_two, long long* out6);
+int wino_tile_zrun(bool xs, int wi, int mt, int r, int nt, int cc, long long* out3);
+int wino_tile_zread(bool xs, int t_e, int tp, int cc, int i, long long* out1);
 int launch_wino_pack_h3_pair(const float* w1, float* packed1, int Cin1, const float* w2, float* packed2, int Cin2, int Cout, bool transpose,
                              hipStream_t s);
 int launch_fold_compose(const float* W, const float* L, const float* bias, float* wc, float* btab, int Cout, int Cmid, int Cin,
diff --git a/fastposecnn_amd/csrc/net_plan.hpp b/fastposecnn_amd/csrc/net_plan.hpp
--- a/fastposecnn_amd/csrc/net_plan.hpp
+++ b/fastposecnn_amd/csrc/net_plan.hpp
@@ -106,6 +106,7 @@
     long long wino_blocks = 0;
     int wino_pack = 1;
     int wino_orient = 1;
+    int wino_xshare = 1;
     std::vector<char> c_tr;
     int split_precision = 0;
     hipGraphExec_t graph_exec = nullptr;
diff --git a/fastposecnn_amd/csrc/wino_h3.hip b/fastposecnn_amd/csrc/wino_h3.hip
--- a/fastposecnn_amd/csrc/wino_h3.hip
+++ b/fastposecnn_amd/csrc/wino_h3.hip
@@ -3,6 +3,7 @@
 #include <cstdlib>
 #endif
 #include <type_traits>
+#include "conv_plan.hpp"
 #include "wino_tile.hpp"
 
 namespace fpc {
@@ -21,8 +22,11 @@
 
 }
 
-template <int VAR, bool FOLD, bool PACK, bool TR = false>
+template <int VAR, bool FOLD, bool PACK, bool TR = false, bool XS = false>
 __global__ __launch_bounds__(256, 1) void k_conv_wino_h3(const WinoArgs a) {
+    static_assert(PACK || !XS, "the x-shared map needs the packed decode's even seams");
+    constexpr int kNC = XS ? 6 : 8;
+    constexpr int kNR = 2 * kNC / 4;
     __shared__ __attribute__((aligned(16))) float lds[kLdsFloats];
     long long* const dbg = kWinoStamp ? a.dbg : nullptr;
     const long long t_entry = dbg ? clock64() : 0;
@@ -68,10 +72,14 @@
     const float* isb = sgpr_ptr(src + (size_t)pt.b * (H >> up) * (W >> up) * Cs);
     unsigned ivo[5];
     unsigned long long imask[5];
-    wino_stage_plan<PACK, TR>(ivo, imask, wi, lane, y_in0, x_in0, H, W, Cs, up, pk_ks, pt.pk_two);
+    wino_stage_plan<PACK, TR, XS>(ivo, imask, wi, lane, y_in0, x_in0, H, W, Cs, up, pk_ks, pt.pk_two);
 #define FPC_H3_ISSUE_IN(BUF, PTR) wino_issue_in(lds + (BUF) * kInFloats, wi, ivo, imask, PTR)
     int in_a[2], in_b[2];
-    const float sgn = wino_frag<PACK>(in_a, in_b, wi, li, lh, pk_ks);
+    const float sgn = wino_frag<PACK, XS>(in_a, in_b, wi, li, lh, pk_ks);
+#define FPC_H3_FA(X) wino_frag_at<XS>(in_a, (X) >> 2, XS ? (X) : (X) & 3)
+#define FPC_H3_FB(X) wino_frag_at<XS>(in_b, (X) >> 2, XS ? (X) : (X) & 3)
+#define FPC_H3_COLUMN(E, MT, JX) ((JX) == 0 ? sub_s4(E[(MT) * (kNC - 4)], E[(MT) * (kNC - 4) + 2]) : (JX) == 1 ? add_s4(E[(MT) * (kNC - 4) + 1], E[(MT) * (kNC - 4) + 2]) : \
+                                  (JX) == 2 ? sub_s4(E[(MT) * (kNC - 4) + 2], E[(MT) * (kNC - 4) + 1]) : sub_s4(E[(MT) * (kNC - 4) + 1], E[(MT) * (kNC - 4) + 3]))
     if (PH == 0) t_plan = fine ? clock64() : 0;
     wino_zero_ring(lds, t, kRing, y_in0, x_in0, H, W, PACK && pk_ks < kTX);
     if (PH == 0) t_zero = fine ? clock64() : 0;
@@ -120,14 +128,14 @@
 #pragma unroll
         for (int mt = 0; mt < 2; ++mt) { TA1[j][mt] = u32x4{0u, 0u, 0u, 0u}; TA2[j][mt] = u32x4{0u, 0u, 0u, 0u}; }
     {
+        f32x4 e[kNC];
 #pragma unroll
         for (int mt = 0; mt < 2; ++mt) {
-            f32x4 e[4];
-#pragma unroll
-            for (int c = 0; c < 4; ++c)
-                e[c] = fma_s4(sgn, *reinterpret_cast<const f32x4*>(lds + in_b[c >> 1] + (c & 1) * in_cs + mt * in_ms),
-                              *reinterpret_cast<const f32x4*>(lds + in_a[c >> 1] + (c & 1) * in_cs + mt * in_ms));
-            vn[mt][0] = sub_s4(e[0], e[2]); vn[mt][1] = add_s4(e[1], e[2]); vn[mt][2] = sub_s4(e[2], e[1]); vn[mt][3] = sub_s4(e[1], e[3]);
+#pragma unroll
+            for (int x = mt * 4; x < (mt ? kNC : 4); ++x)
+                e[x] = fma_s4(sgn, *reinterpret_cast<const f32x4*>(lds + FPC_H3_FB(x)), *reinterpret_cast<const f32x4*>(lds + FPC_H3_FA(x)));
+#pragma unroll
+            for (int j = 0; j < 4; ++j) vn[mt][j] = FPC_H3_COLUMN(e, mt, j);
 #pragma unroll
             for (int j = 0; j < 3; ++j) { FPC_H3_SPLIT_PAIR(j, mt, 0, 0); FPC_H3_SPLIT_PAIR(j, mt, 1, 0); }
         }
@@ -143,14 +151,12 @@
     for (int p = 0; p < npair; ++p) {
         {
             const float* InE = lds + ((2 * p + 1) & 3) * kInFloats;
-            f32x4 ea[2][4], eb[2][4];
-#pragma unroll
-            for (int mt = 0; mt < 2; ++mt)
-#pragma unroll
-                for (int c = 0; c < 4; ++c) {
-                    ea[mt][c] = *reinterpret_cast<const f32x4*>(InE + in_a[c >> 1] + (c & 1) * in_cs + mt * in_ms);
-                    eb[mt][c] = *reinterpret_cast<const f32x4*>(InE + in_b[c >> 1] + (c & 1) * in_cs + mt * in_ms);
-                }
+            f32x4 ea[kNC], eb[kNC];
+#pragma unroll
+            for (int x = 0; x < kNC; ++x) {
+                ea[x] = *reinterpret_cast<const f32x4*>(InE + FPC_H3_FA(x));
+                eb[x] = *reinterpret_cast<const f32x4*>(InE + FPC_H3_FB(x));
+            }
             __builtin_amdgcn_sched_barrier(0);
             if (sn < nkb) { FPC_H3_ISSUE_IN((sn & 3), isb); isb += 8; }
             if (sn + 1 < nkb) { FPC_H3_ISSUE_IN(((sn + 1) & 3), isb); isb += 8; }
@@ -158,18 +164,19 @@
 #pragma unroll
             for (int q = 0; q < 4; ++q) FPC_H3_SPLIT_Q(3, q, 0);
             __builtin_amdgcn_sched_barrier(0);
+            f32x4 e[kNC];
 #pragma unroll
             for (int mt = 0; mt < 2; ++mt) {
-                f32x4 e[4];
-#pragma unroll
-                for (int c = 0; c < 4; ++c) e[c] = fma_s4(sgn, eb[mt][c], ea[mt][c]);
-                vn[mt][0] = sub_s4(e[0], e[2]); vn[mt][1] = add_s4(e[1], e[2]); vn[mt][2] = sub_s4(e[2], e[1]); vn[mt][3] = sub_s4(e[1], e[3]);
+#pragma unroll
+                for (int x = mt * 4; x < (mt ? kNC : 4); ++x) e[x] = fma_s4(sgn, eb[x], ea[x]);
+#pragma unroll
+                for (int j = 0; j < 4; ++j) vn[mt][j] = FPC_H3_COLUMN(e, mt, j);
                 FPC_H3_SPLIT_PAIR(0, mt, 0, 1); FPC_H3_SPLIT_PAIR(0, mt, 1, 1);
             }
         }
         __builtin_amdgcn_sched_barrier(0);
         const float* In = lds + ((2 * p + 2) & 3) * kInFloats;
-        f32x4 da[2][4], db[2][4], e[2][4];
+        f32x4 da[kNC], db[kNC], e[kNC];
         __builtin_amdgcn_s_setprio(1);
 #pragma unroll
         for (int j = 0; j < 4; ++j)
@@ -191,25 +198,22 @@
                         }
                         if (sl < 4) {
 #pragma unroll
-                            for (int c = 2 * (sl & 1); c < 2 * (sl & 1) + 2; ++c) {
-                                da[sl >> 1][c] = *reinterpret_cast<const f32x4*>(In + in_a[c >> 1] + (c & 1) * in_cs + (sl >> 1) * in_ms);
-                                db[sl >> 1][c] = *reinterpret_cast<const f32x4*>(In + in_b[c >> 1] + (c & 1) * in_cs + (sl >> 1) * in_ms);
+                            for (int q = kNR * sl; q < kNR * sl + kNR; ++q) {
+                                if ((q & 1) == 0) da[q >> 1] = *reinterpret_cast<const f32x4*>(In + FPC_H3_FA(q >> 1));
+                                if ((q & 1) == 1) db[q >> 1] = *reinterpret_cast<const f32x4*>(In + FPC_H3_FB(q >> 1));
                             }
                         }
-                        if (sl >= 4 && sl < 12) {
-                            const int m_ = (sl - 4) >> 2, c = (sl - 4) & 3;
-                            e[m_][c] = fma_s4(sgn, db[m_][c], da[m_][c]);
-                            FPC_H3_PIN4(e[m_][c]);
+                        if (sl >= 12 - kNC && sl < 12) {
+                            const int x = sl - (12 - kNC);
+                            e[x] = fma_s4(sgn, db[x], da[x]);
+                            FPC_H3_PIN4(e[x]);
                         }
                         if (sl < 4) FPC_H3_SPLIT_Q(1, sl, 1);
                         if (sl >= 4 && sl < 8) FPC_H3_SPLIT_Q(2, sl - 4, 1);
                         if (sl >= 8 && sl < 12) FPC_H3_SPLIT_Q(3, sl - 8, 1);
                         if (sl >= 12 && sl < 20 && !(SKIPC && ((sl - 12) & 3) == 2)) {
                             const int m_ = (sl - 12) >> 2, jx = (sl - 12) & 3;
-                            if (jx == 0) vn[m_][0] = sub_s4(e[m_][0], e[m_][2]);
-                            if (jx == 1) vn[m_][1] = add_s4(e[m_][1], e[m_][2]);
-                            if (jx == 2) vn[m_][2] = sub_s4(e[m_][2], e[m_][1]);
-                            if (jx == 3) vn[m_][3] = sub_s4(e[m_][1], e[m_][3]);
+                            vn[m_][jx] = FPC_H3_COLUMN(e, m_, jx);
                             FPC_H3_PIN4(vn[m_][jx]);
                         }
                         if (sl >= 20 && sl < 24) FPC_H3_SPLIT_Q(0, sl - 20, 0);
@@ -234,6 +238,9 @@
 #undef FPC_H3_LOAD_U1_AT
 #undef FPC_H3_LOAD_U2_AT
 #undef FPC_H3_XI_LIVE
+#undef FPC_H3_FA
+#undef FPC_H3_FB
+#undef FPC_H3_COLUMN
     };
 
     if (!FOLD) {
@@ -250,7 +257,7 @@
     }
     long long* const fdbg = (!(FOLD && PACK) && fine) ? dbg + (size_t)gridDim.x * 32 + ((size_t)blockIdx.x * 4 + wi) * 16 : nullptr;
     if (fdbg && lane == 0) { fdbg[0] = t_dec - t_entry; fdbg[1] = t_wld - t_entry; fdbg[2] = t_plan - t_entry; fdbg[3] = t_zero - t_entry; fdbg[4] = t_issued - t_entry; }
-    wino_output<PACK, FOLD, TR>(lds, acc, P, pt, WinoEpi{H, W, Cout, a.relu, a.tbx, a.tby, a.pack_rx}, inv_s,
+    wino_output<PACK, FOLD, TR, XS>(lds, acc, P, pt, WinoEpi{H, W, Cout, a.relu, a.tbx, a.tby, a.pack_rx}, inv_s,
                             wino_group(a.btab[0], a.btab[1], a.btab[2], a.btab[3], grp), dbg, t_kend, t, wi, fdbg);
 }
 
@@ -274,6 +281,45 @@
     return q;
 }
 
+int wino_tile_frag(bool xs, int wi, int lane, int pk_ks, long long* out17) {
+    if (wi < 0 || wi > 3 || lane < 0 || lane > 63 || pk_ks < 0) return FPC_EINVAL;
+    int in_a[2], in_b[2];
+    if (xs) wino_frag<true, true>(in_a, in_b, wi, lane & 31, lane >> 5, pk_ks);
+    else wino_frag<true, false>(in_a, in_b, wi, lane & 31, lane >> 5, pk_ks);
+    const int n = xs ? 6 : 8;
+    out17[0] = n;
+    for (int x = 0; x < n; ++x) {
+        out17[1 + 2 * x] = 4 * (xs ? wino_frag_at<true>(in_a, 0, x) : wino_frag_at<false>(in_a, x >> 2, x & 3));
+        out17[2 + 2 * x] = 4 * (xs ? wino_frag_at<true>(in_b, 0, x) : wino_frag_at<false>(in_b, x >> 2, x & 3));
+    }
+    return 0;
+}
+int wino_tile_slot(bool xs, bool tr, int slot, int y_in0, int x_in0, int H, int W, int Cs, int up, int pk_ks, int pk_two, long long* out6) {
+    if (slot < 0 || slot >= 5 * 4 * 64 || pk_ks < 0 || H < 1 || W < 1 || Cs < 8 || up < 0 || up > 1) return FPC_EINVAL;
+    const WinoSlot u = xs ? wino_slot<true>(slot, pk_ks) : wino_slot<false>(slot, pk_ks);
+    const WinoSrc q = xs ? (tr ? wino_stage_src<true, true, true>(slot, y_in0, x_in0, H, W, Cs, up, pk_ks, pk_two != 0)
+                               : wino_stage_src<true, false, true>(slot, y_in0, x_in0, H, W, Cs, up, pk_ks, pk_two != 0))
+                         : (tr ? wino_stage_src<true, true, false>(slot, y_in0, x_in0, H, W, Cs, up, pk_ks, pk_two != 0)
+                               : wino_stage_src<true, false, false>(slot, y_in0, x_in0, H, W, Cs, up, pk_ks, pk_two != 0));
+    out6[0] = 2 * u.ah + ((u.block >> 2) & 1); out6[1] = 2 * u.qh + ((u.block >> 1) & 1); out6[2] = u.block & 1;
+    out6[3] = u.qh > pk_ks; out6[4] = q.ok; out6[5] = q.off;
+    return 0;
+}
+int wino_tile_zrun(bool xs, int wi, int mt, int r, int nt, int cc, long long* out3) {
+    if (wi < 0 || wi > 3 || (mt | nt | cc) < 0 || (mt | nt | cc) > 1 || r < 0 || r > 15) return FPC_EINVAL;
+    out3[0] = z_run(cc, mt, r, nt, xs) + 256 * wi;
+    for (int hb = 0; hb < 2; ++hb) {
+        const int li = (r & 3) + 8 * (r >> 2) + 4 * hb;
+        out3[1 + hb] = xs ? 8 * (li >> 2) + 2 * (li & 3) + mt : 32 * mt + li;
+    }
+    return 0;
+}
+int wino_tile_zread(bool xs, int t_e, int tp, int cc, int i, long long* out1) {
+    if (t_e < 0 || t_e > 255 || tp < 0 || tp > 3 || cc < 0 || cc > 1 || i < 0 || i > 3) return FPC_EINVAL;
+    out1[0] = z_read_base(t_e >> 4, t_e & 15, xs) + z_read_step(tp, cc, i, xs);
+    return 0;
+}
+
 static int wino_fold_check(const WinoArgs& a, int groups) {
     if (a.Cin2 % 16 != 0 || (a.H | a.W) & 1 || (long long)(a.H / 2) * (a.W / 2) * a.Cin2 * (long long)sizeof(float) >= (1LL << 32) ||
         (long long)(a.Cin2 >> 4) * kPairBytes >= (1LL << 31) || a.relu || a.dbg)
@@ -304,22 +350,27 @@
         const WinoArgs& a = a_in;
         WinoArgs t = a;
         std::swap(t.H, t.W);
-        if (a.pack < 1 || a.dbg) return FPC_EINVAL;
+        if (a.pack < 1) return FPC_EINVAL;
         if (const int rc = wino_tile_check(t, groups, 16, kPairBytes, true, &nblk)) return rc;
         t.dec = wino_decode(t.Cout, groups, t.tbx, t.tby, t.W, t.B, t.pack);
+        if (a.xshare && !wino_xshare_rule(t.W)) return FPC_EINVAL;
         if (a.fold) {
             if (const int rc = wino_fold_check(a, groups)) return rc;
-            hipLaunchKernelGGL((k_conv_wino_h3<0, true, true, true>), dim3((unsigned)nblk), dim3(256), 0, s, t);
+            if (a.xshare) hipLaunchKernelGGL((k_conv_wino_h3<0, true, true, true, true>), dim3((unsigned)nblk), dim3(256), 0, s, t);
+            else hipLaunchKernelGGL((k_conv_wino_h3<0, true, true, true>), dim3((unsigned)nblk), dim3(256), 0, s, t);
         } else {
-            hipLaunchKernelGGL((k_conv_wino_h3<0, false, true, true>), dim3((unsigned)nblk), dim3(256), 0, s, t);
+            if (a.xshare) hipLaunchKernelGGL((k_conv_wino_h3<0, false, true, true, true>), dim3((unsigned)nblk), dim3(256), 0, s, t);
+            else hipLaunchKernelGGL((k_conv_wino_h3<0, false, true, true>), dim3((unsigned)nblk), dim3(256), 0, s, t);
         }
         return check_launch();
     }
     if (const int rc = wino_tile_check(a_in, groups, 16, kPairBytes, a_in.pack > 1, &nblk)) return rc;
     WinoArgs a = a_in;
     a.dec = wino_decode(a.Cout, groups, a.tbx, a.tby, a.W, a.B, a.pack > 1 ? a.pack : 0);
+    if (a.xshare && (a.pack <= 1 || a.fold || !wino_xshare_rule(a.W))) return FPC_EINVAL;
     if (a.pack > 1) {
-        hipLaunchKernelGGL((k_conv_wino_h3<0, false, true>), dim3((unsigned)nblk), dim3(256), 0, s, a);
+        if (a.xshare) hipLaunchKernelGGL((k_conv_wino_h3<0, false, true, false, true>), dim3((unsigned)nblk), dim3(256), 0, s, a);
+        else hipLaunchKernelGGL((k_conv_wino_h3<0, false, true>), dim3((unsigned)nblk), dim3(256), 0, s, a);
         return check_launch();
     }
     if (a.fold) {
diff --git a/fastposecnn_amd/csrc/wino_tile.hpp b/fastposecnn_amd/csrc/wino_tile.hpp
--- a/fastposecnn_amd/csrc/wino_tile.hpp
+++ b/fastposecnn_amd/csrc/wino_tile.hpp
@@ -18,10 +18,18 @@
 constexpr int kInFloats = kInPieces * 256;
 constexpr int kPairBytes = 16 * 2 * 2 * 64 * 16;
 constexpr int kZOdd = 64 * 1024 + 128;
-constexpr int z_run(int cc, int mt, int r, int nt) { return ((((cc * 2 + mt) * 8 + (r >> 1)) * 2 + nt) * 4) * 256 + (r & 1) * kZOdd; }
+constexpr int z_run(int cc, int mt, int r, int nt, bool xs = false) {
+    return ((((cc * 2 + (xs ? (r & 1) : mt)) * 8 + (r >> 1)) * 2 + nt) * 4) * 256 + (xs ? mt : (r & 1)) * kZOdd;
+}
+constexpr int z_read_base(int otl, int oq, bool xs = false) {
+    return xs ? z_run(0, otl & 1, (otl >> 1) & 3, oq >> 3, true) + (otl >> 3) * 128 + (oq & 7) * 16
+              : z_run(0, 0, (otl & 3) + 4 * (otl >> 3), oq >> 3) + ((otl >> 2) & 1) * 128 + (oq & 7) * 16;
+}
+constexpr int z_read_step(int tp, int cc, int i, bool xs = false) { return (xs ? z_run(cc, 0, 4 * tp, 0, true) : z_run(cc, tp >> 1, 8 * (tp & 1), 0)) + 256 * i; }
 constexpr int kZOddM0 = 64704;
 constexpr int kZM0Slack = 65535 - 3 * 256 - kZOddM0;
 static_assert(z_run(1, 1, 15, 1) - kZOddM0 < 65536 && z_run(0, 0, 1, 0) >= kZOddM0 && kZM0Slack >= 0, "ds_write_addtid_b32's reach");
+static_assert(z_run(1, 1, 15, 1, true) == z_run(1, 1, 15, 1) && z_run(0, 1, 0, 0, true) == z_run(0, 0, 1, 0) && z_run(1, 0, 15, 1, true) < 65536 - 3 * 256, "... and the x-shared map's");
 constexpr int kLdsFloats = 4 * 2 * kNT * kBN + 32;
 static_assert(z_run(1, 1, 15, 1) + 3 * 256 + 256 == kLdsFloats * 4, "the last run ends the image");
 
@@ -82,26 +90,48 @@
     return r;
 }
 
-template <bool PACK, bool TR = false>
+struct WinoSlot { int ah, qh, block; bool ok; };
+template <bool XS>
+constexpr WinoSlot wino_slot(int slot, int ks) {
+    const int blk = slot >> 4, res = slot & 15, cell = blk >> 3;
+    const int ah = (cell / 3) * 4 + (res & 3);
+    if (!XS) return WinoSlot{ah, (cell % 3) * 4 + (res >> 2), blk & 7, true};
+    const int col = cell % 3, g = res >> 2;
+    const bool seam = ks < kTX;
+    if (col < 2) return WinoSlot{ah, 2 * g + col + ((seam && 2 * g + col >= ks) ? 1 : 0), blk & 7, true};
+    if (seam && ks > 0 && g == (ks >> 1)) return WinoSlot{ah, ks, blk & 7, true};
+    return WinoSlot{ah, kTX + (seam ? 1 : 0), blk & 7, g == 0};
+}
+constexpr int wino_xs_unit(int ah, int qh, int block, int ks) {
+    const bool seam = ks < kTX;
+    const int u = qh - ((seam && qh > ks) ? 1 : 0);
+    const bool last = seam && qh == ks;
+    const int col = (last || u == kTX) ? 2 : (u & 1), g = last ? (ks >> 1) : ((u >> 1) & 3);
+    return (((ah >> 2) * 3 + col) * 8 + block) * 16 + 4 * g + (ah & 3);
+}
+struct WinoSrc { bool ok; unsigned off; };
+template <bool PACK, bool TR = false, bool XS = false>
+constexpr WinoSrc wino_stage_src(int slot, int y_in0, int x_in0, int H, int W, int Cs, int up, int pk_ks, bool pk_two) {
+    const int Hs = H >> up, Ws = W >> up;
+    const WinoSlot us = wino_slot<XS>(slot, pk_ks);
+    const int blk = us.block, ah = us.ah, qh = us.qh;
+    const int hf = blk & 1;
+    const int ry = 2 * ah + ((blk >> 2) & 1), rx = 2 * qh + ((blk >> 1) & 1);
+    const bool far = PACK && qh > pk_ks;
+    const int y = y_in0 + ry, x = far ? rx - 2 * pk_ks - 3 : x_in0 + rx;
+    const int qmax = (PACK && pk_ks < kTX) ? kTX + 1 : kTX;
+    const bool iok = slot < kInPieces * 64 && us.ok && ah <= kTY && qh <= qmax && y >= 0 && y < H && x >= 0 && x < W && (!far || pk_two);
+    const size_t px = TR ? (size_t)(x >> up) * Hs + (y >> up) : (size_t)(y >> up) * Ws + (x >> up);
+    return WinoSrc{iok, iok ? (unsigned)((px * Cs + 4 * hf) * sizeof(float)) + (far ? (unsigned)((size_t)Hs * Ws * Cs * sizeof(float)) : 0u) : 0u};
+}
+template <bool PACK, bool TR = false, bool XS = false>
 __device__ __forceinline__ void wino_stage_plan(unsigned (&ivo)[5], unsigned long long (&imask)[5], int wi, int lane, int y_in0, int x_in0, int H,
                                                 int W, int Cs, int up, int pk_ks, bool pk_two) {
-    const int Hs = H >> up, Ws = W >> up;
 #pragma unroll
     for (int i = 0; i < 5; ++i) {
-        const int slot = (wi + 4 * i) * 64 + lane;
-        const int blk = slot >> 4, res = slot & 15, cell = blk >> 3;
-        const int ah = (cell / 3) * 4 + (res & 3), qh = (cell % 3) * 4 + (res >> 2);
-        const int hf = blk & 1;
-        const int ry = 2 * ah + ((blk >> 2) & 1), rx = 2 * qh + ((blk >> 1) & 1);
-        const bool far = PACK && qh > pk_ks;
-        const int y = y_in0 + ry, x = far ? rx - 2 * pk_ks - 3 : x_in0 + rx;
-        const int qmax = (PACK && pk_ks < kTX) ? kTX + 1 : kTX;
-        const bool iok = wi + 4 * i < kInPieces && ah <= kTY && qh <= qmax && y >= 0 && y < H && x >= 0 && x < W && (!far || pk_two);
-        const size_t px = TR ? (size_t)(x >> up) * Hs + (y >> up) : (size_t)(y >> up) * Ws + (x >> up);
-        ivo[i] = iok ? (unsigned)((px * Cs + 4 * hf) * sizeof(float)) +
-                              (far ? (unsigned)((size_t)Hs * Ws * Cs * sizeof(float)) : 0u)
-                        : 0u;
-        imask[i] = __ballot(iok);
+        const WinoSrc q = wino_stage_src<PACK, TR, XS>((wi + 4 * i) * 64 + lane, y_in0, x_in0, H, W, Cs, up, pk_ks, pk_two);
+        ivo[i] = q.off;
+        imask[i] = __ballot(q.ok);
     }
 }
 #pragma clang diagnostic push
@@ -126,18 +156,25 @@
 
 constexpr int in_cs = 2 * 16 * 4;
 constexpr int in_ms = 3 * 8 * 16 * 4;
-template <bool PACK>
-__device__ __forceinline__ float wino_frag(int (&in_a)[2], int (&in_b)[2], int wi, int li, int lh, int pk_ks) {
-    const int tyl = li >> 3, txl = (li & 7) + ((PACK && (li & 7) >= pk_ks) ? 1 : 0);
+constexpr int in_xc = 8 * 16 * 4;
+template <bool PACK, bool XS = false>
+__host__ __device__ __forceinline__ float wino_frag(int (&in_a)[2], int (&in_b)[2], int wi, int li, int lh, int pk_ks) {
+    const int tyl = XS ? li >> 2 : li >> 3;
+    const int txl = XS ? 2 * (li & 3) + ((PACK && 2 * (li & 3) >= pk_ks) ? 1 : 0) : (li & 7) + ((PACK && (li & 7) >= pk_ks) ? 1 : 0);
     const int ra = (wi == 0) ? 0 : (wi == 2 ? 2 : 1);
     const int rb = (wi == 0) ? 2 : (wi == 1 ? 2 : (wi == 2 ? 1 : 3));
     auto unit = [&](int r, int ch) {
         const int ah = tyl + (r >> 1), qh = txl + ch;
+        if (XS) return wino_xs_unit(ah, qh, (r & 1) * 4 + lh, PACK ? pk_ks : 99) * 4;
         return ((((ah >> 2) * 3 + (qh >> 2)) * 8 + (r & 1) * 4 + lh) * 16 + 4 * (qh & 3) + (ah & 3)) * 4;
     };
-    in_a[0] = unit(ra, 0); in_a[1] = unit(ra, 1);
-    in_b[0] = unit(rb, 0); in_b[1] = unit(rb, 1);
+    in_a[0] = unit(ra, 0); in_a[1] = unit(ra, XS ? 2 : 1);
+    in_b[0] = unit(rb, 0); in_b[1] = unit(rb, XS ? 2 : 1);
     return (wi == 1) ? 1.f : -1.f;
+}
+template <bool XS>
+__host__ __device__ __forceinline__ int wino_frag_at(const int (&in_x)[2], int mt, int c) {
+    return XS ? ((c >> 1) == 2 ? in_x[1] : in_x[0] + (c >> 1) * in_xc) + (c & 1) * in_cs : in_x[c >> 1] + (c & 1) * in_cs + mt * in_ms;
 }
 __device__ __forceinline__ void wino_zero_ring(float* lds, int t, int nbuf, int y_in0, int x_in0, int H, int W, bool seam) {
     if (y_in0 < 0 || x_in0 < 0 || y_in0 + kRH > H || x_in0 + kRW > W || seam) {
@@ -150,7 +187,7 @@
 struct WinoEpi { int H, W, Cout, relu, tbx, tby, pack_rx; };
 #pragma clang diagnostic push
 #pragma clang diagnostic ignored "-Winline-asm"
-template <bool PACK, bool FOLD, bool TR = false>
+template <bool PACK, bool FOLD, bool TR = false, bool XS = false>
 __device__ __forceinline__ void wino_output(float* lds, const f32x16 (&acc)[4][2][2], const ConvPtrs P, const WinoPatch pt, const WinoEpi e,
                                             const float inv_s, const float* btab, long long* dbg, const long long t_kend, const int t,
                                             const int wi, long long* fdbg = nullptr) {
@@ -186,6 +223,7 @@
                 for (int cc = 0; cc < 2; ++cc)
 #pragma unroll
                     for (int odd = 0; odd < 2; ++odd) {
+                        const int late = XS ? mt : odd;
                         float z[8];
 #pragma unroll
                         for (int h = 0; h < 8; ++h) {
@@ -193,14 +231,14 @@
                             const float m0 = acc[0][mt][nt][r], m1 = acc[1][mt][nt][r], m2 = acc[2][mt][nt][r], m3 = acc[3][mt][nt][r];
                             z[h] = cc == 0 ? m0 + m1 + m2 : m1 - m2 - m3;
                         }
-#define FPC_Z_IMM(H) "i"(z_run(cc, mt, 2 * (H) + odd, nt) - odd * kZOddM0)
+#define FPC_Z_IMM(H) "i"(z_run(cc, mt, 2 * (H) + odd, nt, XS) - late * kZOddM0)
                         asm volatile("s_mov_b32 m0, %8\n s_nop 0\n"
                                      "ds_write_addtid_b32 %0 offset:%9\n ds_write_addtid_b32 %1 offset:%10\n"
                                      "ds_write_addtid_b32 %2 offset:%11\n ds_write_addtid_b32 %3 offset:%12\n"
                                      "ds_write_addtid_b32 %4 offset:%13\n ds_write_addtid_b32 %5 offset:%14\n"
                                      "ds_write_addtid_b32 %6 offset:%15\n ds_write_addtid_b32 %7 offset:%16\n"
                                      :: "v"(z[0]), "v"(z[1]), "v"(z[2]), "v"(z[3]), "v"(z[4]), "v"(z[5]), "v"(z[6]), "v"(z[7]),
-                                        "s"(zm0 + odd * kZOddM0), FPC_Z_IMM(0), FPC_Z_IMM(1), FPC_Z_IMM(2), FPC_Z_IMM(3), FPC_Z_IMM(4),
+                                        "s"(zm0 + late * kZOddM0), FPC_Z_IMM(0), FPC_Z_IMM(1), FPC_Z_IMM(2), FPC_Z_IMM(3), FPC_Z_IMM(4),
                                         FPC_Z_IMM(5), FPC_Z_IMM(6), FPC_Z_IMM(7)
                                      : "memory", "m0");
 #undef FPC_Z_IMM
@@ -211,8 +249,7 @@
     __syncthreads();
     if (kWinoStamp && fdbg && (t & 63) == 0) fdbg[10] = clock64() - t_kend;
     f32x4 s1 = {0.f, 0.f, 0.f, 0.f}, s2 = {0.f, 0.f, 0.f, 0.f};
-    const float* const zr = lds + z_run(0, 0, (otl & 3) + 4 * (otl >> 3), oq >> 3) / 4 +
-                            ((otl >> 2) & 1) * 32 + (oq & 7) * 4;
+    const float* const zr = lds + z_read_base(otl, oq, XS) / 4;
 #pragma unroll
     for (int tp = 0; tp < 4; ++tp) {
         const int ot = otl + 16 * tp;
@@ -221,7 +258,7 @@
 #pragma unroll
         for (int i = 0; i < 4; ++i)
 #pragma unroll
-            for (int cc = 0; cc < 2; ++cc) z[i][cc] = *reinterpret_cast<const f32x4*>(zr + (z_run(cc, tp >> 1, 8 * (tp & 1), 0) + 256 * i) / 4);
+            for (int cc = 0; cc < 2; ++cc) z[i][cc] = *reinterpret_cast<const f32x4*>(zr + z_read_step(tp, cc, i, XS) / 4);
 #pragma unroll
         for (int rr = 0; rr < 2; ++rr)
 #pragma unroll
diff --git a/fastposecnn_amd/engine.py b/fastposecnn_amd/engine.py
--- a/fastposecnn_amd/engine.py
+++ b/fastposecnn_amd/engine.py
@@ -158,6 +158,9 @@
     def set_wino_orient(self, on):
         nat.check(self._lib.fpc_net_set_wino_orient(self._h, int(on)), "fpc_net_set_wino_orient")
 
+    def set_wino_xshare(self, on):
+        nat.check(self._lib.fpc_net_set_wino_xshare(self._h, int(on)), "fpc_net_set_wino_xshare")
+
     def wino_blocks(self):
         return int(self._lib.fpc_net_wino_blocks(self._h))
 
diff --git a/include/fpc.h b/include/fpc.h
--- a/include/fpc.h
+++ b/include/fpc.h
@@ -252,11 +252,18 @@
 int fpc_wino_orient_geometry(int H, int W, int B, int Cin, int fold, int pack, int64_t* out9);
 int fpc_wino_recip(uint32_t d, int64_t* out2);
 int fpc_wino_decode(int Cout, int groups, int tbx, int tby, int W, int B, int pack, int64_t* out14);
+int fpc_wino_xshare_rule(int W);
+int fpc_net_set_wino_xshare(fpc_net_t* net, int on);
+int fpc_wino_tile_frag(int xshare, int wi, int lane, int pk_ks, int64_t* out17);
+int fpc_wino_tile_slot(int xshare, int tr, int slot, int y_in0, int x_in0, int H, int W, int Cs, int up, int pk_ks, int pk_two, int64_t* out6);
+int fpc_wino_tile_zrun(int xshare, int wi, int mt, int r, int nt, int cc, int64_t* out3);
+int fpc_wino_tile_zread(int xshare, int t_e, int tp, int cc, int i, int64_t* out1);
 int64_t fpc_net_wino_blocks(const fpc_net_t* net);
 int fpc_net_flops(const fpc_net_t* net, double* out3);
 int fpc_net_tensor(const fpc_net_t* net, const char* name, const float** ptr, int* H, int* W, int* C);
 
 enum {
+    FPC_PLAN_WINO_ORIENT_ROWSPLIT = -13, FPC_PLAN_WINO_PACKED_ROWSPLIT = -12,
     FPC_PLAN_WINO_ORIENT = -11, FPC_PLAN_WINO_PACKED = -10, FPC_PLAN_TWO_LAUNCH = 100, FPC_PLAN_BF3 = 1000, FPC_PLAN_LATERAL = 2000, FPC_PLAN_STEM = 3000,
     FPC_PLAN_STEM_POOL = 3100, FPC_PLAN_POINTWISE = 4000, FPC_PLAN_FOLDED = 5000, FPC_PLAN_H3 = 6000, FPC_PLAN_LATERAL_H3 = 7000,
     FPC_PLAN_GROUPED = 8000
diff --git a/tools_dev/wino_xshare_stamps.py b/tools_dev/wino_xshare_stamps.py
--- /dev/null
+++ b/tools_dev/wino_xshare_stamps.py
@@ -0,0 +1,45 @@
+import ctypes, os, sys
+sys.path.insert(0, os.path.dirname(os.path.dirname(os.path.abspath(__file__))))
+import torch
+from fastposecnn_amd import _native as nat
+dev = torch.device("cuda:0"); L = nat.lib()
+if not hasattr(L, "fpc_dbg_wino_diag"):
+    sys.exit("wino_xshare_stamps.py needs a diagnostic build of the library (-DFPC_STAMP_WINO)")
+ROUNDS, LAUNCHES = 5, 20
+shapes = [(32, 64, 120, 160, 64), (32, 128, 60, 80, 128), (32, 256, 120, 160, 128)]
+if len(sys.argv) > 5:
+    v = [int(a) for a in sys.argv[1:]]
+    shapes = [tuple(v[i:i + 5]) for i in range(0, len(v) - 4, 5)]
+for B, Cin, H, W, Cout in shapes:
+    o9 = (ctypes.c_int64 * 9)()
+    nat.check(L.fpc_wino_orient_geometry(H, W, B, Cin, 0, 1, o9), "geometry")
+    tr = bool(o9[0])
+    codes = (-13, -11) if tr else (-12, -10)
+    xs = bool(L.fpc_wino_xshare_rule(H if tr else W)) and (tr or o9[1] > 1)
+    x = torch.randn((B, H, W, Cin), device=dev); w = torch.randn((Cout, Cin, 3, 3), device=dev) * 0.05
+    out = torch.empty((B, H, W, Cout), device=dev)
+    ws = torch.empty(L.fpc_conv2d_workspace_bytes(B, H, W, Cin, Cout, 3, 3), dtype=torch.uint8, device=dev)
+    nblk = -(-((W + 1) // 2) // 8) * -(-((H + 1) // 2) // 8) * B * (Cout // 64)
+    dbg = torch.zeros((nblk, 4, 8), dtype=torch.int64, device=dev)
+    sb, sh, sw, sc = x.stride(); st = torch.cuda.current_stream().cuda_stream
+    rows = {c: [] for c in codes}
+    for _ in range(ROUNDS):
+        for c in codes:
+            dbg.zero_()
+            for _ in range(LAUNCHES):
+                nat.check(L.fpc_conv2d(x.data_ptr(), sb, sh, sw, sc, w.data_ptr(), None, None, None, None, out.data_ptr(), dbg.data_ptr(),
+                                       B, H, W, Cin, Cout, 3, 3, 1, 1, 77, 0, 0, c, ws.data_ptr(), ws.numel(), st), "conv")
+            torch.cuda.synchronize()
+            d = dbg.cpu().double().reshape(-1, 8)
+            d = d[d[:, 5] > 0]
+            rows[c].append((d.shape[0] // 4, (d[:, 3] / (d[:, 5] / 2)).mean().item(), d[:, 6].mean().item(), d[:, 7].mean().item(),
+                            (d[:, 3] / d[:, 4] * 100.0).mean().item()))
+    print(f"{B} x {Cin} x {H} x {W} -> {Cout}  ({'transposed' if tr else 'stored orientation'}, {'x-shared map taken' if xs else 'ROW-SPLIT ON BOTH REQUESTS'})")
+    for c in codes:
+        t = torch.tensor(rows[c])
+        print(f"  request {c}: workgroups {int(t[0, 0])}  cycles per pair {t[:, 1].mean():8.1f} (rounds {t[:, 1].min():.1f} .. {t[:, 1].max():.1f})"
+              f"  entry {t[:, 2].mean():7.0f} ({t[:, 2].min():.0f} .. {t[:, 2].max():.0f})  exit {t[:, 3].mean():7.0f} ({t[:, 3].min():.0f} .. {t[:, 3].max():.0f})"
+              f"  clock {t[:, 4].mean():.0f} MHz")
+    a, b = torch.tensor(rows[codes[0]]), torch.tensor(rows[codes[1]])
+    print(f"  x-shared - row-split: pair {b[:, 1].mean() - a[:, 1].mean():+.1f} cycles ({(b[:, 1].mean() / a[:, 1].mean() - 1) * 100:+.2f} %), "
+          f"entry {b[:, 2].mean() - a[:, 2].mean():+.0f}, exit {b[:, 3].mean() - a[:, 3].mean():+.0f}")
```

Result: faster. 2809, median of 6 (+1.1%).
